# BoyBaykiller/OpenTK-PathTracer

Hardware: AMD Instinct MI355X
Metric: Msamples/sec + ms/frame @1080p 8-bounce default scene, 1/2/4/8 GPU (higher is better)
Workload: dtype f32

## Files before the change

### opentk-pathtracer_amd/csrc/mi355pt.cpp

```cpp
#include "pt_renderer.hpp"

#include <cmath>
#include <cstdio>
#include <cstdlib>
#include <chrono>
#include <thread>
#include <cstring>
#include <new>

namespace {
thread_local std::string g_create_error;
}

namespace ptimpl {

#define FEED_LOG(...)                                                                                                                \
    do {                                                                                                                             \
        if (pt::tuning().feedLog) {                                                                                                  \
            std::fprintf(stderr, "[feed %9.1f us] ", std::chrono::duration<double, std::micro>(std::chrono::steady_clock::now().time_since_epoch()).count() - 1e6 * (long long)(std::chrono::duration<double>(std::chrono::steady_clock::now().time_since_epoch()).count())); \
            std::fprintf(stderr, "%p ", (void *)h);                                                                                  \
            std::fprintf(stderr, __VA_ARGS__);                                                                                       \
            std::fprintf(stderr, "\n");                                                                                              \
        }                                                                                                                            \
    } while (0)
// ... 97 lines not shown
}

unsigned int feed_word(const pt_renderer::FeedState &f, bool closed)
{
    return (closed ? pt::kFeedClosed : 0u) | ((unsigned int)f.published << 16) | (f.slots16 & 0xffffu);
}

void feed_close(pt_handle h)
{
    pt_renderer::FeedState &f = h->feed;
    if (!f.open) return;
    f.open = false;
    __atomic_store_n(&h->hostFeed[f.hostWord], feed_word(f, true), __ATOMIC_RELEASE);
    FEED_LOG("close word %d = %08x (first %d published %d pendingSlot %d)", f.hostWord, feed_word(f, true), f.firstFrame, f.published, f.pendingSlot);
    for (pt_renderer::LaunchRecord &r : h->unverified)
        if (r.a.launchSeq == f.seq) r.a.batchFrames = f.published;
    const unsigned int tickets = (unsigned int)(((long long)f.published * f.tilesFrame + f.queueChunk - 1) / f.queueChunk);
    (f.streamIdx == 1 ? h->chainQueueBase : h->stripeQueueBase[0]) += tickets;
    for (int j = 0; j < f.published; j++) h->feedDoneBase[f.streamIdx][j & 7] += f.pixelsPerFrame;
    if (f.published >= 8) h->feedIdleStrikes = 0;
    if (f.pendingSlot >= 0) {
        h->fusedOrphanSlot = f.pendingSlot;
        f.pendingSlot = -1;
    }
}

static int resolve_fused_orphan(pt_handle h)
{
    if (h->fusedOrphanSlot < 0) return PT_OK;
    FEED_LOG("orphan present of slot %d: tone map from the image", h->fusedOrphanSlot);
    PresentSlot &s = h->slots[h->fusedOrphanSlot];
    h->fusedOrphanSlot = -1;
    if (!s.fusedWaiting) return PT_OK;
    void *const image = s.boundDev ? s.boundDev : s.dRgba8;
    const size_t pixels = (size_t)s.rows * s.width;
    PT_HIP(h, ptimpl::launch_tone_map(s.arithmetic, h->accum(), image, pixels, h->stream));
    PT_HIP(h, hipEventRecord(s.toneMapped, h->stream));
    PT_HIP(h, hipStreamWaitEvent(h->copyStream, s.toneMapped, 0));
    if (!s.boundDev) PT_HIP(h, hipMemcpyAsync(s.host, s.dRgba8, pixels * 4, hipMemcpyDeviceToHost, h->copyStream));
    PT_HIP(h, hipEventRecord(s.copied, h->copyStream));
    s.fusedWaiting = false;
    s.fedPresent = false;
    s.snapSource = nullptr;
    return PT_OK;
}

int join_stripes(pt_handle h, bool repairNow)
{
    FEED_LOG("join (repairNow %d, frame %d, pending %d, tagsLive %d, %zu remembered, flag %u)", (int)repairNow, h->frame, h->pendingFrames, (int)h->tagsLive, h->unverified.size(),
             h->hostErrWord ? *(volatile unsigned int *)h->hostErrWord : 0u);
    feed_close(h);
    if (h->pendingFrames > 0) {
        h->flushFinal = true;
        int rc = flush_frames(h);
        h->flushFinal = false;
        if (rc) return rc;
    }
    h->snapFrame = -1;
    h->mainDirty = true;
    h->chainBroken = true;
    if (h->chainPending) {
        PT_HIP(h, hipStreamWaitEvent(h->stream, h->chainDone, 0));
        h->chainPending = false;
    }
    for (int j = 0; j < kMaxStripes; j++) {
        if (h->stripePending[j]) {
            if (j > 0) PT_HIP(h, hipStreamWaitEvent(h->stream, h->stripeDone[j], 0));
            h->stripePending[j] = false;
        }
    }
    const bool raised = h->hostErrWord && *(volatile unsigned int *)h->hostErrWord;
    if (raised || (!h->unverified.empty() && (repairNow || h->tagsLive))) {
        if (raised) note_abandonment(h);
        if (int rc = enqueue_repairs(h, !raised && !h->repairPendingAll)) return rc;
        h->repairPendingAll = false;
    }
    return resolve_fused_orphan(h);
}

int settle_handover(pt_handle h)
{
    if (h->hostErrWord && *(volatile unsigned int *)h->hostErrWord) {
        note_abandonment(h);
        if (int rc = enqueue_repairs(h, false)) return rc;
        h->repairPendingAll = false;
        PT_HIP(h, hipStreamSynchronize(h->stream));
    }
    if (!h->unverified.empty()) FEED_LOG("settle: %zu launches forgotten (synchronised, flag down)", h->unverified.size());
    h->unverified.clear();
    if (h->repairCheckDue) {
        h->repairCheckDue = false;
        unsigned int ctl[4] = {0, 0, 0, 0};
        PT_HIP(h, hipMemcpy(ctl, h->dRepairCtl, sizeof ctl, hipMemcpyDeviceToHost));
        if (ctl[1] != h->inconsistentSeen) {
            h->inconsistentSeen = ctl[1];
            return fail(h, PT_E_HIP, "hand-over repair: a pixel's frame tag fits no launch of this handle (image inconsistent; pt_reset / pt_set_size start over)");
        }
    }
    return PT_OK;
}

int fix_alpha(pt_handle h, bool repairNow)
{
    if (int rc = join_stripes(h, repairNow)) return rc;
    if (h->tagsLive) {
        PT_HIP(h, pt::launch_set_alpha(h->accum(), h->tilePixels(), h->stream));
        h->tagsLive = false;
    }
    return PT_OK;
}

int ensure_stripe(pt_handle h, int j)
{
    if (j > 0 && !h->stripeStream[j]) PT_HIP(h, hipStreamCreateWithFlags(&h->stripeStream[j], hipStreamNonBlocking));
    if (!h->stripeDone[j]) PT_HIP(h, hipEventCreateWithFlags(&h->stripeDone[j], hipEventDisableTiming));
    return PT_OK;
}

hipStream_t stripe_stream(pt_handle h, int j) { return j == 0 ? h->stream : h->stripeStream[j]; }

int free_first_hit(pt_handle h)
{
    if (!h->dFirstHit) return PT_OK;
    PT_HIP(h, hipStreamSynchronize(h->stream));
    PT_HIP(h, hipFree(h->dFirstHit));
    h->dFirstHit = nullptr;
    return PT_OK;
}

int free_denoise(pt_handle h)
{
    h->denoiseResult = -1;
    h->denoiseVarianceValid = false;
    h->denoiseIntegratedValid = h->denoiseHistoryUsed = false;
    for (pt_renderer::DenoiseSet &set : h->denoiseSet) set.valid = false;
    if (!h->dGuides && !h->dDenoise[0] && !h->dDenoise[1] && !h->dVariance && !h->denoiseSet[0].image && !h->denoiseSet[0].guides &&
        !h->denoiseSet[1].image && !h->denoiseSet[1].guides)
        return PT_OK;
    PT_HIP(h, hipStreamSynchronize(h->stream));
    if (h->dGuides) PT_HIP(h, hipFree(h->dGuides));
    h->dGuides = nullptr;
    if (h->dVariance) PT_HIP(h, hipFree(h->dVariance));
    h->dVariance = nullptr;
    for (float4 *&img : h->dDenoise) {
        if (img) PT_HIP(h, hipFree(img));
        img = nullptr;
    }
    for (pt_renderer::DenoiseSet &set : h->denoiseSet) {
        if (set.image) PT_HIP(h, hipFree(set.image));
        set.image = nullptr;
        if (set.guides) PT_HIP(h, hipFree(set.guides));
        set.guides = nullptr;
    }
    return PT_OK;
}
}

namespace {

int ensure_accum(pt_handle h)
{
    size_t need = h->tilePixels();
    if (need > h->accumCapacity) {
        if (h->dAccum) PT_HIP(h, hipFree(h->dAccum));
        h->dAccum = nullptr;
        h->accumCapacity = 0;
        PT_HIP(h, hipMalloc((void **)&h->dAccum, need * sizeof(float4)));
        h->accumCapacity = need;
    }
    if ((size_t)((h->width + 7) / 8) * (size_t)((h->rows + 7) / 8) > h->tileMaskTiles) {
        const size_t tiles = (size_t)((h->width + 7) / 8) * (size_t)((h->rows + 7) / 8);
        PT_HIP(h, hipStreamSynchronize(h->stream));
        if (h->dTileMasks) PT_HIP(h, hipFree(h->dTileMasks));
        h->dTileMasks = nullptr;
        h->tileMaskTiles = 0;
        h->tileMasksValid = false;
        PT_HIP(h, hipMalloc((void **)&h->dTileMasks, tiles * pt::kTileMaskWords * sizeof(unsigned long long)));
        h->tileMaskTiles = tiles;
    }
    const size_t flagTiles = (size_t)((h->width + 7) / 8) * (size_t)((h->rows + 7) / 8);
    if (flagTiles > h->tileFlagTiles) {
        PT_HIP(h, hipStreamSynchronize(h->stream));
        if (h->dTileFlags) PT_HIP(h, hipFree(h->dTileFlags));
        h->dTileFlags = nullptr;
        h->tileFlagTiles = 0;
        PT_HIP(h, hipMalloc((void **)&h->dTileFlags, flagTiles * sizeof(unsigned int)));
        PT_HIP(h, hipMemsetAsync(h->dTileFlags, 0, flagTiles * sizeof(unsigned int), h->stream));
        h->tileFlagTiles = flagTiles;
    }
#ifdef PT_AUDIT
    if (need > h->auditCapacity) {
        PT_HIP(h, hipStreamSynchronize(h->stream));
        if (h->dAudit) PT_HIP(h, hipFree(h->dAudit));
        h->dAudit = nullptr;
        h->auditCapacity = 0;
        PT_HIP(h, hipMalloc((void **)&h->dAudit, need * sizeof(unsigned long long)));
        h->auditCapacity = need;
    }
#endif
    return PT_OK;
}

int audit_forget(pt_handle h)
{
    if (h->dAudit) PT_HIP(h, hipMemsetAsync(h->dAudit, 0xFF, h->tilePixels() * sizeof(unsigned long long), h->stream));
    return PT_OK;
}

int clear_accum(pt_handle h)
{
    if (h->boundAccum && h->boundBytes < h->tilePixels() * sizeof(float4))
        return fail(h, PT_E_BAD_ARGUMENT, "bound result buffer is smaller than the tile");
    if (int rc = join_stripes(h)) return rc;
    PT_HIP(h, pt::launch_clear(h->accum(), h->tilePixels(), h->stream));
    h->tagsLive = false;
    return audit_forget(h);
}

}

extern "C" {

PT_API const char *pt_version(void) { return "mi355pt 0.1 (gfx950, pt-f32)"; }

PT_API int pt_device_count(void)
{
    int n = 0;
    if (hipGetDeviceCount(&n) != hipSuccess) return 0;
    return n;
}

PT_API const char *pt_last_error(pt_handle h)
{
    if (h && h->magic == ptimpl::kAlive) return h->error.c_str();
    return g_create_error.c_str();
}

PT_API int pt_create(int device_id, int width, int height, pt_handle *out)
{
    if (!out) return fail(nullptr, PT_E_BAD_ARGUMENT, "out == NULL");
    *out = nullptr;
    if (width <= 0 || height <= 0) return fail(nullptr, PT_E_BAD_ARGUMENT, "width/height must be positive");
    if (width > PT_MAX_IMAGE_DIM || height > PT_MAX_IMAGE_DIM)
        return fail(nullptr, PT_E_OUT_OF_RANGE, "width/height exceed PT_MAX_IMAGE_DIM (32767)");
    int n = 0;
    hipError_t e = hipGetDeviceCount(&n);
    if (e != hipSuccess || n <= 0)
        return fail(nullptr, PT_E_NO_DEVICE, "no HIP device available (libmi355pt has no CPU fallback)");
    if (device_id < 0 || device_id >= n) return fail(nullptr, PT_E_BAD_ARGUMENT, "device_id out of range");
    pt_renderer *h = new (std::nothrow) pt_renderer();
    if (!h) return fail(nullptr, PT_E_OUT_OF_MEMORY, "host allocation failed");
    h->device = device_id;
    {
        const pt::Tuning &t = pt::tuning();
        if (t.drainCompaction >= -1) h->drainCompaction = t.drainCompaction;
        if (t.batchWorkgroupsPerCU >= 1 && t.batchWorkgroupsPerCU <= 8) h->batchWorkgroupsPerCU = t.batchWorkgroupsPerCU;
        if (t.frameBatch >= 1 && t.frameBatch <= 64) { h->maxBatch = t.frameBatch; h->maxBatchExplicit = true; }
        if (t.queueChunk >= 1 && t.queueChunk <= 1024) h->queueChunk = t.queueChunk;
    }
    h->width = width;
    h->height = height;
    h->y0 = 0;
    h->rows = height;
#define PT_CREATE_HIP(call)                                                                                            \
    do {                                                                                                               \
        hipError_t e2_ = (call);                                                                                       \
        if (e2_ != hipSuccess) {                                                                                       \
            int rc_ = hip_fail(nullptr, e2_, #call);                                                                   \
            pt_destroy(h);                                                                                             \
            return rc_;                                                                                                \
        }                                                                                                              \
    } while (0)
    PT_CREATE_HIP(hipSetDevice(device_id));
    PT_CREATE_HIP(hipStreamCreateWithFlags(&h->ownStream, hipStreamNonBlocking));
    h->stream = h->ownStream;
    PT_CREATE_HIP(hipEventCreateWithFlags(&h->inputsReady, hipEventDisableTiming));
    PT_CREATE_HIP(hipEventCreateWithFlags(&h->gatherReady, hipEventDisableTiming));
    PT_CREATE_HIP(hipStreamCreateWithFlags(&h->copyStream, hipStreamNonBlocking));
    PT_CREATE_HIP(hipEventCreate(&h->evBegin));
    PT_CREATE_HIP(hipEventCreate(&h->evEnd));
    PT_CREATE_HIP(hipMalloc((void **)&h->dObjects, PT_GAME_OBJECTS_UBO_SIZE));
    PT_CREATE_HIP(hipMemsetAsync(h->dObjects, 0, PT_GAME_OBJECTS_UBO_SIZE, h->stream));
    PT_CREATE_HIP(hipMalloc((void **)&h->dGrid, (ptgrid::kMaxCells + 1) * 2 + ptgrid::kMaxRefs + 16));
    PT_CREATE_HIP(hipMalloc((void **)&h->dLut, 256 * sizeof(float)));
    PT_CREATE_HIP(hipMalloc((void **)&h->dQueue, ptimpl::kQueueWords * sizeof(unsigned int)));
    PT_CREATE_HIP(hipMemsetAsync(h->dQueue, 0, ptimpl::kQueueWords * sizeof(unsigned int), h->stream));
    PT_CREATE_HIP(hipHostMalloc((void **)&h->hostErrWord, sizeof(unsigned int), hipHostMallocMapped));
    *h->hostErrWord = 0;
    PT_CREATE_HIP(hipHostGetDevicePointer((void **)&h->devErrWord, h->hostErrWord, 0));
    PT_CREATE_HIP(hipMalloc((void **)&h->dAbandon, sizeof(unsigned int)));
    PT_CREATE_HIP(hipMemsetAsync(h->dAbandon, 0xFF, sizeof(unsigned int), h->stream));
    PT_CREATE_HIP(hipMalloc((void **)&h->dRepairCtl, 4 * sizeof(unsigned int)));
    PT_CREATE_HIP(hipMemsetAsync(h->dRepairCtl, 0, 4 * sizeof(unsigned int), h->stream));
    {
        int khz = 0;
        if (hipDeviceGetAttribute(&khz, hipDeviceAttributeWallClockRate, device_id) != hipSuccess || khz <= 0) khz = 100000;
        (void)hipGetLastError();
        h->wallClockKhz = khz;
        const pt::Tuning &t = pt::tuning();
        const double unitsPerMs = (double)khz / 1024.0;
        double budget = (double)t.handoverBudgetMs * unitsPerMs, check = (double)t.handoverCheckUs * unitsPerMs / 1000.0;
        if (budget > 1.0e9) budget = 1.0e9;
        if (check > budget / 4.0) check = budget / 4.0;
        h->waitBudgetUnits = (unsigned int)budget;
        h->waitCheckUnits = (unsigned int)check;
    }
    PT_CREATE_HIP(hipHostMalloc((void **)&h->hostFeed, pt_renderer::kFeedHostWords * sizeof(unsigned int), hipHostMallocMapped | hipHostMallocCoherent));
    for (int i = 0; i < pt_renderer::kFeedHostWords; i++) h->hostFeed[i] = pt::kFeedClosed;
    PT_CREATE_HIP(hipHostMalloc((void **)&h->hostFeedDone, pt_renderer::kFeedHostWords * sizeof(unsigned int), hipHostMallocMapped | hipHostMallocCoherent));
    std::memset(h->hostFeedDone, 0, pt_renderer::kFeedHostWords * sizeof(unsigned int));
    PT_CREATE_HIP(hipHostGetDevicePointer((void **)&h->devFeedHostDone, h->hostFeedDone, 0));
    PT_CREATE_HIP(hipHostGetDevicePointer((void **)&h->devFeedHost, h->hostFeed, 0));
    PT_CREATE_HIP(hipMalloc((void **)&h->dFeedDev, (size_t)2 * pt::kFeedBcastSlots * pt::kFeedBcastStride * sizeof(unsigned int)));
    PT_CREATE_HIP(hipMemsetAsync(h->dFeedDev, 0, (size_t)2 * pt::kFeedBcastSlots * pt::kFeedBcastStride * sizeof(unsigned int), h->stream));
    PT_CREATE_HIP(hipMalloc((void **)&h->dFeedDone, (size_t)16 * pt::kFeedDoneStride * sizeof(unsigned long long)));
    PT_CREATE_HIP(hipMemsetAsync(h->dFeedDone, 0, (size_t)16 * pt::kFeedDoneStride * sizeof(unsigned long long), h->stream));
    PT_CREATE_HIP(hipHostMalloc((void **)&h->hostStarted, ptimpl::kStartedWords * sizeof(unsigned int), hipHostMallocMapped | hipHostMallocCoherent));
    std::memset(h->hostStarted, 0, ptimpl::kStartedWords * sizeof(unsigned int));
    PT_CREATE_HIP(hipHostGetDevicePointer((void **)&h->devStarted, h->hostStarted, 0));
#ifdef PT_AUDIT
    {
        const size_t words = 4 + (size_t)pt::kAuditLogRecords * pt::kAuditRecordWords;
        PT_CREATE_HIP(hipHostMalloc((void **)&h->hostAuditLog, words * sizeof(unsigned int), hipHostMallocMapped | hipHostMallocCoherent));
        std::memset(h->hostAuditLog, 0, words * sizeof(unsigned int));
        PT_CREATE_HIP(hipHostGetDevicePointer((void **)&h->devAuditLog, h->hostAuditLog, 0));
    }
#endif
    {
        hipDeviceProp_t prop;
        PT_CREATE_HIP(hipGetDeviceProperties(&prop, device_id));
        h->numCUs = prop.multiProcessorCount > 0 ? prop.multiProcessorCount : 256;
    }
    float lut[256];
    make_srgb_lut(lut);
    PT_CREATE_HIP(hipMemcpyAsync(h->dLut, lut, sizeof lut, hipMemcpyHostToDevice, h->stream));
    PT_CREATE_HIP(hipStreamSynchronize(h->stream));
#undef PT_CREATE_HIP
    int rc = ensure_accum(h);
    if (rc == PT_OK) rc = clear_accum(h);
    if (rc != PT_OK) {
        g_create_error = h->error;
        pt_destroy(h);
        return rc;
    }
    *out = h;
    return PT_OK;
}

PT_API int pt_destroy(pt_handle h)
{
    PT_CHECK_HANDLE(h);
    if (h->isGroup()) return ptimpl::group_destroy(h);
    h->pendingFrames = 0;
    (void)hipSetDevice(h->device);
    ptimpl::feed_close(h);
    for (int j = 0; j < ptimpl::kMaxStripes; j++)
        if (h->stripeStream[j]) (void)hipStreamSynchronize(h->stripeStream[j]);
    if (h->stream) (void)hipStreamSynchronize(h->stream);
    if (h->copyStream) (void)hipStreamSynchronize(h->copyStream);
    for (int k = 0; k < pt_renderer::kSnapshots; k++) {
        if (h->snapRead[k]) (void)hipEventDestroy(h->snapRead[k]);
        if (h->dSnap[k]) (void)hipFree(h->dSnap[k]);
    }
    ptimpl::free_slots(h);
    if (h->copyStream) (void)hipStreamDestroy(h->copyStream);
    if (h->gatherReady) (void)hipEventDestroy(h->gatherReady);
    for (int j = 0; j < ptimpl::kMaxStripes; j++)
        if (h->stripeStream[j]) (void)hipStreamSynchronize(h->stripeStream[j]);
    if (h->stream) (void)hipStreamSynchronize(h->stream);
    for (int j = 0; j < ptimpl::kMaxStripes; j++) {
        if (h->stripeDone[j]) (void)hipEventDestroy(h->stripeDone[j]);
        if (h->stripeStream[j]) (void)hipStreamDestroy(h->stripeStream[j]);
    }
    if (h->inputsReady) (void)hipEventDestroy(h->inputsReady);
    for (hipEvent_t e : h->launchEvents)
        if (e) (void)hipEventDestroy(e);
    if (h->dAbandon) (void)hipFree(h->dAbandon);
    if (h->dRepairCtl) (void)hipFree(h->dRepairCtl);
    if (h->dTileFlags) (void)hipFree(h->dTileFlags);
    if (h->dObjects) (void)hipFree(h->dObjects);
    if (h->dGrid) (void)hipFree(h->dGrid);
    if (h->dLut) (void)hipFree(h->dLut);
    if (h->dQueue) (void)hipFree(h->dQueue);
    if (h->dTileMasks) (void)hipFree(h->dTileMasks);
    if (h->hostErrWord) (void)hipHostFree(h->hostErrWord);
    if (h->hostStarted) (void)hipHostFree(h->hostStarted);
    if (h->hostFeed) (void)hipHostFree(h->hostFeed);
    if (h->hostFeedDone) (void)hipHostFree(h->hostFeedDone);
    if (h->dFeedDev) (void)hipFree(h->dFeedDev);
    if (h->dFeedDone) (void)hipFree(h->dFeedDone);
    for (hipEvent_t e : h->feedWordBusy)
        if (e) (void)hipEventDestroy(e);
    if (h->feedResetEvent) (void)hipEventDestroy(h->feedResetEvent);
    if (h->hostAuditLog) (void)hipHostFree(h->hostAuditLog);
    if (h->dAudit) (void)hipFree(h->dAudit);
    if (h->dEnv) (void)hipFree(h->dEnv);
    if (h->dAccum) (void)hipFree(h->dAccum);
    if (h->dRgba8) (void)hipFree(h->dRgba8);
    if (h->dFirstHit) (void)hipFree(h->dFirstHit);
    if (h->dPick) (void)hipFree(h->dPick);
    if (h->dGuides) (void)hipFree(h->dGuides);
    if (h->dVariance) (void)hipFree(h->dVariance);
    if (h->dDenoise[0]) (void)hipFree(h->dDenoise[0]);
    if (h->dDenoise[1]) (void)hipFree(h->dDenoise[1]);
    for (pt_renderer::DenoiseSet &set : h->denoiseSet) {
        if (set.image) (void)hipFree(set.image);
        if (set.guides) (void)hipFree(set.guides);
    }
    if (h->dTimeline) (void)hipFree(h->dTimeline);
    if (h->evBegin) (void)hipEventDestroy(h->evBegin);
    if (h->evEnd) (void)hipEventDestroy(h->evEnd);
    if (h->ownStream) (void)hipStreamDestroy(h->ownStream);
    h->magic = 0;
    delete h;
    return PT_OK;
}

PT_API int pt_set_size(pt_handle h, int width, int height)
{
    PT_CHECK_HANDLE(h);
    if (width <= 0 || height <= 0) return fail(h, PT_E_BAD_ARGUMENT, "width/height must be positive");
    if (width > PT_MAX_IMAGE_DIM || height > PT_MAX_IMAGE_DIM)
        return fail(h, PT_E_OUT_OF_RANGE, "width/height exceed PT_MAX_IMAGE_DIM (32767)");
    if (h->isGroup()) return ptimpl::group_set_size(h, width, height);
    if (int rc = flush_frames(h)) return rc;
    if (int rc = bind_device(h)) return rc;
    if (int rc = join_stripes(h)) return rc;
    if (int rc = ptimpl::free_first_hit(h)) return rc;
    if (int rc = ptimpl::free_denoise(h)) return rc;
    h->resetEpoch++;
    h->width = width;
    h->height = height;
    h->y0 = 0;
    h->rows = height;
    h->bandRows = 0;
    h->frame = 0;
    h->tileMasksValid = false;
    h->launchesSinceInputChange = 0;
    if (int rc = ensure_accum(h)) return rc;
    return clear_accum(h);
}

PT_API int pt_set_tile(pt_handle h, int y0, int rows)
{
    PT_CHECK_HANDLE(h);
    if (h->isGroup()) return fail(h, PT_E_BAD_ARGUMENT, "a group handle owns its tiling (pt_multi_set_partition)");
    if (int rc = flush_frames(h)) return rc;
    if (y0 < 0 || rows <= 0 || y0 + rows > h->height) return fail(h, PT_E_BAD_ARGUMENT, "tile outside the image");
    if (int rc = bind_device(h)) return rc;
    if (int rc = join_stripes(h)) return rc;
    if (int rc = ptimpl::free_first_hit(h)) return rc;
    if (int rc = ptimpl::free_denoise(h)) return rc;
    h->resetEpoch++;
    h->y0 = y0;
    h->rows = rows;
    h->bandRows = 0;
    h->frame = 0;
    h->tileMasksValid = false;
    h->launchesSinceInputChange = 0;
    if (int rc = ensure_accum(h)) return rc;
    return clear_accum(h);
}

PT_API int pt_set_interleaved_tile(pt_handle h, int rank, int world, int band_rows)
{
    PT_CHECK_HANDLE(h);
    if (h->isGroup()) return fail(h, PT_E_BAD_ARGUMENT, "a group handle owns its tiling (pt_multi_set_partition)");
    if (int rc = flush_frames(h)) return rc;
    if (world < 1 || rank < 0 || rank >= world || band_rows < 8 || (band_rows & 7))
        return fail(h, PT_E_BAD_ARGUMENT, "need 0 <= rank < world and band_rows a positive multiple of 8");
    if (int rc = bind_device(h)) return rc;
    long long rows = 0;
    for (long long b = rank; b * band_rows < h->height; b += world) {
        long long top = (b + 1) * band_rows;
        rows += (top < h->height ? top : h->height) - b * band_rows;
    }
    if (rows <= 0) return fail(h, PT_E_BAD_ARGUMENT, "this rank owns no rows (image too small for world * band_rows)");
    if (int rc = join_stripes(h)) return rc;
    if (int rc = ptimpl::free_first_hit(h)) return rc;
    if (int rc = ptimpl::free_denoise(h)) return rc;
    h->resetEpoch++;
    h->y0 = 0;
    h->rows = (int)rows;
    h->bandRows = band_rows;
    h->bandWorld = world;
    h->bandRank = rank;
    h->frame = 0;
    h->tileMasksValid = false;
    h->launchesSinceInputChange = 0;
    if (int rc = ensure_accum(h)) return rc;
    return clear_accum(h);
}

#define PT_FAN_OUT(h, call)                                                                                            \
    do {                                                                                                               \
        if ((h)->isGroup()) {                                                                                          \
            for (pt_handle part : (h)->parts) {                                                                        \
                int rc_ = (call);                                                                                      \
                if (rc_ != PT_OK) return fail((h), rc_, part->error);                                                  \
            }                                                                                                          \
            return PT_OK;                                                                                              \
        }                                                                                                              \
    } while (0)

PT_API int pt_reset(pt_handle h)
{
    PT_CHECK_HANDLE(h);
    PT_FAN_OUT(h, pt_reset(part));
    if (int rc = flush_frames(h)) return rc;
    if (int rc = bind_device(h)) return rc;
    if (int rc = ptimpl::fix_alpha(h)) return rc;
    h->frame = 0;
    h->resetEpoch++;
    return audit_forget(h);
}

PT_API int pt_set_params(pt_handle h, int num_spheres, int num_cuboids, int ray_depth, int spp, float focal_length,
                         float aperture_diameter)
{
    PT_CHECK_HANDLE(h);
    PT_FAN_OUT(h, pt_set_params(part, num_spheres, num_cuboids, ray_depth, spp, focal_length, aperture_diameter));
    if (num_spheres == h->numSpheres && num_cuboids == h->numCuboids && ray_depth == h->rayDepth && spp == h->spp &&
        std::memcmp(&focal_length, &h->focalLength, sizeof(float)) == 0 && std::memcmp(&aperture_diameter, &h->apertureDiameter, sizeof(float)) == 0)
        return PT_OK;
    if (num_spheres < 0 || num_spheres > PT_MAX_SPHERES || num_cuboids < 0 || num_cuboids > PT_MAX_CUBOIDS)
        return fail(h, PT_E_OUT_OF_RANGE, "object counts exceed the GameObjectsUBO arrays (256 spheres / 64 cuboids)");
    if (ray_depth < 0 || spp < 1) return fail(h, PT_E_BAD_ARGUMENT, "ray_depth must be >= 0 and spp >= 1");
    if (ray_depth > PT_MAX_RAY_DEPTH || spp > PT_MAX_SPP)
        return fail(h, PT_E_OUT_OF_RANGE, "ray_depth / spp exceed PT_MAX_RAY_DEPTH / PT_MAX_SPP (4095)");
    if (int rc = flush_frames(h)) return rc;
    if (num_spheres != h->numSpheres) h->gridDirty = true;
    if (num_spheres != h->numSpheres || num_cuboids != h->numCuboids || focal_length != h->focalLength || aperture_diameter != h->apertureDiameter) {
        h->tileMasksValid = false;
        h->launchesSinceInputChange = 0;
    }
    h->numSpheres = num_spheres;
    h->numCuboids = num_cuboids;
    h->rayDepth = ray_depth;
    h->spp = spp;
    h->focalLength = focal_length;
    h->apertureDiameter = aperture_diameter;
    return PT_OK;
}

PT_API int pt_upload_basic_data(pt_handle h, int byte_offset, int size, const void *src)
{
    PT_CHECK_HANDLE(h);
    PT_FAN_OUT(h, pt_upload_basic_data(part, byte_offset, size, src));
    if (!src) return fail(h, PT_E_BAD_ARGUMENT, "src == NULL");
    if (byte_offset < 0 || size < 0 || (long long)byte_offset + size > PT_BASIC_DATA_UBO_SIZE)
        return fail(h, PT_E_OUT_OF_RANGE, "BasicDataUBO range outside [0,144)");
    if (std::memcmp(h->basic + byte_offset, src, (size_t)size) == 0) return PT_OK;
    h->statFlushes++;
    if (int rc = flush_frames(h)) return rc;
    std::memcpy(h->basic + byte_offset, src, (size_t)size);
    h->tileMasksValid = false; h->launchesSinceInputChange = 0;
    return PT_OK;
}

PT_API int pt_upload_game_objects(pt_handle h, int byte_offset, int size, const void *src)
{
    PT_CHECK_HANDLE(h);
    PT_FAN_OUT(h, pt_upload_game_objects(part, byte_offset, size, src));
    if (!src) return fail(h, PT_E_BAD_ARGUMENT, "src == NULL");
    if (byte_offset < 0 || size < 0 || (long long)byte_offset + size > PT_GAME_OBJECTS_UBO_SIZE)
        return fail(h, PT_E_OUT_OF_RANGE, "GameObjectsUBO range outside [0,26624)");
    if (size == 0) return PT_OK;
    if (std::memcmp(h->objectsShadow + byte_offset, src, (size_t)size) == 0) return PT_OK;
    h->statFlushes++;
    if (int rc = bind_device(h)) return rc;
    if (int rc = join_stripes(h)) return rc;
    PT_HIP(h, hipMemcpyAsync((char *)h->dObjects + byte_offset, src, (size_t)size, hipMemcpyHostToDevice, h->stream));
    std::memcpy(h->objectsShadow + byte_offset, src, (size_t)size);
    if (byte_offset < PT_MAX_SPHERES * 80) h->gridDirty = true;
    h->tileMasksValid = false;
    h->launchesSinceInputChange = 0;
    return PT_OK;
}

PT_API int pt_set_environment(pt_handle h, int face_size, int format, const void *const faces[6])
{
    PT_CHECK_HANDLE(h);
    PT_FAN_OUT(h, pt_set_environment(part, face_size, format, faces));
    if (face_size <= 0 || face_size > 16384) return fail(h, PT_E_BAD_ARGUMENT, "face_size out of range");
    if (format != PT_ENV_RGBA32F && format != PT_ENV_SRGB8_A8) return fail(h, PT_E_BAD_ARGUMENT, "unknown format");
    if (!faces) return fail(h, PT_E_BAD_ARGUMENT, "faces == NULL");
    for (int f = 0; f < 6; f++)
        if (!faces[f]) return fail(h, PT_E_BAD_ARGUMENT, "faces[i] == NULL");
    if (int rc = bind_device(h)) return rc;
    if (int rc = join_stripes(h)) return rc;
    size_t faceBytes = (size_t)face_size * face_size * (format == PT_ENV_RGBA32F ? 16 : 4);
    size_t total = faceBytes * 6;
    if (total > h->envBytes) {
        PT_HIP(h, hipStreamSynchronize(h->stream));
        if (h->dEnv) PT_HIP(h, hipFree(h->dEnv));
        h->dEnv = nullptr;
        h->envBytes = 0;
        PT_HIP(h, hipMalloc(&h->dEnv, total));
        h->envBytes = total;
    }
    for (int f = 0; f < 6; f++)
        PT_HIP(h, hipMemcpyAsync((char *)h->dEnv + f * faceBytes, faces[f], faceBytes, hipMemcpyHostToDevice, h->stream));
    h->envSize = face_size;
    h->envFormat = format;
    return PT_OK;
}

}

namespace {

bool gpu_busy(pt_handle h);

struct LaunchMode {
    bool tagged = false, chainable = false;
    int stripes = 1, kernelVariant = 0;
};

constexpr long long kSmallChunkBelowTiles = 12000;

int fill_frame_args(pt_handle h, pt::FrameArgs &a, int firstFrame, int n)
{
    std::memcpy(a.invProj, h->basic, 64);
    std::memcpy(a.invView, h->basic + 64, 64);
    std::memcpy(a.viewPos, h->basic + 128, 12);
    a.focalLength = h->focalLength;
    a.apertureDiameter = h->apertureDiameter;
    a.width = h->width;
    a.height = h->height;
    a.invW = 1.0f / (float)h->width;
    a.invH = 1.0f / (float)h->height;
    a.numSpheres = h->numSpheres;
    a.numCuboids = h->numCuboids;
    a.rayDepth = h->rayDepth;
    a.spp = h->spp;
    a.frame = firstFrame;
    a.batchFrames = n;
    a.envSize = h->envSize;
    a.envFormat = h->envFormat;
    a.objects = h->dObjects;
    a.env = h->dEnv;
    a.srgbLut = h->dLut;
    a.tilesX = (h->width + 7) / 8;
    a.bandRows = h->bandRows;
    a.bandWorld = h->bandWorld;
    a.bandRank = h->bandRank;
    a.localRow0 = 0;
    a.numCUs = h->numCUs;
    a.queueChunk = h->queueChunk > 0 ? h->queueChunk : (n > 1 && (long long)((h->width + 7) / 8) * ((h->rows + 7) / 8) < kSmallChunkBelowTiles ? 4 : 8);
    a.errorWord = h->devErrWord;
    a.startedFlags = nullptr;
    a.launchSeq = 0;
    a.snapshot = nullptr;
    a.audit = nullptr;
    a.auditLog = h->devAuditLog;
    a.auditSabotage = 0;
#ifdef PT_AUDIT
    a.auditSabotage = pt::tuning().auditSabotage;
#endif
    a.timeline = h->dTimeline;
    if (h->gridDirty) {
        h->gridDirty = false;
        h->grid = ptgrid::build((const float *)h->objectsShadow, h->numSpheres);
        ptgrid::sphere_runs((const float *)h->objectsShadow, h->numSpheres, h->sphereRunStart);
        if (h->grid.valid) {
            if (int rc = join_stripes(h)) return rc;
            PT_HIP(h, hipMemcpyAsync(h->dGrid, h->grid.packed.data(), h->grid.packed.size(), hipMemcpyHostToDevice, h->stream));
        }
    }
    a.grid = h->grid.valid ? h->dGrid : nullptr;
    a.gridBytes = h->grid.valid ? (int)h->grid.packed.size() : 0;
    a.gridLdsBytes = 0;
    for (int k = 0; k < 3; k++) {
        a.gridDims[k] = h->grid.dims[k];
        a.gridLo[k] = h->grid.lo[k];
        a.gridHi[k] = h->grid.hi[k];
        a.gridCell[k] = h->grid.cell[k];
        a.gridInvCell[k] = h->grid.invCell[k];
        a.gridCenter[k] = h->grid.center[k];
    }
    a.gridReach2 = h->grid.reach2;
    std::memcpy(a.sphereRunStart, h->sphereRunStart, sizeof(a.sphereRunStart));
    a.tileMasks = nullptr;
    a.tagged = 0;
    a.keepTags = 0;
    a.chainTag = 0.0f;
    a.abandonWord = nullptr;
    a.tileFlags = nullptr;
    a.waitBudget = h->waitBudgetUnits;
    a.waitCheckInterval = h->waitCheckUnits;
    return PT_OK;
}

LaunchMode choose_launch_mode(pt_handle h, pt::FrameArgs &a, int n)
{
    LaunchMode m;
    m.kernelVariant = h->variant;
    if (h->arithmetic != PT_ARITH_CONTRACT) {
        m.chainable = false;
        m.tagged = false;
        m.stripes = 1;
        m.kernelVariant = 1;
        a.variant = m.kernelVariant;
        a.drainCompaction = 0;
        a.tagged = 0;
        return m;
    }
    const bool noSingleTagged = pt::tuning().noSingleTagged != 0;
    m.chainable = h->variant == 0 && !h->externalStream() && !ptimpl::timeline_blocks_pipelining(h);
    m.tagged = h->variant == 0 && (n > 1 || (m.chainable && !noSingleTagged && (gpu_busy(h) || (h->sawBatch && h->presentCadence != 1))));
    const int shortWg = pt::tuning().shortWorkgroupsPerCU;
    if (m.tagged) { m.stripes = 1; m.kernelVariant = 10 + (n < 8 ? shortWg : h->batchWorkgroupsPerCU) - 1; h->batchLaunched = true; if (n > 1) h->sawBatch = true; }
    else if (h->variant == 0 && h->externalStream()) { m.stripes = 1; m.kernelVariant = 14; }
    else if (h->variant == 0) { m.stripes = 2; m.kernelVariant = 14; }
    else if (h->variant >= 20 && h->variant < 50) { m.stripes = h->variant / 10; m.kernelVariant = 10 + h->variant % 10; }
    if (h->rows < 16 * m.stripes) m.stripes = 1;
    a.variant = m.kernelVariant;
    a.drainCompaction = h->drainCompaction >= 0 ? h->drainCompaction : (m.stripes > 1 || m.tagged ? 0 : 32);
    a.tagged = m.tagged ? 1 : 0;
    return m;
}

int use_tile_masks(pt_handle h, pt::FrameArgs &a)
{
    if (pt::tuning().tileMasks == 0) return PT_OK;
    const bool settled = h->launchesSinceInputChange > 2;
    h->launchesSinceInputChange += a.batchFrames;
    if (!h->tileMasksValid && settled) {
        if (int rc = join_stripes(h)) return rc;
        if ((size_t)a.tilesX * a.tilesY <= h->tileMaskTiles) {
            PT_HIP(h, pt::launch_tile_masks(a, h->dTileMasks, h->stream));
            h->tileMasksValid = true;
            h->statMaskBuilds++;
        }
    }
    if (h->tileMasksValid) a.tileMasks = h->dTileMasks;
    return PT_OK;
}

bool predecessor_resident(pt_handle h)
{
    for (int i = 0; i < h->lastWorkgroups; i++)
        if (((volatile unsigned int *)h->hostStarted)[i] != h->launchSeq) return false;
    return true;
}
bool wait_for_residency(pt_handle h, const pt::FrameArgs &a, long waitUs)
{
    if (pt::tuning().serialLaunches != 0) return false;
    if (h->overlapHoldoff > 0) h->overlapHoldoff--;
    const bool mayChain = !h->chainBroken && h->lastWorkgroups > 0 && h->lastWorkgroups <= ptimpl::kStartedWords && h->overlapHoldoff == 0;
    bool resident = mayChain && predecessor_resident(h);
    const bool bigShare = (long long)a.tilesX * a.tilesY >= 12000;
    if (mayChain && !resident && (bigShare || h->flushFinal)) {
        const auto t0 = std::chrono::steady_clock::now();
        while (!resident) {
            const auto waited = std::chrono::duration_cast<std::chrono::microseconds>(std::chrono::steady_clock::now() - t0).count();
            if (waited >= waitUs) break;
            if (waited > 200) std::this_thread::sleep_for(std::chrono::microseconds(20));
            resident = predecessor_resident(h);
        }
    }
    return resident;
}

void arm_handover(pt_handle h, pt::FrameArgs &a)
{
    a.launchSeq = ++h->launchSeq;
    if (a.launchSeq == 0 || a.launchSeq >= 0xfffffff0u) a.launchSeq = h->launchSeq = 1;
    a.abandonWord = h->dAbandon;
    a.tileFlags = a.chainTag == 0.0f ? h->dTileFlags : nullptr;
}
void remember_launch(pt_handle h, const pt::FrameArgs &a, hipEvent_t done)
{
    auto flag_down = [&]() -> bool { return !(h->hostErrWord && *(volatile unsigned int *)h->hostErrWord); };
    while (h->unverified.size() > 2 && hipEventQuery(h->unverified.front().done) == hipSuccess && flag_down()) {
        FEED_LOG("remember: launch %u frames [%d,+%d) seen complete with the flag down: forgotten", h->unverified.front().a.launchSeq, h->unverified.front().a.frame, h->unverified.front().a.batchFrames);
        h->unverified.pop_front();
    }
    (void)hipGetLastError();
    static_assert(pt_renderer::kLaunchEvents / 2 <= pt::kMaxUnverifiedLaunches, "frame-tag window (pt_kernels.hpp)");
    if (h->unverified.size() >= (size_t)pt_renderer::kLaunchEvents / 2) {
        (void)hipEventSynchronize(h->unverified.front().done);
        if (flag_down()) h->unverified.pop_front();
    }
    h->unverified.push_back({a, done});
    FEED_LOG("launch %u frames [%d,+%d) chainTag %g keepTags %d variant %d spp %d (%zu remembered)", a.launchSeq, a.frame, a.batchFrames, (double)a.chainTag, a.keepTags, a.variant, a.spp, h->unverified.size());
    if (pt::tuning().feedLog >= 2) {
        unsigned int w = 0, q[2] = {0, 0};
        (void)hipDeviceSynchronize();
        (void)hipMemcpy(&w, h->dAbandon, 4, hipMemcpyDeviceToHost);
        (void)hipMemcpy(&q[0], h->dQueue, 4, hipMemcpyDeviceToHost);
        (void)hipMemcpy(&q[1], h->dQueue + ptimpl::kChainQueueWord, 4, hipMemcpyDeviceToHost);
        FEED_LOG("  after launch %u: abandon word %08x, tickets main %u (host %u) chain %u (host %u), flag %u", a.launchSeq, w, q[0], h->stripeQueueBase[0], q[1], h->chainQueueBase,
                 h->hostErrWord ? *(volatile unsigned int *)h->hostErrWord : 0u);
// ... 707 lines not shown
        if (int rc = join_stripes(h)) return rc;
        if (s.inFlight) PT_HIP(h, hipStreamWaitEvent(h->stream, s.copied, 0));
        PT_HIP(h, ptimpl::launch_tone_map(h->presentArithmetic, h->accum(), image, pixels, h->stream));
        PT_HIP(h, hipEventRecord(s.toneMapped, h->stream));
        PT_HIP(h, hipStreamWaitEvent(h->copyStream, s.toneMapped, 0));
    }
    if (!s.boundDev) PT_HIP(h, hipMemcpyAsync(s.host, s.dRgba8, pixels * 4, hipMemcpyDeviceToHost, h->copyStream));
    PT_HIP(h, hipEventRecord(s.copied, h->copyStream));
    s.inFlight = true;
    s.valid = false;
    s.frame = h->frame;
    s.rows = h->rows;
    s.width = h->width;
    s.arithmetic = h->presentArithmetic;
    s.snapSource = nullptr;
    return PT_OK;
}

PT_API int pt_present_bind_device_image(pt_handle h, int slot, void *device_rgba8, size_t bytes)
{
    PT_CHECK_HANDLE(h);
    if (slot < 0 || slot >= PT_PRESENT_SLOTS) return fail(h, PT_E_BAD_ARGUMENT, "slot must be 0..PT_PRESENT_SLOTS-1");
    if (h->isGroup()) return fail(h, PT_E_BAD_ARGUMENT, "pt_present_bind_device_image is not available on a group handle");
    if (device_rgba8 && bytes < h->tilePixels() * 4) return fail(h, PT_E_BAD_ARGUMENT, "device image smaller than rows*width*4 bytes");
    if (int rc = bind_device(h)) return rc;
    ptimpl::PresentSlot &s = h->slots[slot];
    if (h->feed.open || h->fusedOrphanSlot >= 0) {
        ptimpl::feed_close(h);
        if (int rc = join_stripes(h)) return rc;
    }
    if (s.inFlight) {
        if (int rc = ptimpl::wait_slot(h, s, nullptr)) return rc;
        s.inFlight = false;
    }
    s.valid = false;
    s.fedPresent = false;
    s.boundDev = device_rgba8;
    s.boundBytes = device_rgba8 ? bytes : 0;
    return PT_OK;
}

PT_API int pt_present_wait(pt_handle h, int slot, const uint8_t **out_host_rgba8, size_t *out_row_pitch_bytes,
                           int *out_frame_index)
{
    PT_CHECK_HANDLE(h);
    if (slot < 0 || slot >= PT_PRESENT_SLOTS) return fail(h, PT_E_BAD_ARGUMENT, "slot must be 0..PT_PRESENT_SLOTS-1");
    ptimpl::PresentSlot &s = h->slots[slot];
    if (!s.inFlight && !s.valid) return fail(h, PT_E_BAD_ARGUMENT, "nothing was presented into this slot");
    if (int rc = bind_device(h)) return rc;
    if (s.inFlight) {
        bool fusedAbandoned = false;
        if (int rc = ptimpl::wait_slot(h, s, &fusedAbandoned)) return rc;
        if (fusedAbandoned) s.abandonEpoch = h->abandonEpoch - 1;
        s.inFlight = false;
        s.valid = true;
        if (!h->isGroup() && s.snapSource != nullptr) {
            if (h->hostErrWord && *(volatile unsigned int *)h->hostErrWord) {
                if (int rc = join_stripes(h)) return rc;
                if (*(volatile unsigned int *)h->hostErrWord) ptimpl::note_abandonment(h);
            }
            if (s.abandonEpoch != h->abandonEpoch && s.fedPresent) {
                if (int rc = ptimpl::fix_alpha(h)) return rc;
                void *const image = s.boundDev ? s.boundDev : s.dRgba8;
                const size_t pixels = (size_t)s.rows * s.width;
                PT_HIP(h, ptimpl::launch_tone_map(s.arithmetic, h->accum(), image, pixels, h->stream));
                if (!s.boundDev) PT_HIP(h, hipMemcpyAsync(s.host, s.dRgba8, pixels * 4, hipMemcpyDeviceToHost, h->stream));
                PT_HIP(h, hipStreamSynchronize(h->stream));
                if (int rc = ptimpl::settle_handover(h)) return rc;
                s.abandonEpoch = h->abandonEpoch;
                s.frame = h->frame;
            } else if (s.abandonEpoch != h->abandonEpoch) {
                int k = -1;
                for (int i = 0; i < pt_renderer::kSnapshots; i++)
                    if (h->dSnap[i] == s.snapSource && h->snapGeneration[i] == s.snapGeneration) k = i;
                if (k < 0)
                    return fail(h, PT_E_HIP, "present: a launch was abandoned and this slot's snapshot has been reused (call pt_present_wait on a slot before presenting into it again)");
                if (int rc = join_stripes(h)) return rc;
                void *const image = s.boundDev ? s.boundDev : s.dRgba8;
                const size_t pixels = (size_t)s.rows * s.width;
                PT_HIP(h, ptimpl::launch_tone_map(s.arithmetic, h->dSnap[k], image, pixels, h->stream));
                if (!s.boundDev) PT_HIP(h, hipMemcpyAsync(s.host, s.dRgba8, pixels * 4, hipMemcpyDeviceToHost, h->stream));
                PT_HIP(h, hipStreamSynchronize(h->stream));
                s.abandonEpoch = h->abandonEpoch;
            }
        }
    }
    if (out_host_rgba8) *out_host_rgba8 = s.boundDev ? nullptr : s.host;
    if (out_row_pitch_bytes) *out_row_pitch_bytes = (size_t)s.width * 4;
    if (out_frame_index) *out_frame_index = s.frame;
    return PT_OK;
}

PT_API int pt_get_frame_index(pt_handle h, int *out)
{
    PT_CHECK_HANDLE(h);
    if (!out) return fail(h, PT_E_BAD_ARGUMENT, "out == NULL");
    *out = h->isGroup() ? h->parts[0]->frame : h->frame;
    return PT_OK;
}

PT_API int pt_synchronize(pt_handle h)
{
    PT_CHECK_HANDLE(h);
    PT_FAN_OUT(h, pt_synchronize(part));
    if (int rc = bind_device(h)) return rc;
    if (int rc = ptimpl::fix_alpha(h, false)) return rc;
    PT_HIP(h, hipStreamSynchronize(h->stream));
    return ptimpl::settle_handover(h);
}

PT_API int pt_atmosphere_upload_data(pt_handle h, int byte_offset, int size, const void *src)
{
    PT_CHECK_HANDLE(h);
    PT_FAN_OUT(h, pt_atmosphere_upload_data(part, byte_offset, size, src));
    if (!src) return fail(h, PT_E_BAD_ARGUMENT, "src == NULL");
    if (byte_offset < 0 || size < 0 || (long long)byte_offset + size > PT_ATMOSPHERE_UBO_SIZE)
        return fail(h, PT_E_OUT_OF_RANGE, "AtmosphericDataUBO range outside [0,464)");
    std::memcpy(h->atmoUbo + byte_offset, src, (size_t)size);
    return PT_OK;
}

PT_API int pt_atmosphere_render(pt_handle h, int size, int i_steps, int j_steps, const float light_pos[3],
                                float light_intensity)
{
    PT_CHECK_HANDLE(h);
    PT_FAN_OUT(h, pt_atmosphere_render(part, size, i_steps, j_steps, light_pos, light_intensity));
    if (size <= 0 || size > 8192 || i_steps < 0 || j_steps < 0 || !light_pos)
        return fail(h, PT_E_BAD_ARGUMENT, "bad atmosphere parameters");
    if (int rc = bind_device(h)) return rc;
    if (int rc = join_stripes(h)) return rc;
    size_t total = (size_t)6 * size * size * 16;
    if (total > h->envBytes) {
        PT_HIP(h, hipStreamSynchronize(h->stream));
        if (h->dEnv) PT_HIP(h, hipFree(h->dEnv));
        h->dEnv = nullptr;
        h->envBytes = 0;
        PT_HIP(h, hipMalloc(&h->dEnv, total));
        h->envBytes = total;
    }
    pt::AtmoArgs a;
    std::memcpy(a.invProj, h->atmoUbo, 64);
    std::memcpy(a.invView, h->atmoUbo + 64, 6 * 64);
    a.lightPos[0] = light_pos[0];
    a.lightPos[1] = light_pos[1];
    a.lightPos[2] = light_pos[2];
    a.lightIntensity = light_intensity < 0.0f ? 0.0f : light_intensity;
    a.size = size;
    a.iSteps = i_steps;
    a.jSteps = j_steps;
    a.out = (float4 *)h->dEnv;
    PT_HIP(h, h->atmoArithmetic == PT_ARITH_REFERENCE ? pt::launch_atmosphere_reference(a, h->stream) : pt::launch_atmosphere(a, h->stream));
    h->envSize = size;
    h->envFormat = PT_ENV_RGBA32F;
    return PT_OK;
}

PT_API int pt_atmosphere_set_arithmetic(pt_handle h, int mode)
{
    PT_CHECK_HANDLE(h);
    if (mode != PT_ARITH_CONTRACT && mode != PT_ARITH_REFERENCE) return fail(h, PT_E_BAD_ARGUMENT, "mode must be PT_ARITH_CONTRACT or PT_ARITH_REFERENCE");
    PT_FAN_OUT(h, pt_atmosphere_set_arithmetic(part, mode));
    h->atmoArithmetic = mode;
    return PT_OK;
}

PT_API int pt_present_set_arithmetic(pt_handle h, int mode)
{
    PT_CHECK_HANDLE(h);
    if (mode != PT_ARITH_CONTRACT && mode != PT_ARITH_REFERENCE) return fail(h, PT_E_BAD_ARGUMENT, "mode must be PT_ARITH_CONTRACT or PT_ARITH_REFERENCE");
    PT_FAN_OUT(h, pt_present_set_arithmetic(part, mode));
    if (mode == h->presentArithmetic) return PT_OK;
    if (int rc = bind_device(h)) return rc;
    if (int rc = join_stripes(h)) return rc;
    h->presentArithmetic = mode;
    return PT_OK;
}

PT_API int pt_read_environment(pt_handle h, float *dst, int *out_face_size)
{
    PT_CHECK_HANDLE(h);
    if (h->isGroup()) {
        int rc = pt_read_environment(h->parts[0], dst, out_face_size);
        return rc == PT_OK ? rc : fail(h, rc, h->parts[0]->error);
    }
    if (!h->dEnv) return fail(h, PT_E_NO_ENVIRONMENT, "no environment set");
    if (out_face_size) *out_face_size = h->envSize;
    if (!dst) return PT_OK;
    if (int rc = bind_device(h)) return rc;
    if (int rc = join_stripes(h)) return rc;
    size_t n = (size_t)6 * h->envSize * h->envSize;
    if (h->envFormat == PT_ENV_RGBA32F) {
        PT_HIP(h, hipMemcpyAsync(dst, h->dEnv, n * 16, hipMemcpyDeviceToHost, h->stream));
        PT_HIP(h, hipStreamSynchronize(h->stream));
        return PT_OK;
    }
    float4 *tmp = nullptr;
    PT_HIP(h, hipMalloc((void **)&tmp, n * 16));
    hipError_t e = pt::launch_env_to_float(h->dEnv, h->envSize, h->envFormat, h->dLut, tmp, h->stream);
    if (e == hipSuccess) e = hipMemcpyAsync(dst, tmp, n * 16, hipMemcpyDeviceToHost, h->stream);
    if (e == hipSuccess) e = hipStreamSynchronize(h->stream);
    (void)hipFree(tmp);
    if (e != hipSuccess) return hip_fail(h, e, "pt_read_environment");
    return PT_OK;
}

PT_API int pt_result_device_ptr(pt_handle h, void **out_ptr, size_t *out_bytes)
{
    PT_CHECK_HANDLE(h);
    if (h->isGroup()) return ptimpl::group_result_device_ptr(h, out_ptr, out_bytes);
    if (int rc = bind_device(h)) return rc;
    if (int rc = ptimpl::fix_alpha(h)) return rc;
    if (out_ptr) *out_ptr = h->accum();
    if (out_bytes) *out_bytes = h->tilePixels() * sizeof(float4);
    return PT_OK;
}

PT_API int pt_bind_result_buffer(pt_handle h, void *device_ptr, size_t bytes)
{
    PT_CHECK_HANDLE(h);
    if (h->isGroup()) return fail(h, PT_E_BAD_ARGUMENT, "pt_bind_result_buffer is not available on a group handle");
    if (device_ptr && bytes < h->tilePixels() * sizeof(float4))
        return fail(h, PT_E_BAD_ARGUMENT, "buffer smaller than rows*width*16 bytes");
    if (int rc = bind_device(h)) return rc;
    if (int rc = ptimpl::fix_alpha(h)) return rc;
    h->boundAccum = (float4 *)device_ptr;
    h->boundBytes = device_ptr ? bytes : 0;
    if (device_ptr) PT_HIP(h, pt::launch_set_alpha(h->boundAccum, h->tilePixels(), h->stream));
    return audit_forget(h);
}

PT_API int pt_set_stream(pt_handle h, void *hip_stream)
{
    PT_CHECK_HANDLE(h);
    if (h->isGroup()) return fail(h, PT_E_BAD_ARGUMENT, "pt_set_stream is not available on a group handle");
    if (int rc = bind_device(h)) return rc;
    if (int rc = ptimpl::fix_alpha(h)) return rc;
    PT_HIP(h, hipStreamSynchronize(h->stream));
    h->stream = hip_stream ? (hipStream_t)hip_stream : h->ownStream;
    return PT_OK;
}

PT_API int pt_timer_begin(pt_handle h)
{
    PT_CHECK_HANDLE(h);
    PT_FAN_OUT(h, pt_timer_begin(part));
    if (int rc = bind_device(h)) return rc;
    if (int rc = join_stripes(h)) return rc;
    PT_HIP(h, hipEventRecord(h->evBegin, h->stream));
    return PT_OK;
}

PT_API int pt_timer_end(pt_handle h, float *out_ms)
{
    PT_CHECK_HANDLE(h);
    if (!out_ms) return fail(h, PT_E_BAD_ARGUMENT, "out == NULL");
    if (h->isGroup()) return ptimpl::group_timer_end(h, out_ms);
    if (int rc = bind_device(h)) return rc;
    if (int rc = join_stripes(h)) return rc;
    PT_HIP(h, hipEventRecord(h->evEnd, h->stream));
    PT_HIP(h, hipEventSynchronize(h->evEnd));
    PT_HIP(h, hipEventElapsedTime(out_ms, h->evBegin, h->evEnd));
    return PT_OK;
}

static_assert(pt::kFirstHitCuboidBase == PT_MAX_SPHERES, "first-hit ids: cuboid j is PT_MAX_SPHERES + j");

static void first_hit_args(pt_handle h, pt::FrameArgs &a, int frame_index)
{
    std::memset(&a, 0, sizeof a);
    std::memcpy(a.invProj, h->basic, 64);
    std::memcpy(a.invView, h->basic + 64, 64);
    std::memcpy(a.viewPos, h->basic + 128, 12);
    a.focalLength = h->focalLength;
    a.apertureDiameter = h->apertureDiameter;
    a.width = h->width;
    a.height = h->height;
    a.invW = 1.0f / (float)h->width;
    a.invH = 1.0f / (float)h->height;
    a.y0 = h->y0;
    a.rows = h->rows;
    a.bandRows = h->bandRows;
    a.bandWorld = h->bandWorld;
    a.bandRank = h->bandRank;
    a.numSpheres = h->numSpheres;
    a.numCuboids = h->numCuboids;
    a.rayDepth = 1;
    a.spp = 1;
    a.batchFrames = 1;
    a.frame = frame_index;
    a.objects = h->dObjects;
    a.tilesX = (h->width + 7) / 8;
    a.tilesY = (h->rows + 7) / 8;
}

PT_API int pt_first_hit_render(pt_handle h, int frame_index)
{
    PT_CHECK_HANDLE(h);
    if (frame_index < 0) return fail(h, PT_E_BAD_ARGUMENT, "frame_index must be >= 0");
    PT_FAN_OUT(h, pt_first_hit_render(part, frame_index));
    if (int rc = bind_device(h)) return rc;
    if (int rc = join_stripes(h)) return rc;
    if (!h->dFirstHit) PT_HIP(h, hipMalloc((void **)&h->dFirstHit, h->tilePixels() * 2 * sizeof(float4)));
    pt::FrameArgs a;
    first_hit_args(h, a, frame_index);
    PT_HIP(h, pt::launch_first_hit(a, h->dFirstHit, -1, h->stream));
    return PT_OK;
}
// ... 568 lines not shown
```

### opentk-pathtracer_amd/csrc/pt_denoise.hip

```cpp
#include "pt_kernel_common.hpp"

namespace pt {

__global__ __launch_bounds__(256) void pt_guides_kernel(const FrameArgs a, float4 *guides)
{
    SceneLds sc = stage_scene(a);
    const int tid = threadIdx.x;
    const int ns = a.numSpheres, nc = a.numCuboids;
    float4 *ids = g_lds + scene_lds_bytes(ns, nc, 0, false) / sizeof(float4);
    for (int i = tid; i < ns + nc; i += 256) ids[4 * i] = make_float4((float)(i < ns ? i : kFirstHitCuboidBase + (i - ns)), 0.0f, 0.0f, 0.0f);
    __syncthreads();
    sc.mat = ids;
    const int b = xcd_band_id(blockIdx.x, gridDim.x);
    const int wave = tid >> 6, lane = tid & 63;
    const int tile = b * 4 + wave;
    if (tile >= a.tilesX * a.tilesY) return;
    const int tx = tile % a.tilesX, ty = tile / a.tilesX;
    const int px = tx * 8 + (lane & 7);
    const int ly = ty * 8 + (lane >> 3);
    if (px >= a.width || ly >= a.rows) return;
#ifdef PT_PROFILE
    unsigned long long prof_dummy[10] = {0, 0, 0, 0, 0, 0, 0, 0, 0, 0};
#endif
    uint32_t seed = pixel_seed(px, global_row(a, ly), a.frame);
    v3 ro, rd;
    primary_ray(a, px, global_row(a, ly), seed, ro, rd);
    Hit h;
    const bool hit = ray_trace(sc, ns, nc, ro, rd, h PROF_DUMMY);
    float4 g0 = make_float4(0.0f, 0.0f, 0.0f, __int_as_float(-1));
    float4 g1 = make_float4(0.0f, 0.0f, 0.0f, __builtin_inff());
    if (hit) {
        g0 = make_float4(rd.x * h.T + ro.x, rd.y * h.T + ro.y, rd.z * h.T + ro.z, __int_as_float((int)h.m.albedo.x));
        g1 = make_float4(h.normal.x, h.normal.y, h.normal.z, h.T);
    }
    const size_t at = (size_t)ly * a.width + px;
    guides[2 * at] = g0;
    guides[2 * at + 1] = g1;
}

hipError_t launch_guides(const FrameArgs &args, float4 *guides, hipStream_t stream)
{
    FrameArgs a = args;
    a.materialsInLds = 0;
    a.gridLdsBytes = 0;
    a.envFormat = 0;
    if (a.tilesX < 1 || a.tilesY < 1) return hipErrorInvalidValue;
    const int tiles = a.tilesX * a.tilesY;
    const size_t lds = scene_lds_bytes(a.numSpheres, a.numCuboids, 0, false) + (size_t)(a.numSpheres + a.numCuboids) * 4 * sizeof(float4);
    hipLaunchKernelGGL(pt_guides_kernel, dim3((tiles + 3) / 4), dim3(256), lds, stream, a, guides);
    return hipGetLastError();
}

PT_DEV float dn_u(float r, float g, float b)
{
    const float l = (0.2126f * r + 0.7152f * g) + 0.0722f * b;
    return l / (1.0f + l);
}

template <int S>
__global__ __launch_bounds__(256) void pt_atrous_kernel(const AtrousArgs a)
{
    constexpr int TX = S ? 16 : 64, TY = S ? 16 : 4, HALO = 2 * S, LW = TX + 2 * HALO, LH = TY + 2 * HALO;
    __shared__ float4 sG0[S ? LW * LH : 1], sG1[S ? LW * LH : 1], sC[S ? LW * LH : 1];
    const int tid = threadIdx.x, lx = tid % TX, ly = tid / TX;
    const int x0 = blockIdx.x * TX, y0 = blockIdx.y * TY;
    const int px = x0 + lx, py = y0 + ly;
    const int step = S ? S : a.step;
    if constexpr (S != 0) {
        for (int i = tid; i < LW * LH; i += 256) {
            const int qx = x0 - HALO + i % LW, qy = y0 - HALO + i / LW;
            if (qx >= 0 && qx < a.width && qy >= 0 && qy < a.height) {
                const size_t at = (size_t)qy * a.width + qx;
                float4 c = a.colIn[at];
                c.w = dn_u(c.x, c.y, c.z);
                sG0[i] = a.guides[2 * at];
                sG1[i] = a.guides[2 * at + 1];
                sC[i] = c;
            }
        }
        __syncthreads();
    }
    if (px >= a.width || py >= a.height) return;
    const size_t center = (size_t)py * a.width + px;
    const int lc = (ly + HALO) * LW + lx + HALO;
    const float4 g0p = S ? sG0[lc] : a.guides[2 * center];
    const float4 g1p = S ? sG1[lc] : a.guides[2 * center + 1];
    float4 cp = S ? sC[lc] : a.colIn[center];
    const int idp = __float_as_int(g0p.w);
    float4 out = make_float4(cp.x, cp.y, cp.z, 1.0f);
    if (idp != -1) {
        const float up = S ? cp.w : dn_u(cp.x, cp.y, cp.z);
        const float planeDen = a.sigmaPlane * g1p.w;
        float W = 0.0f, Sr = 0.0f, Sg = 0.0f, Sb = 0.0f;
#pragma unroll
        for (int dy = -2; dy <= 2; dy++) {
#pragma unroll
            for (int dx = -2; dx <= 2; dx++) {
                const float kx = dx == 0 ? 0.375f : (dx == 1 || dx == -1 ? 0.25f : 0.0625f);
                const float ky = dy == 0 ? 0.375f : (dy == 1 || dy == -1 ? 0.25f : 0.0625f);
                const float hk = kx * ky;
                const int qx = px + step * dx, qy = py + step * dy;
                if (qx < 0 || qx >= a.width || qy < 0 || qy >= a.height) continue;
                const size_t at = (size_t)qy * a.width + qx;
                const int lq = lc + dy * S * LW + dx * S;
                const float4 g0q = S ? sG0[lq] : a.guides[2 * at];
                if (__float_as_int(g0q.w) != idp) continue;
                const float4 g1q = S ? sG1[lq] : a.guides[2 * at + 1];
                const float4 cq = S ? sC[lq] : a.colIn[at];
                const float d = (g1p.x * g1q.x + g1p.y * g1q.y) + g1p.z * g1q.z;
                float wn = d > 0.0f ? d : 0.0f;
                for (int k = 0; k < a.normalPower; k++) wn = wn * wn;
                const float ex = g0q.x - g0p.x, ey = g0q.y - g0p.y, ez = g0q.z - g0p.z;
                const float e = (g1p.x * ex + g1p.y * ey) + g1p.z * ez;
                const float r = e / planeDen;
                const float z = 1.0f - r * r;
                const float wz = z > 0.0f ? z : 0.0f;
                const float uq = S ? cq.w : dn_u(cq.x, cq.y, cq.z);
                const float da = (uq - up) * a.invSigma;
                const float c1 = 1.0f - da * da;
                const float c2 = c1 > 0.0f ? c1 : 0.0f;
                const float wc = c2 * c2;
                const float w = ((hk * wn) * wz) * wc;
                W = W + w;
                Sr = Sr + w * cq.x;
                Sg = Sg + w * cq.y;
                Sb = Sb + w * cq.z;
            }
        }
        if (W > 0.0f) out = make_float4(Sr / W, Sg / W, Sb / W, 1.0f);
    }
    a.colOut[center] = out;
}

hipError_t launch_atrous(const AtrousArgs &a, hipStream_t stream)
{
    if (a.width < 1 || a.height < 1 || a.step < 1) return hipErrorInvalidValue;
    if (a.step <= 2) {
        const dim3 grid((a.width + 15) / 16, (a.height + 15) / 16);
        if (a.step == 1) hipLaunchKernelGGL(pt_atrous_kernel<1>, grid, dim3(256), 0, stream, a);
        else hipLaunchKernelGGL(pt_atrous_kernel<2>, grid, dim3(256), 0, stream, a);
    } else {
        hipLaunchKernelGGL(pt_atrous_kernel<0>, dim3((a.width + 63) / 64, (a.height + 3) / 4), dim3(256), 0, stream, a);
    }
    return hipGetLastError();
}

__global__ void pt_denoise_copy_kernel(const float4 *in, float4 *out, size_t n)
{
    size_t i = (size_t)blockIdx.x * blockDim.x + threadIdx.x;
    const size_t stride = (size_t)gridDim.x * blockDim.x;
    for (; i < n; i += stride) {
        const float4 c = in[i];
        out[i] = make_float4(c.x, c.y, c.z, 1.0f);
    }
}

hipError_t launch_denoise_copy(const float4 *in, float4 *out, size_t n, hipStream_t stream)
{
    if (n == 0) return hipSuccess;
    size_t blocks = (n + 255) / 256;
    if (blocks > 2048) blocks = 2048;
    hipLaunchKernelGGL(pt_denoise_copy_kernel, dim3((unsigned)blocks), dim3(256), 0, stream, in, out, n);
    return hipGetLastError();
}

constexpr int kVarOutsideId = (int)0x80000000;

template <int R>
__global__ __launch_bounds__(256) void pt_variance_kernel(const VarianceArgs a)
{
    static_assert(R == 3, "the definition's 7x7 window");
    constexpr int LW = 23;
    __shared__ float2 sU[LW * LW];
    const int tid = threadIdx.x, lx = tid & 15, ly = tid >> 4;
    const int x0 = blockIdx.x * 16, y0 = blockIdx.y * 16;
// ... 227 lines not shown
```

### opentk-pathtracer_amd/csrc/pt_device.hpp

```cpp
#pragma once
#include "pt_debug_hooks.hpp"
#include "pt_kernels.hpp"
#include "pt_math.hpp"

namespace pt {

struct Material {
    v3 albedo;
    float specularChance;
    v3 emissiv;
    float specularRoughness;
    v3 absorbance;
    float refractionChance;
    float refractionRoughness, ior;
};

struct Hit {
    float T;
    bool fromInside;
    v3 nearHitPos, normal;
    Material m;
};

struct SceneLds {
    const float4 *sph;
    const float4 *cmin;
    const float4 *cmax;
    const float4 *mat;
    const float *invr;
    const float *lut;
    const float4 *objects;
    const unsigned short *gridStarts;
    const unsigned char *gridRefs;
};

__host__ __device__ inline size_t scene_lds_bytes(int ns, int nc, int envFormat, bool matInLds, int gridLdsBytes = 0)
{
    return (size_t)(ns + 2 * nc + (matInLds ? 4 * (ns + nc) : 0)) * 16 + (size_t)((ns + 3) & ~3) * 4 + (envFormat == 1 ? 1024 : 0) +
           (size_t)gridLdsBytes;
}

typedef const __attribute__((address_space(3))) float *LdsFloats;
struct EnvRef {
    const void *data;
    LdsFloats lut;
    int size, format;
};

typedef const __attribute__((address_space(4))) FrameArgs *ColdArgs;
typedef const __attribute__((address_space(4))) float *ColdFloats;
PT_DEV ColdArgs cold_args()
{
    ColdArgs p = (ColdArgs)__builtin_amdgcn_kernarg_segment_ptr();
    asm volatile("" : "+s"(p));
    return p;
}

PT_DEV v3 env_texel(const EnvRef &e, int face, int x, int y)
{
    size_t idx = ((size_t)face * e.size + (size_t)y) * e.size + (size_t)x;
    if (e.format == 0) {
        float4 t = ((const float4 *)e.data)[idx];
        return V(t.x, t.y, t.z);
    }
    uchar4 t = ((const uchar4 *)e.data)[idx];
    return V(e.lut[t.x], e.lut[t.y], e.lut[t.z]);
}

PT_DEV void face_to_dir(int face, float sc, float tc, float &x, float &y, float &z)
{
    switch (face) {
    case 0: x = 1.0f; y = -tc; z = -sc; break;
    case 1: x = -1.0f; y = -tc; z = sc; break;
    case 2: x = sc; y = 1.0f; z = tc; break;
    case 3: x = sc; y = -1.0f; z = -tc; break;
    case 4: x = sc; y = -tc; z = 1.0f; break;
    default: x = -sc; y = -tc; z = -1.0f; break;
    }
}

PT_DEV void dir_to_face(float x, float y, float z, int &face, float &sc, float &tc, float &ma)
{
    float ax = f_abs(x), ay = f_abs(y), az = f_abs(z);
    if (az >= f_max(ax, ay)) {
        face = z < 0.0f ? 5 : 4; ma = az; sc = z < 0.0f ? -x : x; tc = -y;
    } else if (ax >= ay) {
        face = x < 0.0f ? 1 : 0; ma = ax; sc = x < 0.0f ? z : -z; tc = -y;
    } else {
        face = y < 0.0f ? 3 : 2; ma = ay; sc = x; tc = y < 0.0f ? -z : z;
    }
}

PT_DEV v3 env_texel_wrapped(const EnvRef &e, int face, int ix, int iy)
{
    int S = e.size;
    if (ix >= 0 && ix < S && iy >= 0 && iy < S) return env_texel(e, face, ix, iy);
    float fs = (float)S;
    float rfs = f_div_ieee(1.0f, fs);
    float sc = ((float)ix + 0.5f) * rfs * 2.0f - 1.0f;
    float tc = ((float)iy + 0.5f) * rfs * 2.0f - 1.0f;
    float x, y, z, ma, nsc, ntc;
    int nface;
    face_to_dir(face, sc, tc, x, y, z);
    dir_to_face(x, y, z, nface, nsc, ntc, ma);
    float rma = f_rcp(ma);
    float u = (nsc * rma * 0.5f + 0.5f) * fs;
    float v = (ntc * rma * 0.5f + 0.5f) * fs;
    int nx = (int)__builtin_floorf(u), ny = (int)__builtin_floorf(v);
    nx = nx < 0 ? 0 : (nx > S - 1 ? S - 1 : nx);
    ny = ny < 0 ? 0 : (ny > S - 1 ? S - 1 : ny);
    return env_texel(e, nface, nx, ny);
}

PT_DEV v3 sample_env(const EnvRef &e, v3 d)
{
    int S = e.size, face;
    float sc, tc, ma;
    dir_to_face(d.x, d.y, d.z, face, sc, tc, ma);
    float ima = 0.5f * f_rcp(ma);
    float fs = (float)S;
    float u = f_fma(sc, ima, 0.5f) * fs - 0.5f;
    float v = f_fma(tc, ima, 0.5f) * fs - 0.5f;
    u = f_min(f_max(u, -1.0f), fs);
    v = f_min(f_max(v, -1.0f), fs);
    float fu = __builtin_floorf(u), fv = __builtin_floorf(v);
    float wu = u - fu, wv = v - fv;
    int x0 = (int)fu, y0 = (int)fv, x1 = x0 + 1, y1 = y0 + 1;
    bool offx0 = x0 < 0, offx1 = x1 >= S, offy0 = y0 < 0, offy1 = y1 >= S;
    float w00 = (1.0f - wu) * (1.0f - wv), w10 = wu * (1.0f - wv), w01 = (1.0f - wu) * wv, w11 = wu * wv;
    v3 t00, t10, t01, t11;
    if (!(offx0 || offx1 || offy0 || offy1)) {
        const unsigned base = ((unsigned)face * (unsigned)S + (unsigned)y0) * (unsigned)S + (unsigned)x0;
        if (e.format == 0) {
            const float4 *p = (const float4 *)e.data + base;
            float4 a = p[0], b = p[1], c = p[S], d = p[S + 1];
            t00 = V(a.x, a.y, a.z); t10 = V(b.x, b.y, b.z); t01 = V(c.x, c.y, c.z); t11 = V(d.x, d.y, d.z);
        } else {
            const uchar4 *p = (const uchar4 *)e.data + base;
            uchar4 a = p[0], b = p[1], c = p[S], d = p[S + 1];
            t00 = V(e.lut[a.x], e.lut[a.y], e.lut[a.z]); t10 = V(e.lut[b.x], e.lut[b.y], e.lut[b.z]);
            t01 = V(e.lut[c.x], e.lut[c.y], e.lut[c.z]); t11 = V(e.lut[d.x], e.lut[d.y], e.lut[d.z]);
        }
    } else {
        bool miss00 = offx0 && offy0, miss10 = offx1 && offy0, miss01 = offx0 && offy1, miss11 = offx1 && offy1;
        v3 zero = V(0.0f, 0.0f, 0.0f);
        t00 = miss00 ? zero : env_texel_wrapped(e, face, x0, y0);
        t10 = miss10 ? zero : env_texel_wrapped(e, face, x1, y0);
        t01 = miss01 ? zero : env_texel_wrapped(e, face, x0, y1);
        t11 = miss11 ? zero : env_texel_wrapped(e, face, x1, y1);
        if (miss00 || miss10 || miss01 || miss11) {
            float a = (miss00 ? w00 : miss10 ? w10 : miss01 ? w01 : w11) * 0.333333343f;
            w00 = miss00 ? 0.0f : w00 + a;
            w10 = miss10 ? 0.0f : w10 + a;
            w01 = miss01 ? 0.0f : w01 + a;
            w11 = miss11 ? 0.0f : w11 + a;
        }
    }
    v3 o;
    o.x = f_fma(t11.x, w11, f_fma(t01.x, w01, f_fma(t10.x, w10, t00.x * w00)));
    o.y = f_fma(t11.y, w11, f_fma(t01.y, w01, f_fma(t10.y, w10, t00.y * w00)));
    o.z = f_fma(t11.z, w11, f_fma(t01.z, w01, f_fma(t10.z, w10, t00.z * w00)));
    return o;
}

PT_DEV float f_sign(float x) { return x > 0.0f ? 1.0f : (x < 0.0f ? -1.0f : 0.0f); }
PT_DEV float f_step(float edge, float x) { return x < edge ? 0.0f : 1.0f; }

PT_DEV v3 cuboid_normal(v3 mn, v3 mx, v3 p)
{
    v3 half = v_scale(v_sub(mx, mn), 0.5f);
    v3 cs = v_sub(p, v_scale(v_add(mx, mn), 0.5f));
    v3 n;
    n.x = f_sign(cs.x) * f_step(f_abs(f_abs(cs.x) - half.x), EPSILON);
    n.y = f_sign(cs.y) * f_step(f_abs(f_abs(cs.y) - half.y), EPSILON);
    n.z = f_sign(cs.z) * f_step(f_abs(f_abs(cs.z) - half.z), EPSILON);
    return v_normalize(n);
}

PT_DEV Material load_material(const float4 *m)
{
    float4 a = m[0], b = m[1], c = m[2], d = m[3];
    Material r;
    r.albedo = V(a.x, a.y, a.z);     r.specularChance = a.w;
    r.emissiv = V(b.x, b.y, b.z);    r.specularRoughness = b.w;
    r.absorbance = V(c.x, c.y, c.z); r.refractionChance = c.w;
    r.refractionRoughness = d.x;     r.ior = d.y;
    return r;
}

#ifndef PT_WALK_ROUNDS
#define PT_WALK_ROUNDS 6
#endif

template <bool MASKED, bool MATLDS, bool GRID = false, bool SHARE = false>
PT_DEV bool ray_trace_t(const SceneLds &sc, int ns, int nc, v3 o, v3 d, Hit &h, const unsigned long long *masks, float &walkFrom PROF_PARAM)
{
    PROF_BEGIN
    float T = FLOAT_MAX, wt2 = 0.0f;
    int winner = -1;
    bool needBrute = true;
    float wf = -1.0f;
    if (GRID && !MASKED && sc.gridStarts != nullptr) {
        ColdArgs ca = cold_args();
        const v3 rel = V(o.x - ca->gridCenter[0], o.y - ca->gridCenter[1], o.z - ca->gridCenter[2]);
        const float dd = v_dot(d, d);
        needBrute = !(v_dot(rel, rel) <= ca->gridReach2 && __builtin_fabsf(dd - 1.0f) < 1e-5f);
        if (!needBrute) {
            const float ix_ = __builtin_fabsf(d.x) > 1e-18f ? __builtin_amdgcn_rcpf(d.x) : (d.x < 0.0f ? -1e18f : 1e18f);
            const float iy_ = __builtin_fabsf(d.y) > 1e-18f ? __builtin_amdgcn_rcpf(d.y) : (d.y < 0.0f ? -1e18f : 1e18f);
            const float iz_ = __builtin_fabsf(d.z) > 1e-18f ? __builtin_amdgcn_rcpf(d.z) : (d.z < 0.0f ? -1e18f : 1e18f);
            const float ax0 = (ca->gridLo[0] - o.x) * ix_, ax1 = (ca->gridHi[0] - o.x) * ix_;
            const float ay0 = (ca->gridLo[1] - o.y) * iy_, ay1 = (ca->gridHi[1] - o.y) * iy_;
            const float az0 = (ca->gridLo[2] - o.z) * iz_, az1 = (ca->gridHi[2] - o.z) * iz_;
            float tn = f_max(0.0f, f_max(f_min(ax0, ax1), f_max(f_min(ay0, ay1), f_min(az0, az1))));
            const bool resumed = walkFrom >= 0.0f;
            tn = resumed ? f_max(tn, walkFrom) : tn;
            const float tf = f_min(f_max(ax0, ax1), f_min(f_max(ay0, ay1), f_max(az0, az1)));
            if (tn <= tf) {
                const int nx = ca->gridDims[0], ny = ca->gridDims[1], nz = ca->gridDims[2];
                const v3 p = v_fma(d, tn, o);
                int cx = (int)((p.x - ca->gridLo[0]) * ca->gridInvCell[0]), cy = (int)((p.y - ca->gridLo[1]) * ca->gridInvCell[1]),
                    cz = (int)((p.z - ca->gridLo[2]) * ca->gridInvCell[2]);
                cx = cx < 0 ? 0 : (cx >= nx ? nx - 1 : cx);
                cy = cy < 0 ? 0 : (cy >= ny ? ny - 1 : cy);
                cz = cz < 0 ? 0 : (cz >= nz ? nz - 1 : cz);
                const bool px = !(d.x < 0.0f), py = !(d.y < 0.0f), pz = !(d.z < 0.0f);
                float mx = (ca->gridLo[0] + (float)(cx + (px ? 1 : 0)) * ca->gridCell[0] - o.x) * ix_;
                float my = (ca->gridLo[1] + (float)(cy + (py ? 1 : 0)) * ca->gridCell[1] - o.y) * iy_;
                float mz = (ca->gridLo[2] + (float)(cz + (pz ? 1 : 0)) * ca->gridCell[2] - o.z) * iz_;
                const float dx = __builtin_fabsf(ca->gridCell[0] * ix_), dy = __builtin_fabsf(ca->gridCell[1] * iy_),
                            dz = __builtin_fabsf(ca->gridCell[2] * iz_);
                int rx = px ? nx - 1 - cx : cx, ry = py ? ny - 1 - cy : cy, rz = pz ? nz - 1 - cz : cz;
                int cell = (cz * ny + cy) * nx + cx;
                const int sx = px ? 1 : -1, sy = py ? nx : -nx, sz = pz ? nx * ny : -(nx * ny);
                int L = -1, viol = 0;
                bool first = !resumed;
                int k = sc.gridStarts[cell], kEnd = sc.gridStarts[cell + 1];
                for (int round = 0;; round++) {
                    const bool xm = mx <= my && mx <= mz, ym = !xm && my <= mz;
                    const float texit = xm ? mx : (ym ? my : mz);
                    const bool more = (xm ? rx : (ym ? ry : rz)) > 0;
                    const int ncell = more ? cell + (xm ? sx : (ym ? sy : sz)) : cell;
                    const int nk = sc.gridStarts[ncell], nkEnd = sc.gridStarts[ncell + 1];
                    int j = sc.gridRefs[k], jn = sc.gridRefs[k + 1];
                    float4 s = sc.sph[j];
                    while (k < kEnd) {
                        const float4 sn = sc.sph[jn];
                        const int jnn = sc.gridRefs[k + 2];
                        k++;
                        const v3 oc = V(o.x - s.x, o.y - s.y, o.z - s.z);
                        const float b = v_dot(d, oc);
                        const float c = f_fma(-s.w, s.w, v_dot(oc, oc));
                        const float disc = f_fma(b, b, -c);
                        if (!(disc < 0.0f) && !(c > 0.0f && b > 1e-10f)) {
                            const float sq = pt_sqrt(disc);
                            const float t1 = -b - sq, t2 = -b + sq;
                            const bool valid = (t1 <= t2) & (t2 > 0.0f);
                            const bool inside = valid & (t1 < 0.0f);
                            const bool nearer = (t1 < T) | ((t1 == T) & (winner != L) & (j < winner));
                            const bool accOut = valid & !inside & (j > L) & nearer;
                            const bool accIn = inside & first;
                            viol |= (inside & !first) ? 1 : 0;
                            const bool acc = accIn | accOut;
                            T = acc ? (inside ? t2 : t1) : T;
                            wt2 = acc ? t2 : wt2;
                            winner = acc ? j : winner;
                            L = accIn ? j : L;
                        }
                        j = jn;
                        jn = jnn;
                        s = sn;
                    }
                    first = false;
                    if (T <= texit || !more) break;
                    if (round == PT_WALK_ROUNDS - 1) { wf = texit; break; }
                    mx = xm ? mx + dx : mx;
                    my = ym ? my + dy : my;
                    mz = (xm || ym) ? mz : mz + dz;
                    rx = xm ? rx - 1 : rx;
                    ry = ym ? ry - 1 : ry;
                    rz = (xm || ym) ? rz : rz - 1;
                    cell = ncell;
                    k = nk;
                    kEnd = nkEnd;
                }
                needBrute = viol != 0;
            }
        }
        if (needBrute) { T = FLOAT_MAX; wt2 = 0.0f; winner = -1; wf = -1.0f; }
    }
    auto candidate = [&](int i, float b, float c, float disc) {
        if (!(disc < 0.0f) && !(c > 0.0f && b > 1e-10f)) {
            float sq = pt_sqrt(disc);
            float t1 = -b - sq, t2 = -b + sq;
            if (t1 <= t2 && t2 > 0.0f && t1 < T) {
                T = t1 < 0.0f ? t2 : t1;
                wt2 = t2;
                winner = i;
            }
        }
    };
    int i = 0;
    if (MASKED) {
#pragma unroll
        for (int w = 0; w < 4; w++) {
            if (w * 64 >= ns) break;
            unsigned long long mk = masks[w];
            while (mk != 0ull) {
                int k = w * 64 + (int)__builtin_ctzll(mk);
// ... 241 lines not shown

PT_DEV unsigned long long cone_cuboid_mask(const SceneLds &sc, int nc, v3 O, float rho, float ct, const v3 dirs[4], float lensSin)
{
    const int lane = threadIdx.x & 63;
    const bool usable = ct > 0.05f;
    const bool in = lane < nc;
    const float4 mn = sc.cmin[in ? lane : 0], mx = sc.cmax[in ? lane : 0];
    const float scale = 1.0f + f_max(f_max(f_abs(O.x), f_max(f_abs(O.y), f_abs(O.z))),
                                     f_max(f_max(f_abs(mn.x), f_max(f_abs(mn.y), f_abs(mn.z))), f_max(f_abs(mx.x), f_max(f_abs(mx.y), f_abs(mx.z)))));
    const float pad = f_fma(scale, 2e-3f, rho * 1.01f);
    const float q = f_fma(lensSin, 1.01f, 1e-3f);
    bool outside = false;
    const int order[5] = {0, 1, 3, 2, 0};
#pragma unroll
    for (int e = 0; e < 4; e++) {
        const v3 a = dirs[order[e]], b = dirs[order[e + 1]];
        v3 n = V(a.y * b.z - a.z * b.y, a.z * b.x - a.x * b.z, a.x * b.y - a.y * b.x);
        const v3 mid = V(dirs[0].x + dirs[1].x + dirs[2].x + dirs[3].x, dirs[0].y + dirs[1].y + dirs[2].y + dirs[3].y, dirs[0].z + dirs[1].z + dirs[2].z + dirs[3].z);
        const float il = __builtin_amdgcn_rsqf(f_fma(n.z, n.z, f_fma(n.y, n.y, n.x * n.x)));
        const float sgn = (n.x * mid.x + n.y * mid.y + n.z * mid.z) < 0.0f ? -il : il;
        n = V(n.x * sgn, n.y * sgn, n.z * sgn);
        bool allOut = true;
#pragma unroll
        for (int v = 0; v < 8; v++) {
            const v3 p = V(((v & 1) ? mx.x : mn.x) - O.x, ((v & 2) ? mx.y : mn.y) - O.y, ((v & 4) ? mx.z : mn.z) - O.z);
            const float len = __builtin_amdgcn_sqrtf(f_fma(p.z, p.z, f_fma(p.y, p.y, p.x * p.x)));
            const float g = f_fma(n.x, p.x, f_fma(n.y, p.y, n.z * p.z)) + f_fma(len + rho, q, pad);
            allOut = allOut && (g < 0.0f);
        }
        outside = outside || allOut;
    }
    const unsigned long long keep = __ballot(in && !(usable && outside));
    return keep;
}

PT_DEV void hemisphere_draws(uint32_t &seed, float &z, float &a)
{
    z = f_fma(rand01(seed), 2.0f, -1.0f);
    a = rand01(seed) * 2.0f * PI;
}
PT_DEV v3 hemisphere_direction(v3 n, float z, float a)
{
    float r = pt_sqrt(f_fma(-z, z, 1.0f));
    float sn, cs;
    pt_sincos(a, sn, cs);
    return v_normalize(v_add(n, V(r * cs, r * sn, z)));
}
PT_DEV v3 cosine_sample_hemisphere(v3 n, uint32_t &seed)
{
    float z, a;
    hemisphere_draws(seed, z, a);
    return hemisphere_direction(n, z, a);
}

PT_DEV float fresnel_schlick(float cosTheta, float n1, float n2)
{
    float r0 = (n1 - n2) * f_rcp(n1 + n2);
    r0 *= r0;
    return f_fma(1.0f - r0, pt_pow5(1.0f - cosTheta), r0);
}

PT_DEV v3 f_reflect(v3 i, v3 n) { return v_fma(n, -(2.0f * v_dot(n, i)), i); }

PT_DEV v3 f_refract(v3 i, v3 n, float eta)
{
    float ni = v_dot(n, i);
    float k = f_fma(-(eta * eta), f_fma(-ni, ni, 1.0f), 1.0f);
    if (k < 0.0f) return V(0.0f, 0.0f, 0.0f);
    float f = f_fma(eta, ni, pt_sqrt(k));
    return V(f_fma(eta, i.x, -(f * n.x)), f_fma(eta, i.y, -(f * n.y)), f_fma(eta, i.z, -(f * n.z)));
}

PT_DEV float bsdf(v3 &ro, v3 &rd, const Hit &h, bool &isRefractive, uint32_t &seed)
{
    isRefractive = false;
    float spec = h.m.specularChance, refr = h.m.refractionChance;
    if (spec > 0.0f) {
        float n1 = h.fromInside ? h.m.ior : 1.0f, n2 = !h.fromInside ? h.m.ior : 1.0f;
        spec = f_mix(spec, 1.0f, fresnel_schlick(v_dot(v_neg(rd), h.normal), n1, n2));
        float diffuse = 1.0f - spec - refr;
        refr = 1.0f - spec - diffuse;
    }
    float hz, ha;
    hemisphere_draws(seed, hz, ha);
    float prob;
    float roll = rand01(seed);
    const bool specular = spec > roll;
    const bool refractive = !specular && spec + refr > roll;
    v3 hn = h.normal;
    if (refractive) {
        hemisphere_draws(seed, hz, ha);
        hn = v_neg(h.normal);
    }
    const v3 hemi = hemisphere_direction(hn, hz, ha);
    v3 raw = hemi;
    bool lobe = false;
    if (specular) {
        v3 refl = f_reflect(rd, h.normal);
        raw = v_mix(refl, hemi, h.m.specularRoughness * h.m.specularRoughness);
        prob = spec;
        lobe = true;
    } else if (refractive) {
        v3 rf = f_refract(rd, h.normal, h.fromInside ? h.m.ior : f_rcp(h.m.ior));
        raw = v_mix(rf, hemi, h.m.refractionRoughness * h.m.refractionRoughness);
        prob = refr;
        isRefractive = true;
        lobe = true;
    } else {
        prob = 1.0f - spec - refr;
    }
    rd = lobe ? v_normalize(raw) : raw;
    ro = v_fma(rd, EPSILON, h.nearHitPos);
    return f_max(prob, EPSILON);
}

template <bool MASKED, bool MATLDS, bool GRID = false, bool SHARE = false>
PT_DEV bool bounce_step_t(const SceneLds &sc, int ns, int nc, const EnvRef &env, v3 &ro, v3 &rd, v3 &throughput, v3 &rad,
                          uint32_t &seed, const unsigned long long *masks, float &walkFrom PROF_PARAM)
{
    Hit h;
    const bool hit = ray_trace_t<MASKED, MATLDS, GRID, SHARE>(sc, ns, nc, ro, rd, h, masks, walkFrom PROF_PASS);
    if constexpr (GRID) {
        if (walkFrom >= 0.0f) return true;
    }
    if (hit) {
        PROF_BEGIN
        if (h.fromInside) {
            h.normal = v_neg(h.normal);
            throughput.x *= pt_exp<SHARE>(-h.m.absorbance.x * h.T);
            throughput.y *= pt_exp<SHARE>(-h.m.absorbance.y * h.T);
            throughput.z *= pt_exp<SHARE>(-h.m.absorbance.z * h.T);
        }
        PROF_MARK(4)
        bool isRefractive;
        float prob = bsdf(ro, rd, h, isRefractive, seed);
        PROF_MARK(5)
#ifdef PT_PROFILE
        prof[8] += 1ull;
        prof[9] += __ballot(isRefractive) != 0ull ? 1ull : 0ull;
#endif
        rad = V(f_fma(h.m.emissiv.x, throughput.x, rad.x), f_fma(h.m.emissiv.y, throughput.y, rad.y),
                f_fma(h.m.emissiv.z, throughput.z, rad.z));
        if (!isRefractive) throughput = v_mul(throughput, h.m.albedo);
        throughput = v_scale(throughput, f_rcp(prob));
        float p = f_max(throughput.x, f_max(throughput.y, throughput.z));
        if (rand01(seed) > p) return false;
        throughput = v_scale(throughput, f_rcp(p));
        return true;
    }
    PROF_BEGIN
    v3 e;
    if (env.data == nullptr) {
        ColdArgs ca = cold_args();
        EnvRef cold{ca->env, env.lut, ca->envSize, ca->envFormat};
        e = sample_env(cold, rd);
    } else {
        e = sample_env(env, rd);
    }
    rad = V(f_fma(e.x, throughput.x, rad.x), f_fma(e.y, throughput.y, rad.y), f_fma(e.z, throughput.z, rad.z));
    PROF_MARK(6)
    return false;
}
PT_DEV bool bounce_step(const SceneLds &sc, int ns, int nc, const EnvRef &env, v3 &ro, v3 &rd, v3 &throughput, v3 &rad,
                        uint32_t &seed PROF_PARAM)
{
    float fresh = -1.0f;
    return bounce_step_t<false, true>(sc, ns, nc, env, ro, rd, throughput, rad, seed, nullptr, fresh PROF_PASS);
}

PT_DEV v3 radiance(const FrameArgs &a, const SceneLds &sc, const EnvRef &env, v3 ro, v3 rd, uint32_t &seed)
{
#ifdef PT_PROFILE
    unsigned long long prof_dummy[10] = {0, 0, 0, 0, 0, 0, 0, 0, 0, 0};
#endif
    v3 throughput = V(1.0f, 1.0f, 1.0f), rad = V(0.0f, 0.0f, 0.0f);
    for (int i = 0; i < a.rayDepth; i++)
        if (!bounce_step(sc, a.numSpheres, a.numCuboids, env, ro, rd, throughput, rad, seed PROF_DUMMY)) break;
    return rad;
}

template <typename FP>
PT_DEV void mat_vec(FP m, float x, float y, float z, float w, float *out)
{
#pragma unroll
    for (int r = 0; r < 4; r++) out[r] = f_fma(m[12 + r], w, f_fma(m[8 + r], z, f_fma(m[4 + r], y, m[r] * x)));
}

template <typename FP>
PT_DEV void primary_ray_cam(FP cam, float invW, float invH, int px, int py, uint32_t &seed, v3 &ro, v3 &rd)
{
    FP invProj = cam, invView = cam + 16;
    v3 viewPos = V(cam[32], cam[33], cam[34]);
    float u0 = rand01(seed), u1 = rand01(seed);
    float ndcx = f_fma(((float)px + u0) * invW, 2.0f, -1.0f);
    float ndcy = f_fma(((float)py + u1) * invH, 2.0f, -1.0f);
    float eye[4], wd[4];
    mat_vec(invProj, ndcx, ndcy, -1.0f, 0.0f, eye);
    mat_vec(invView, eye[0], eye[1], -1.0f, 0.0f, wd);
    v3 dir = v_normalize(V(wd[0], wd[1], wd[2]));
    v3 focal = v_fma(dir, cam[35], viewPos);
    float angle = rand01(seed) * 2.0f * PI;
    float rr = pt_sqrt(rand01(seed));
    float sn, cs;
    pt_sincos(angle, sn, cs);
    float half_ap = cam[36] * 0.5f;
    float ox = half_ap * (cs * rr), oy = half_ap * (sn * rr);
    float org[4];
    mat_vec(invView, ox, oy, 0.0f, 1.0f, org);
    ro = V(org[0], org[1], org[2]);
    rd = v_normalize(v_sub(focal, ro));
}

PT_DEV void primary_ray(const FrameArgs &a, int px, int py, uint32_t &seed, v3 &ro, v3 &rd)
{
    primary_ray_cam<const float *>(a.invProj, a.invW, a.invH, px, py, seed, ro, rd);
}

PT_DEV int global_row_v(int bandRows, int bandWorld, int bandRank, int localRow0, int y0, int ly)
{
    if (bandRows == 0) return y0 + ly;
    int l = localRow0 + ly;
    int band = l / bandRows;
    return (band * bandWorld + bandRank) * bandRows + (l - band * bandRows);
}
PT_DEV int global_row(const FrameArgs &a, int ly) { return global_row_v(a.bandRows, a.bandWorld, a.bandRank, a.localRow0, a.y0, ly); }

PT_DEV uint32_t pixel_seed(int px, int py, int frame)
{
    return ((uint32_t)px * 1973u + (uint32_t)py * 9277u + (uint32_t)frame * 2699u) | 1u;
}

PT_DEV float4 resolve_pixel(const FrameArgs &a, v3 irr, float4 last)
{
    irr = v_scale(irr, f_div_ieee(1.0f, (float)a.spp));
    float w = f_div_ieee(1.0f, (float)(a.frame + 1));
    return make_float4(f_mix(last.x, irr.x, w), f_mix(last.y, irr.y, w), f_mix(last.z, irr.z, w), 1.0f);
}

PT_DEV float4 shade_pixel(const FrameArgs &a, const SceneLds &sc, const EnvRef &env, int px, int py, float4 last)
{
    uint32_t seed = pixel_seed(px, py, a.frame);
    v3 irr = V(0.0f, 0.0f, 0.0f);
    for (int s = 0; s < a.spp; s++) {
        v3 ro, rd;
        primary_ray(a, px, py, seed, ro, rd);
        irr = v_add(irr, radiance(a, sc, env, ro, rd, seed));
    }
    return resolve_pixel(a, irr, last);
}

}
```

### opentk-pathtracer_amd/csrc/pt_first_hit.hip

```cpp
#include "pt_kernel_common.hpp"

namespace pt {

__global__ __launch_bounds__(256) void pt_first_hit_kernel(const FrameArgs a, float4 *records, const int pickTile)
{
    SceneLds sc = stage_scene(a);
    const int tid = threadIdx.x;
    const int ns = a.numSpheres, nc = a.numCuboids;
    float4 *ids = g_lds + scene_lds_bytes(ns, nc, 0, false) / sizeof(float4);
    for (int i = tid; i < ns + nc; i += 256) ids[4 * i] = make_float4((float)(i < ns ? i : kFirstHitCuboidBase + (i - ns)), 0.0f, 0.0f, 0.0f);
    __syncthreads();
    sc.mat = ids;
    const int b = xcd_band_id(blockIdx.x, gridDim.x);
    const int wave = tid >> 6, lane = tid & 63;
    const int tile = pickTile >= 0 ? pickTile : b * 4 + wave;
    if (tile >= a.tilesX * a.tilesY || (pickTile >= 0 && wave != 0)) return;
    const int tx = tile % a.tilesX, ty = tile / a.tilesX;
    const int px = tx * 8 + (lane & 7);
    const int ly = ty * 8 + (lane >> 3);
    if (px >= a.width || ly >= a.rows) return;
#ifdef PT_PROFILE
    unsigned long long prof_dummy[10] = {0, 0, 0, 0, 0, 0, 0, 0, 0, 0};
#endif
    uint32_t seed = pixel_seed(px, global_row(a, ly), a.frame);
    v3 ro, rd;
    primary_ray(a, px, global_row(a, ly), seed, ro, rd);
    Hit h;
    const bool hit = ray_trace(sc, ns, nc, ro, rd, h PROF_DUMMY);
    const float t = hit ? h.T : __builtin_inff();
    const int id = hit ? (int)h.m.albedo.x : -1;
    const size_t at = pickTile >= 0 ? (size_t)lane : (size_t)ly * a.width + px;
    records[2 * at] = make_float4(ro.x, ro.y, ro.z, t);
    records[2 * at + 1] = make_float4(rd.x, rd.y, rd.z, __int_as_float(id));
}

hipError_t launch_first_hit(const FrameArgs &args, float4 *records, int pickTile, hipStream_t stream)
{
    FrameArgs a = args;
    a.materialsInLds = 0;
    a.gridLdsBytes = 0;
    a.envFormat = 0;
    if (a.tilesX < 1 || a.tilesY < 1 || pickTile >= a.tilesX * a.tilesY) return hipErrorInvalidValue;
    const int tiles = a.tilesX * a.tilesY;
    const size_t lds = scene_lds_bytes(a.numSpheres, a.numCuboids, 0, false) + (size_t)(a.numSpheres + a.numCuboids) * 4 * sizeof(float4);
    hipLaunchKernelGGL(pt_first_hit_kernel, dim3(pickTile >= 0 ? 1 : (tiles + 3) / 4), dim3(256), lds, stream, a, records, pickTile);
    return hipGetLastError();
}

}
```

### opentk-pathtracer_amd/csrc/pt_helper_kernels.hip

```cpp
#include "pt_atmosphere.hpp"
#include "pt_device.hpp"
#include "pt_kernels.hpp"
#include "pt_math.hpp"

namespace pt {

__global__ void pt_clear_kernel(float4 *p, size_t n)
{
    size_t i = (size_t)blockIdx.x * blockDim.x + threadIdx.x;
    size_t stride = (size_t)gridDim.x * blockDim.x;
    for (; i < n; i += stride) p[i] = make_float4(0.0f, 0.0f, 0.0f, 0.0f);
}

hipError_t launch_clear(float4 *p, size_t n, hipStream_t stream)
{
    if (n == 0) return hipSuccess;
    size_t blocks = (n + 255) / 256;
    if (blocks > 2048) blocks = 2048;
    hipLaunchKernelGGL(pt_clear_kernel, dim3((unsigned)blocks), dim3(256), 0, stream, p, n);
    return hipGetLastError();
}

__global__ void pt_set_alpha_kernel(float4 *p, size_t n)
{
    size_t i = (size_t)blockIdx.x * blockDim.x + threadIdx.x;
    size_t stride = (size_t)gridDim.x * blockDim.x;
    for (; i < n; i += stride) p[i].w = 1.0f;
}

hipError_t launch_set_alpha(float4 *p, size_t n, hipStream_t stream)
{
    if (n == 0) return hipSuccess;
    size_t blocks = (n + 255) / 256;
    if (blocks > 2048) blocks = 2048;
    hipLaunchKernelGGL(pt_set_alpha_kernel, dim3((unsigned)blocks), dim3(256), 0, stream, p, n);
    return hipGetLastError();
}

template <typename T>
__global__ __launch_bounds__(256) void pt_assemble_bands_kernel(const AssembleArgs a)
{
    const size_t n = (size_t)a.width * a.height;
    size_t i = (size_t)blockIdx.x * 256 + threadIdx.x;
    const size_t stride = (size_t)gridDim.x * 256;
    for (; i < n; i += stride) {
        const int y = (int)(i / a.width), x = (int)(i - (size_t)y * a.width);
        const int band = y / a.bandRows, g = band % a.world, lb = band / a.world;
        const size_t ly = (size_t)lb * a.bandRows + (size_t)(y - band * a.bandRows);
        ((T *)a.out)[i] = ((const T *)a.stage)[a.partOffset[g] + ly * a.width + x];
    }
}

hipError_t launch_assemble_bands(const AssembleArgs &a, hipStream_t stream)
{
    const size_t n = (size_t)a.width * a.height;
    if (n == 0) return hipSuccess;
    size_t blocks = (n + 255) / 256;
    if (blocks > 8192) blocks = 8192;
    if (a.bytesPerPixel == 16) hipLaunchKernelGGL(pt_assemble_bands_kernel<float4>, dim3((unsigned)blocks), dim3(256), 0, stream, a);
    else hipLaunchKernelGGL(pt_assemble_bands_kernel<uchar4>, dim3((unsigned)blocks), dim3(256), 0, stream, a);
    return hipGetLastError();
}

__global__ void pt_env_to_float_kernel(const void *env, int size, int format, const float *lut, float4 *out)
{
    size_t n = (size_t)6 * size * size;
    size_t i = (size_t)blockIdx.x * blockDim.x + threadIdx.x;
    if (i >= n) return;
    if (format == 0) {
        out[i] = ((const float4 *)env)[i];
    } else {
        uchar4 t = ((const uchar4 *)env)[i];
        out[i] = make_float4(lut[t.x], lut[t.y], lut[t.z], (float)t.w / 255.0f);
    }
}

hipError_t launch_env_to_float(const void *env, int envSize, int envFormat, const float *srgbLut, float4 *out,
                               hipStream_t stream)
{
    size_t n = (size_t)6 * envSize * envSize;
    hipLaunchKernelGGL(pt_env_to_float_kernel, dim3((unsigned)((n + 255) / 256)), dim3(256), 0, stream, env, envSize,
                       envFormat, srgbLut, out);
    return hipGetLastError();
}

__global__ __launch_bounds__(256) void pt_postprocess_kernel(const float4 *accum, uchar4 *out, size_t n)
{
    __builtin_amdgcn_s_setprio(3);
    size_t i = (size_t)blockIdx.x * 256 + threadIdx.x;
    size_t stride = (size_t)gridDim.x * 256;
    for (; i < n; i += stride) {
        float4 c = accum[i];
        uchar4 o;
        o.x = to_unorm8(linear_to_inverse_gamma(aces_film(c.x), 2.4f));
        o.y = to_unorm8(linear_to_inverse_gamma(aces_film(c.y), 2.4f));
        o.z = to_unorm8(linear_to_inverse_gamma(aces_film(c.z), 2.4f));
        o.w = 255;
        out[i] = o;
    }
}

hipError_t launch_postprocess(const float4 *accum, void *outRgba8, size_t n, hipStream_t stream)
{
    if (n == 0) return hipSuccess;
    size_t blocks = (n + 255) / 256;
    if (blocks > 4096) blocks = 4096;
    hipLaunchKernelGGL(pt_postprocess_kernel, dim3((unsigned)blocks), dim3(256), 0, stream, accum, (uchar4 *)outRgba8, n);
    return hipGetLastError();
}

PT_DEV v3 atmo_texel_direction(const AtmoArgs &a, int face, int x, int y)
{
    const int S = a.size;
    float ndcx = f_fma((float)x / (float)S, 2.0f, -1.0f), ndcy = f_fma((float)y / (float)S, 2.0f, -1.0f);
    float eye[4], wd[4];
    mat_vec(a.invProj, ndcx, ndcy, -1.0f, 0.0f, eye);
    mat_vec(a.invView[face], eye[0], eye[1], -1.0f, 0.0f, wd);
    return v_normalize(V(wd[0], wd[1], wd[2]));
}

__host__ __device__ inline int atmo_half_columns(int S) { return S / 2 + 1; }
__host__ __device__ inline int atmo_row_lanes(int S) { return S + 1 + 4 * atmo_half_columns(S); }

__global__ __launch_bounds__(256) void atmo_precompute_kernel(const AtmoArgs a)
{
    const int S = a.size, C = atmo_half_columns(S), T = atmo_row_lanes(S);
    const size_t i = (size_t)blockIdx.x * 256 + threadIdx.x;
    if (i >= (size_t)S * T) return;
    const int y = (int)(i / T);
    int r = (int)(i % T), face, x;
    if (r < S) { face = 0; x = r; }
    else if (r == S) { face = 1; x = 0; }
    else { r -= S + 1; face = 2 + r / C; x = r % C; }
    const v3 dir = atmo_texel_direction(a, face, x, y);
    const v3 r0 = V(0.0f, 6376e3f, 0.0f), sun = V(a.lightPos[0], a.lightPos[1], a.lightPos[2]), kRlh = V(5.5e-6f, 13.0e-6f, 22.4e-6f);
    const v3 col = atmosphere(dir, r0, sun, a.lightIntensity, 6371e3f, 6471e3f, kRlh, 21e-6f, 8e3f, 1.2e3f, 0.758f, a.iSteps, a.jSteps);
    a.out[((size_t)face * S + y) * S + x] = make_float4(col.x, col.y, col.z, 1.0f);
    const int mface = face < 2 ? 1 - face : face, mx = S - x;
    if (x < 1 || (mface == face && mx == x)) return;
    const v3 pdir = atmo_texel_direction(a, mface, mx, y);
    v3 pcol = col;
    if (!(a.lightPos[0] == 0.0f && pdir.x == -dir.x && pdir.y == dir.y && pdir.z == dir.z))
        pcol = atmosphere(pdir, r0, sun, a.lightIntensity, 6371e3f, 6471e3f, kRlh, 21e-6f, 8e3f, 1.2e3f, 0.758f, a.iSteps, a.jSteps);
    a.out[((size_t)mface * S + y) * S + mx] = make_float4(pcol.x, pcol.y, pcol.z, 1.0f);
}

hipError_t launch_atmosphere(const AtmoArgs &a, hipStream_t stream)
{
    const size_t n = (size_t)a.size * atmo_row_lanes(a.size);
    hipLaunchKernelGGL(atmo_precompute_kernel, dim3((unsigned)((n + 255) / 256)), dim3(256), 0, stream, a);
    return hipGetLastError();
}

}
```

### opentk-pathtracer_amd/csrc/pt_integrate_multisample.hip

```cpp
#include "pt_kernel_common.hpp"

namespace pt {

template <bool MATLDS, bool GRID = false>
__global__ __launch_bounds__(256, 5) void pt_integrate_multisample_kernel(const FrameArgs a)
{
    __shared__ __attribute__((aligned(16))) BlockQueue queue;
    constexpr int NWAVES = 4;
    const int numTilesFrame = a.tilesX * a.tilesY;
    const int numTiles = numTilesFrame * a.batchFrames;
    if (threadIdx.x == 0) {
        long long first = (long long)blockIdx.x * a.queueChunk;
        long long last = first + a.queueChunk < numTiles ? first + a.queueChunk : numTiles;
        if (first >= numTiles || a.tagged) { first = 0; last = 0; }
        queue.pair = ((unsigned long long)last << 32) | (unsigned long long)first;
        queue.lock = 0u;
        queue.done = 0u;
        if (a.startedFlags)
            __hip_atomic_store(a.startedFlags + blockIdx.x, a.launchSeq, __ATOMIC_RELAXED, __HIP_MEMORY_SCOPE_SYSTEM);
    }
    CHAOS(1);
    SceneLds sc = stage_scene(a);
    EnvRef env{nullptr, (LdsFloats)sc.lut, 0, 0};
    const int tid = threadIdx.x, wave = tid >> 6, lane = tid & 63;
    char *ringBase = (char *)g_lds + scene_lds_bytes(a.numSpheres, a.numCuboids, a.envFormat, a.materialsInLds != 0, a.gridLdsBytes);
    PathEntryM *ring = (PathEntryM *)ringBase + wave * 64;
    const int CONT_BATCH_MIN = a.contBatchMin;
    const int parkCapacity = a.contCapacity;
    ContEntry *cq = (ContEntry *)(ringBase + NWAVES * 64 * (int)sizeof(PathEntryM)) + wave * parkCapacity;
#ifndef PT_MS_IRR_LDS
#define PT_MS_IRR_LDS 0
#endif
#ifndef PT_MS_EARLY
#define PT_MS_EARLY 40
#endif
    constexpr bool IRR_LDS = !MATLDS && PT_MS_IRR_LDS != 0;
    [[maybe_unused]] float *const laneIrr = (float *)(ringBase + NWAVES * 64 * (int)sizeof(PathEntryM) + NWAVES * parkCapacity * (int)sizeof(ContEntry)) + wave * 4 * 64 + lane;
    v3 irrReg = V(0, 0, 0);
    auto get_irr = [&]() -> v3 {
        if constexpr (IRR_LDS) return V(laneIrr[0], laneIrr[64], laneIrr[128]);
        else return irrReg;
    };
    auto set_irr = [&](v3 v) -> void {
        if constexpr (IRR_LDS) { laneIrr[0] = v.x; laneIrr[64] = v.y; laneIrr[128] = v.z; }
        else irrReg = v;
    };
    auto pixel_xy = [&](int p) -> int {
        ColdArgs ca = cold_args();
        const int ly = p >> 16, x = p & 0xffff;
        return x | (global_row_v(ca->bandRows, ca->bandWorld, ca->bandRank, ca->localRow0, ca->y0, ly) << 16);
    };

    int avail = 0, parked = 0, qhead = 0;
    HandoverBound bound;
    bound.init();
    unsigned int stallSince = 0u;
    auto qslot = [&](int i) -> int {
        int sl = qhead + i;
        return sl >= parkCapacity ? sl - parkCapacity : sl;
    };
    bool exhausted = false;
    int pixReg = -1, counters = IRR_LDS ? -1 : 0;
    auto lane_idle = [&]() -> bool {
        if constexpr (IRR_LDS) return counters < 0;
        else return pixReg < 0;
    };
    auto set_idle = [&]() -> void {
        if constexpr (IRR_LDS) counters = -1;
        else pixReg = -1;
    };
    auto get_pix = [&]() -> int {
        if constexpr (IRR_LDS) return __builtin_bit_cast(int, laneIrr[192]);
        else return pixReg;
    };
    auto set_pix = [&](int p) -> void {
        if constexpr (IRR_LDS) laneIrr[192] = __builtin_bit_cast(float, p);
        else pixReg = p;
    };
    auto c_bounce = [&]() -> int { return counters & 0xfff; };
    auto c_sample = [&]() -> int { return (counters >> 12) & 0xfff; };
    auto c_fj = [&]() -> int { return (counters >> 24) & 0x7f; };
    bool needRay = false, pending = false;
    float walkFrom = -1.0f;
#ifdef PT_PROFILE
    unsigned long long prof_dummy[10] = {0, 0, 0, 0, 0, 0, 0, 0, 0, 0};
#endif
    uint32_t seed = 0;
    v3 ro = V(0, 0, 0), rd = V(0, 0, 1), throughput = V(1, 1, 1), rad = V(0, 0, 0);

    auto fold = [&](float4 last, v3 rirr, int rfj) -> float4 {
        ColdArgs ca = cold_args();
        rirr = v_scale(rirr, f_div_ieee(1.0f, (float)ca->spp));
        const float w = f_div_ieee(1.0f, (float)(ca->frame + rfj + 1));
        const float alpha = (rfj == ca->batchFrames - 1 && !ca->keepTags) ? 1.0f : frame_tag(ca->frame + rfj);
        return make_float4(f_mix(last.x, rirr.x, w), f_mix(last.y, rirr.y, w), f_mix(last.z, rirr.z, w), alpha);
    };
    auto try_resolve = [&](int rpix, int rfj, v3 rirr) -> bool {
        const size_t pidx = (size_t)((rpix >> 16) * cold_args()->width + (rpix & 0xffff));
        float4 *ptr = a.accum + pidx;
        if (!a.tagged) {
            const float4 last = *ptr, next = fold(last, rirr, 0);
            AUDIT_RESOLVE(a, pidx, a.frame, last, next, 5);
            *ptr = next;
            if (float4 *snap = cold_args()->snapshot) snap[pidx] = next;
            return true;
        }
        CHAOS(20);
        float4 last = load_pixel_sc1(ptr);
        const float expected = rfj > 0 ? frame_tag(a.frame + rfj - 1) : a.chainTag;
        if (expected != 0.0f && last.w != expected) return false;
        if (AUDIT_SABOTAGED(a, rpix, rfj)) last.x += 1.0f;
        CHAOS(21);
        const float4 next = fold(last, rirr, rfj);
        AUDIT_RESOLVE(a, pidx, a.frame + rfj, last, next, 6);
        store_pixel_sc1(ptr, next);
        if (rfj == cold_args()->batchFrames - 1)
            if (float4 *snap = cold_args()->snapshot) snap[pidx] = make_float4(next.x, next.y, next.z, 1.0f);
        CHAOS(22);
        return true;
    };

    auto rescue = [&]() -> void {
        const int room = parkCapacity - parked;
        if (room > 0) {
            if (lane < room) {
                ContEntry e;
                e.pix = get_pix(); e.seed = seed; e.sfj = c_sample() | (c_fj() << 16);
                const v3 irr = get_irr();
                e.irr[0] = irr.x; e.irr[1] = irr.y; e.irr[2] = irr.z;
                cq[qslot(parked + lane)] = e;
                set_idle();
                pending = false;
            }
            parked += room < 64 ? room : 64;
        }
        __builtin_amdgcn_wave_barrier();
    };

    for (;;) {
        bool idle = lane_idle();
        unsigned long long m = __ballot(idle);
        bool forcePass = parked > 0 && avail < 64 && __ballot(!(!lane_idle() && pending && !needRay)) == 0ull;
        if constexpr (GRID && PT_MS_EARLY > 0) forcePass = forcePass || (parked + PT_MS_EARLY >= parkCapacity && avail <= 64 - PT_MS_EARLY && parked > 0);
        for (int pass = 0; pass < 16 && (m != 0ull || forcePass); pass++) {
            if (avail == 0 || forcePass) {
                const bool fromQueue = forcePass || parked >= CONT_BATCH_MIN || (exhausted && parked > 0);
                forcePass = false;
                const int base = avail;
                int tile = -1;
                if (!fromQueue) {
                    if (exhausted) break;
                    tile = queue_pop_tile(&queue);
                    if (tile < 0) {
                        exhausted = true;
                        continue;
                    }
                    if (unsigned int *flags = cold_args()->tileFlags)
                        if (tile < numTilesFrame && lane == 0) flags[tile] = cold_args()->launchSeq;
                }
                ColdArgs ca = cold_args();
                ColdFloats cam = (ColdFloats)ca;
                const int width = ca->width;
                const float invW = ca->invW, invH = ca->invH;
                bool valid = false;
                int tpix = 0, tpxy = 0, tsample = 0, tfj = 0;
                uint32_t tseed = 0;
                v3 tirr = V(0.0f, 0.0f, 0.0f);
                if (fromQueue) {
                    const int n = parked < 64 - base ? parked : 64 - base;
                    valid = lane < n;
                    if (valid) {
                        const ContEntry e = cq[qslot(lane)];
                        tpix = e.pix; tpxy = pixel_xy(e.pix); tseed = e.seed;
                        tsample = e.sfj & 0xffff; tfj = e.sfj >> 16;
                        tirr = V(e.irr[0], e.irr[1], e.irr[2]);
                    }
                    qhead = qslot(n);
                    parked -= n;
                    __builtin_amdgcn_wave_barrier();
                } else {
                    const int tilesX = ca->tilesX;
                    int tx, ty;
                    fast_divmod(tile, numTilesFrame, ca->tilesFrameMagic, tfj, tile);
                    fast_divmod(tile, tilesX, ca->tilesXMagic, ty, tx);
                    const int x = tx * 8 + (lane & 7), ly = ty * 8 + (lane >> 3);
                    valid = x < width && ly < ca->rows;
                    if (valid) {
                        const int gy = global_row_v(ca->bandRows, ca->bandWorld, ca->bandRank, ca->localRow0, ca->y0, ly);
                        tpix = x | (ly << 16);
                        tpxy = x | (gy << 16);
                        tseed = pixel_seed(x, gy, ca->frame + tfj);
                    }
                }
                const bool twaiting = valid && tsample >= a.spp;
                valid = valid && !twaiting;
                v3 to = V(0.0f, 0.0f, 0.0f), td = V(0.0f, 0.0f, 1.0f), tthr = V(1.0f, 1.0f, 1.0f), trad = V(0.0f, 0.0f, 0.0f);
                if (valid) primary_ray_cam(cam, invW, invH, tpxy & 0xffff, tpxy >> 16, tseed, to, td);
                unsigned long long masks[5];
                if (!fromQueue && ca->tileMasks != nullptr) {
                    const __attribute__((address_space(4))) unsigned long long *tm =
                        (const __attribute__((address_space(4))) unsigned long long *)ca->tileMasks + (size_t)tile * kTileMaskWords;
                    masks[0] = tm[0]; masks[1] = tm[1]; masks[2] = tm[2]; masks[3] = tm[3]; masks[4] = tm[4];
                } else if (fromQueue && ca->tileMasks != nullptr) {
                    masks[0] = masks[1] = masks[2] = masks[3] = masks[4] = 0ull;
                    const int myTile = ((tpix >> 16) >> 3) * ca->tilesX + ((tpix & 0xffff) >> 3);
                    unsigned long long rem = __ballot(valid);
                    int distinct = 0;
                    while (rem != 0ull && distinct < 8) {
                        const int t = __builtin_amdgcn_readlane(myTile, (int)__builtin_ctzll(rem));
                        const __attribute__((address_space(4))) unsigned long long *tm =
                            (const __attribute__((address_space(4))) unsigned long long *)ca->tileMasks + (size_t)t * kTileMaskWords;
                        masks[0] |= tm[0]; masks[1] |= tm[1]; masks[2] |= tm[2]; masks[3] |= tm[3]; masks[4] |= tm[4];
                        rem &= ~__ballot(valid && myTile == t);
                        distinct++;
                    }
                    if (rem != 0ull) cull_spheres(sc, a.numSpheres, valid, to, td, masks);
                } else {
                    cull_spheres(sc, a.numSpheres, valid, to, td, masks);
                }
                bool tcont = false;
                float walkFresh = -1.0f;
                if (valid) {
                    if (0 < a.rayDepth) tcont = bounce_step_t<true, MATLDS>(sc, a.numSpheres, a.numCuboids, env, to, td, tthr, trad, tseed, masks, walkFresh PROF_DUMMY);
                    if (1 >= a.rayDepth) tcont = false;
                }
                const unsigned long long cm = __ballot(tcont);
                if (tcont) {
                    const int slot = base + __builtin_amdgcn_mbcnt_hi((unsigned)(cm >> 32), __builtin_amdgcn_mbcnt_lo((unsigned)cm, 0u));
                    PathEntryM e;
                    e.pix = tpix; e.counters = 1 | (tsample << 12) | (tfj << 24); e.seed = tseed;
                    e.ro[0] = to.x; e.ro[1] = to.y; e.ro[2] = to.z;
                    e.rd[0] = td.x; e.rd[1] = td.y; e.rd[2] = td.z;
                    e.thr[0] = tthr.x; e.thr[1] = tthr.y; e.thr[2] = tthr.z;
                    e.rad[0] = trad.x; e.rad[1] = trad.y; e.rad[2] = trad.z;
                    e.irr[0] = tirr.x; e.irr[1] = tirr.y; e.irr[2] = tirr.z;
                    ring[slot] = e;
                }
                avail = base + __builtin_popcountll(cm);
// ... 152 lines not shown
```

### opentk-pathtracer_amd/csrc/pt_integrate_persistent.hip

```cpp
#include <cstdio>

#include "pt_kernel_common.hpp"
#include "pt_tuning.hpp"

namespace pt {

__global__ __launch_bounds__(256) void pt_integrate_kernel(const FrameArgs a)
{
    SceneLds sc = stage_scene(a);
    EnvRef env{a.env, (LdsFloats)sc.lut, a.envSize, a.envFormat};
    const int tid = threadIdx.x;
    const int b = xcd_band_id(blockIdx.x, gridDim.x);
    const int wave = tid >> 6, lane = tid & 63;
    const int tile = b * 4 + wave;
    if (tile >= a.tilesX * a.tilesY) return;
    const int tx = tile % a.tilesX, ty = tile / a.tilesX;
    const int px = tx * 8 + (lane & 7);
    const int ly = ty * 8 + (lane >> 3);
    if (px >= a.width || ly >= a.rows) return;
    const size_t idx = (size_t)ly * a.width + px;
    float4 last = a.accum[idx];
    const float4 next = shade_pixel(a, sc, env, px, global_row(a, ly), last);
    AUDIT_RESOLVE(a, idx, a.frame, last, next, 1);
    a.accum[idx] = next;
}

__global__ __launch_bounds__(256) void pt_repair_kernel(const FrameArgs a, unsigned int *ctl)
{
    if (*(const volatile unsigned int *)a.abandonWord > a.launchSeq) return;
    SceneLds sc = stage_scene(a);
    EnvRef env{a.env, (LdsFloats)sc.lut, a.envSize, a.envFormat};
    const int tid = threadIdx.x, wave = tid >> 6, lane = tid & 63;
    const int tiles = a.tilesX * a.tilesY, n = a.batchFrames;
#ifdef PT_PROFILE
    unsigned long long prof_dummy[10] = {0, 0, 0, 0, 0, 0, 0, 0, 0, 0};
#endif
    for (int tile = (int)blockIdx.x * 4 + wave; tile < tiles; tile += (int)gridDim.x * 4) {
        const int tx = tile % a.tilesX, ty = tile / a.tilesX;
        const int px = tx * 8 + (lane & 7), ly = ty * 8 + (lane >> 3);
        if (px >= a.width || ly >= a.rows) continue;
        const int gy = global_row(a, ly);
        const size_t idx = (size_t)ly * a.width + px;
        float4 last = a.accum[idx];
        int done = 0, odd = 0;
        if (last.w >= FRAME_TAG) {
            const int rel = ((int)last.w - (int)FRAME_TAG - a.frame) & kFrameTagMask;
            if (rel < n) done = rel + 1;
            else if (rel <= kFrameTagMask / 2) done = n;
            else if (last.w != a.chainTag) odd = 1;
        } else if (last.w == 1.0f) {
            done = (a.chainTag != 0.0f || (a.tileFlags && a.tileFlags[tile] == a.launchSeq)) ? n : 0;
        } else if (a.chainTag != 0.0f) {
            odd = 1;
        }
        for (int j = done; j < n; j++) {
            uint32_t seed = pixel_seed(px, gy, a.frame + j);
            v3 irr = V(0.0f, 0.0f, 0.0f);
            for (int sidx = 0; sidx < a.spp; sidx++) {
                v3 ro, rd;
                primary_ray(a, px, gy, seed, ro, rd);
                irr = v_add(irr, radiance(a, sc, env, ro, rd, seed));
            }
            irr = v_scale(irr, f_div_ieee(1.0f, (float)a.spp));
            const float w = f_div_ieee(1.0f, (float)(a.frame + j + 1));
            const float alpha = (j == n - 1 && !a.keepTags) ? 1.0f : frame_tag(a.frame + j);
            const float4 next = make_float4(f_mix(last.x, irr.x, w), f_mix(last.y, irr.y, w), f_mix(last.z, irr.z, w), alpha);
            AUDIT_RESOLVE(a, idx, a.frame + j, last, next, 8);
            last = next;
        }
        if (done < n) {
            a.accum[idx] = last;
            if (a.snapshot) a.snapshot[idx] = make_float4(last.x, last.y, last.z, 1.0f);
            atomicAdd(ctl, (unsigned int)(n - done));
        }
        if (odd) atomicAdd(ctl + 1, 1u);
    }
}

__global__ void pt_repair_done_kernel(unsigned int *abandonWord, unsigned int *queueMain, unsigned int expectMain, unsigned int *queueChain,
                                      unsigned int expectChain, unsigned int *ctl)
{
    if (*abandonWord == ABANDON_NONE) return;
    *abandonWord = ABANDON_NONE;
    *queueMain = expectMain;
    *queueChain = expectChain;
    ctl[2] += 1u;
}

hipError_t launch_repair(const FrameArgs &args, unsigned int *ctl, hipStream_t stream)
{
    FrameArgs a = args;
    a.materialsInLds = 1;
    a.gridLdsBytes = 0;
    a.tileMasks = nullptr;
    a.timeline = nullptr;
    const int tiles = a.tilesX * a.tilesY;
    if (tiles <= 0 || a.abandonWord == nullptr) return hipSuccess;
    int nwg = 2 * a.numCUs;
    if (nwg > (tiles + 3) / 4) nwg = (tiles + 3) / 4;
    const size_t lds = scene_lds_bytes(a.numSpheres, a.numCuboids, a.envFormat, true);
    hipLaunchKernelGGL(pt_repair_kernel, dim3(nwg), dim3(256), lds, stream, a, ctl);
    return hipGetLastError();
}

hipError_t launch_repair_done(unsigned int *abandonWord, unsigned int *queueMain, unsigned int expectMain, unsigned int *queueChain,
                              unsigned int expectChain, unsigned int *ctl, hipStream_t stream)
{
    hipLaunchKernelGGL(pt_repair_done_kernel, dim3(1), dim3(1), 0, stream, abandonWord, queueMain, expectMain, queueChain, expectChain, ctl);
    return hipGetLastError();
}

__global__ __launch_bounds__(256) void pt_integrate_pool_kernel(const FrameArgs a, const int poolTiles)
{
    SceneLds sc = stage_scene(a);
    EnvRef env{a.env, (LdsFloats)sc.lut, a.envSize, a.envFormat};
    const int tid = threadIdx.x;
    const int b = xcd_band_id(blockIdx.x, gridDim.x);
    const int wave = tid >> 6;
    const int numTiles = a.tilesX * a.tilesY;
    const int pool = b * 4 + wave;
    int next = pool * poolTiles * 64;
    int tileEnd = (pool + 1) * poolTiles;
    const int poolEnd = (tileEnd < numTiles ? tileEnd : numTiles) * 64;
    if (next >= poolEnd) return;

#ifdef PT_PROFILE
    unsigned long long prof_dummy[10] = {0, 0, 0, 0, 0, 0, 0, 0, 0, 0};
#endif
    int pix = -1;
    int px = 0, py = 0, sample = 0, bounce = 0;
    bool needRay = false;
    uint32_t seed = 0;
    v3 ro = V(0, 0, 0), rd = V(0, 0, 1), throughput = V(1, 1, 1), rad = V(0, 0, 0), irr = V(0, 0, 0);

    for (;;) {
        bool idle = pix < 0;
        unsigned long long m = __ballot(idle);
        if (m != 0ull && next < poolEnd) {
            int rank = __builtin_amdgcn_mbcnt_hi((unsigned)(m >> 32), __builtin_amdgcn_mbcnt_lo((unsigned)m, 0u));
            int cand = next + rank;
            if (idle && cand < poolEnd) {
                int tile = cand >> 6, q = cand & 63;
                int tx = tile % a.tilesX, ty = tile / a.tilesX;
                int x = tx * 8 + (q & 7), ly = ty * 8 + (q >> 3);
                if (x < a.width && ly < a.rows) {
                    px = x;
                    py = global_row(a, ly);
                    pix = ly * a.width + x;
                    seed = pixel_seed(px, py, a.frame);
                    sample = 0;
                    irr = V(0.0f, 0.0f, 0.0f);
                    needRay = true;
                }
            }
            next += __builtin_popcountll(m);
        }
        bool active = pix >= 0;
        if (!__any(active)) {
            if (next >= poolEnd) break;
            continue;
        }
        if (active && needRay) {
            primary_ray(a, px, py, seed, ro, rd);
            throughput = V(1.0f, 1.0f, 1.0f);
            rad = V(0.0f, 0.0f, 0.0f);
            bounce = 0;
            needRay = false;
        }
        if (active) {
            bool cont = false;
            if (bounce < a.rayDepth) cont = bounce_step(sc, a.numSpheres, a.numCuboids, env, ro, rd, throughput, rad, seed PROF_DUMMY);
            bounce++;
            if (!cont || bounce >= a.rayDepth) {
                irr = v_add(irr, rad);
                sample++;
                if (sample < a.spp) {
                    needRay = true;
                } else {
                    float4 last = a.accum[pix];
                    const float4 next = resolve_pixel(a, irr, last);
                    AUDIT_RESOLVE(a, (size_t)pix, a.frame, last, next, 2);
                    a.accum[pix] = next;
                    pix = -1;
                }
            }
        }
    }
}

struct PathState {
    int pix, pxy, counters;
    uint32_t seed;
    float ro[3], rd[3], thr[3], rad[3], irr[3];
    int pad;
};
constexpr int DONATE_MAX = 32;

__host__ __device__ constexpr int pool_slots(int waves) { return (waves - 1) * DONATE_MAX; }

struct DrainControl {
    unsigned int pushed;
    unsigned int taken;
    unsigned int alive;
    unsigned int pushing;
    unsigned int lock;
    unsigned int pad[3];
};

template <int NWAVES, int MIN_WAVES_PER_SIMD, bool TIMELINE, bool SPP1, bool MATLDS, bool GRID = false, bool CARRY = false, bool COMPACT = true, bool FEED = false>
__global__ __launch_bounds__(NWAVES * 64, MIN_WAVES_PER_SIMD) void pt_integrate_persistent_kernel(const FrameArgs a)
{
    static_assert(!(CARRY && COMPACT), "the carrying kernels are only launched without drain compaction");
    static_assert(!FEED || (SPP1 && !COMPACT && !TIMELINE), "frame-fed launches: spp = 1, no drain compaction");
    __shared__ __attribute__((aligned(16))) BlockQueue queue;
    __shared__ __attribute__((aligned(16))) DrainControl drain;
    __shared__ __attribute__((aligned(16))) FeedQueue feedq;
    __shared__ unsigned int wgDone[8];
    __shared__ unsigned int waveDone[FEED ? NWAVES * 8 : 1];
    const int numTilesFrame = a.tilesX * a.tilesY;
    const int numTiles = numTilesFrame * a.batchFrames;
    auto frame_weights = [&]() -> float2 * { return (float2 *)((char *)g_lds + cold_args()->sceneLdsBytes); };
    if (SPP1) {
        float2 *fw = frame_weights();
        for (int j = (int)threadIdx.x; j < a.batchFrames; j += (int)blockDim.x)
            fw[j] = make_float2(f_div_ieee(1.0f, (float)(a.frame + j + 1)), (j == a.batchFrames - 1 && !a.keepTags) ? 1.0f : frame_tag(a.frame + j));
    }
    if (threadIdx.x == 0) {
        long long first = (long long)blockIdx.x * a.queueChunk;
        long long last = first + a.queueChunk < numTiles ? first + a.queueChunk : numTiles;
        if (first >= numTiles || a.tagged) { first = 0; last = 0; }
        queue.pair = ((unsigned long long)last << 32) | (unsigned long long)first;
        queue.lock = 0u;
        queue.done = 0u;
        drain.pushed = 0u;
        drain.taken = 0u;
        drain.alive = (unsigned int)NWAVES;
        drain.pushing = 0u;
        drain.lock = 0u;
        if constexpr (FEED) {
            feedq.stash = 0ull;
            feedq.limit = 0u;
            feedq.word = 0u;
            feedq.pollAt = 0u;
        }
        if (a.startedFlags)
            __hip_atomic_store(a.startedFlags + blockIdx.x, a.launchSeq, __ATOMIC_RELAXED, __HIP_MEMORY_SCOPE_SYSTEM);
#ifdef PT_AUDIT
        if (a.tagged && a.audit && a.auditLog && blockIdx.x == 0) {
            const unsigned int c = __hip_atomic_load((const unsigned int *)a.queue, __ATOMIC_RELAXED, __HIP_MEMORY_SCOPE_AGENT);
            if ((unsigned int)(c - a.queueBase) > (unsigned int)numTiles + 65536u) {
                const unsigned int slot = atomicAdd(a.auditLog, 1u);
                if (slot < (unsigned int)kAuditLogRecords) {
                    unsigned int *r = a.auditLog + 4 + slot * kAuditRecordWords;
                    r[0] = 91u; r[1] = c; r[2] = a.queueBase; r[3] = 0u; r[4] = 0u; r[5] = 0u; r[6] = 0u; r[7] = a.launchSeq;
                    r[8] = (unsigned int)a.frame | ((unsigned int)a.batchFrames << 24); r[9] = __float_as_uint(a.chainTag); r[10] = 0u;
                    r[11] = (unsigned int)a.tagged | ((unsigned int)a.keepTags << 1) | ((unsigned int)a.variant << 8);
                }
            }
        }
#endif
    }
    if constexpr (FEED) {
        if (threadIdx.x < 8) wgDone[threadIdx.x] = 0u;
        if (threadIdx.x < NWAVES * 8) waveDone[threadIdx.x] = 0u;
    }
    CHAOS(1);
    SceneLds sc = stage_scene(a);
    EnvRef env{nullptr, (LdsFloats)sc.lut, 0, 0};
    const int tid = threadIdx.x, wave = tid >> 6, lane = tid & 63;
    [[maybe_unused]] unsigned int *const myDone = waveDone + (FEED ? wave * 8 : 0);
    [[maybe_unused]] auto count_resolved = [&](int rfj) -> void {
        if constexpr (FEED) atomicAdd(myDone + (rfj & 7), 1u);
    };
    [[maybe_unused]] auto release_resolved = [&]() -> void {
        if constexpr (FEED) {
            asm volatile("s_waitcnt vmcnt(0)" ::: "memory");
            if (lane < 8) {
                const unsigned int v = lds_load(myDone + lane);
                if (v != 0u) {
                    lds_store(myDone + lane, 0u);
                    atomicAdd(wgDone + lane, v);
                }
            }
        }
    };
    [[maybe_unused]] auto flush_resolved = [&]() -> void {
        if constexpr (FEED) {
            if (lane < 8) {
                const unsigned int v = atomicExch(wgDone + lane, 0u);
                if (v != 0u) __hip_atomic_fetch_add(cold_args()->feedDone + lane * kFeedDoneStride, (unsigned long long)v, __ATOMIC_RELAXED, __HIP_MEMORY_SCOPE_AGENT);
            }
        }
    };
    [[maybe_unused]] auto display_slot_before = [&](int rfj) -> unsigned int {
        if constexpr (FEED) {
            if (rfj == 0) return (unsigned int)cold_args()->displayPrev;
            return (lds_load(&feedq.word) >> (2 * ((rfj - 1) & 7))) & 3u;
        } else {
            return 0u;
        }
    };
    [[maybe_unused]] auto display_pixel = [&](unsigned int slot, int rpix, float r, float g, float b) -> void {
        if constexpr (FEED) {
            ColdArgs ca = cold_args();
            uchar4 *img = slot == 1u ? ca->displayImages[0] : (slot == 2u ? ca->displayImages[1] : ca->displayImages[2]);
            uchar4 o;
            o.x = to_unorm8(linear_to_inverse_gamma(aces_film(r), 2.4f));
            o.y = to_unorm8(linear_to_inverse_gamma(aces_film(g), 2.4f));
            o.z = to_unorm8(linear_to_inverse_gamma(aces_film(b), 2.4f));
            o.w = 255;
            unsigned int packed;
            __builtin_memcpy(&packed, &o, 4);
            asm volatile("global_store_dword %0, %1, off sc1\n\ts_nop 0" : : "v"(img + rpix), "v"(packed) : "memory");
        }
    };
    [[maybe_unused]] auto store_snapshot = [&](int rpix, int rfj, float4 next) -> void {
        if constexpr (!FEED) {
            if (float4 *snap = cold_args()->snapshot)
                if (rfj == cold_args()->batchFrames - 1) snap[rpix] = make_float4(next.x, next.y, next.z, 1.0f);
        }
    };

    static_assert(!CARRY || SPP1, "the pixel travels with the path in the tile-pass kernels only");
    using PathRec = typename std::conditional<CARRY, PathEntryCarry, PathEntry>::type;
    constexpr int ENTRY_BYTES = SPP1 ? (int)sizeof(PathRec) : (int)sizeof(RingEntry);
    char *ringBase = (char *)g_lds + scene_lds_bytes(a.numSpheres, a.numCuboids, a.envFormat, a.materialsInLds != 0, a.gridLdsBytes) +
                     (SPP1 ? frame_weight_bytes(a.batchFrames) : 0);
    RingEntry *ring = (RingEntry *)(ringBase + wave * 64 * ENTRY_BYTES);
    PathRec *pring = (PathRec *)(ringBase + wave * 64 * ENTRY_BYTES);
    constexpr int LANE_LAST_BYTES = CARRY ? NWAVES * 3 * 64 * 4 : 0;
    float *laneLast = (float *)(ringBase + NWAVES * 64 * ENTRY_BYTES) + wave * 3 * 64 + lane;
    PathState *pool = (PathState *)(ringBase + NWAVES * 64 * ENTRY_BYTES + LANE_LAST_BYTES);
    const bool compaction = COMPACT && a.drainCompaction != 0;
    ParkedResolve *parkedList = (ParkedResolve *)(ringBase + NWAVES * 64 * ENTRY_BYTES + LANE_LAST_BYTES) + wave * a.parkedMax;
    const bool parking = SPP1 && a.tagged && !compaction && a.parkedMax > 0;
    int nparked = 0;
    bool parkProgress = false;
    unsigned int parkSince = 0u;
    HandoverBound bound;
    bound.init();
    const int donateMax = a.drainCompaction < DONATE_MAX ? a.drainCompaction : DONATE_MAX;
    const bool leader = lane == 0;

    if constexpr (FEED) {
        if (blockIdx.x == 0 && wave == NWAVES - 1) {
            ColdArgs ca = cold_args();
            unsigned int j = 0;
            unsigned int seen = 0u;
            for (;;) {
                unsigned int w = __hip_atomic_load(ca->feedHost, __ATOMIC_RELAXED, __HIP_MEMORY_SCOPE_SYSTEM);
                w = (unsigned int)__builtin_amdgcn_readfirstlane((int)w);
                if (w != seen) {
#ifdef PT_FEED_TIMES
                    if (lane == 0 && a.startedFlags) __hip_atomic_store(a.startedFlags + 3100 + (feed_count(w) & 63), (unsigned int)wall_clock64(), __ATOMIC_RELAXED, __HIP_MEMORY_SCOPE_SYSTEM);
#endif
                    for (int s4 = lane; s4 < kFeedBcastSlots; s4 += 64)
                        __hip_atomic_store(ca->feedBcast + s4 * kFeedBcastStride, w, __ATOMIC_RELAXED, __HIP_MEMORY_SCOPE_AGENT);
                    seen = w;
                }
                while (j < (unsigned int)ca->batchFrames) {
                    const unsigned long long need = ca->feedBase[j & 7] + ca->feedPixels * (unsigned long long)(j / 8 + 1);
                    const unsigned long long have = __hip_atomic_load(ca->feedDone + (j & 7) * kFeedDoneStride, __ATOMIC_RELAXED, __HIP_MEMORY_SCOPE_AGENT);
                    if (!__builtin_amdgcn_readfirstlane((int)(have >= need))) break;
                    j++;
                    if (lane == 0) __hip_atomic_store(ca->feedHostDone, j, __ATOMIC_RELAXED, __HIP_MEMORY_SCOPE_SYSTEM);
#ifdef PT_FEED_TIMES
                    if (lane == 0 && a.startedFlags) __hip_atomic_store(a.startedFlags + 3000 + (j & 63), (unsigned int)wall_clock64(), __ATOMIC_RELAXED, __HIP_MEMORY_SCOPE_SYSTEM);
#endif
                }
                if (((w & kFeedClosed) && j >= feed_count(w)) || j >= (unsigned int)ca->batchFrames) break;
                if (launch_abandoned()) break;
                __builtin_amdgcn_s_sleep(8);
            }
            return;
        }
    }
    int avail = 0;
    bool exhausted = false;
    bool lastAlive = false;
#ifdef PT_PROFILE
    unsigned long long prof[10] = {0, 0, 0, 0, 0, 0, 0, 0, 0, 0}, prof_dummy[10] = {0, 0, 0, 0, 0, 0, 0, 0, 0, 0}, prof_util[3] = {0, 0, 0};
    unsigned long long prof_t = __builtin_readcyclecounter();
#endif
    unsigned long long tStart = 0, tExhausted = 0, nIter = 0;
    if (TIMELINE) tStart = wall_clock64();

    int pix = -1, px = 0, py = 0, sample = 0, bounce = 0;
    bool needRay = false;
    uint32_t seed = 0;
    v3 ro = V(0, 0, 0), rd = V(0, 0, 1), throughput = V(1, 1, 1), rad = V(0, 0, 0), irr = V(0, 0, 0);
    int fj = 0;
    bool pending = false;
    float walkFrom = -1.0f, walkFresh = -1.0f;
    auto begin_path = [&]() -> void { pending = false; walkFrom = -1.0f; };

    auto fold = [&](float4 last, v3 rirr, int rfj) -> float4 {
        float w, alpha;
        if constexpr (SPP1) {
            const float2 wa = frame_weights()[rfj];
            w = wa.x;
            alpha = wa.y;
        } else {
            ColdArgs ca = cold_args();
            rirr = v_scale(rirr, f_div_ieee(1.0f, (float)ca->spp));
            w = f_div_ieee(1.0f, (float)(ca->frame + rfj + 1));
            alpha = (rfj == ca->batchFrames - 1 && !ca->keepTags) ? 1.0f : frame_tag(ca->frame + rfj);
        }
        return make_float4(f_mix(last.x, rirr.x, w), f_mix(last.y, rirr.y, w), f_mix(last.z, rirr.z, w), alpha);
    };
    [[maybe_unused]] auto commit_resolve = [&](int rpix, int rfj, v3 rirr, v3 rlast) -> void {
        const float4 last = make_float4(rlast.x, rlast.y, rlast.z, 0.0f);
        const float4 next = fold(last, rirr, rfj);
        AUDIT_RESOLVE(a, (size_t)rpix, a.frame + rfj, last, next, 7);
        if (!a.tagged) a.accum[rpix] = next;
        else store_pixel_sc1(a.accum + rpix, next);
        store_snapshot(rpix, rfj, next);
        count_resolved(rfj);
    };
    auto try_resolve = [&](int rpix, int rfj, v3 rirr) -> bool {
        float4 *ptr = a.accum + rpix;
        if (!a.tagged) {
            float4 last = *ptr;
            const float4 next = fold(last, rirr, 0);
            AUDIT_RESOLVE(a, (size_t)rpix, a.frame, last, next, 3);
            *ptr = next;
            if (float4 *snap = cold_args()->snapshot) snap[rpix] = next;
            return true;
        }
        CHAOS(10);
        float4 last = load_pixel_sc1(ptr);
        const float expected = rfj > 0 ? frame_tag(a.frame + rfj - 1) : a.chainTag;
        if (expected != 0.0f && last.w != expected) return false;
        if constexpr (FEED) {
            if (cold_args()->displayOn != 0) {
                const unsigned int dslot = (rfj == 0) ? (unsigned int)cold_args()->displayPrev : ((lds_load(&feedq.word) >> (2 * ((rfj - 1) & 7))) & 3u);
                if (dslot != 0u) display_pixel(dslot, rpix, last.x, last.y, last.z);
            }
        }
        if (AUDIT_SABOTAGED(a, rpix, rfj)) last.x += 1.0f;
        CHAOS(11);
        const float4 next = fold(last, rirr, rfj);
        AUDIT_RESOLVE(a, (size_t)rpix, a.frame + rfj, last, next, 4);
        store_pixel_sc1(ptr, next);
        store_snapshot(rpix, rfj, next);
        count_resolved(rfj);
        CHAOS(12);
        return true;
    };

    auto park_resolves = [&](bool want, int rpix, int rfj, v3 rirr) -> bool {
        const unsigned long long wm = __ballot(want);
        if (wm == 0ull) return false;
        const int rank = __builtin_amdgcn_mbcnt_hi((unsigned)(wm >> 32), __builtin_amdgcn_mbcnt_lo((unsigned)wm, 0u));
        const int room = a.parkedMax - nparked;
        const bool fits = want && rank < room;
        if (fits) {
            ParkedResolve e;
            e.pix = rpix; e.fj = rfj; e.irr[0] = rirr.x; e.irr[1] = rirr.y; e.irr[2] = rirr.z;
            parkedList[nparked + rank] = e;
        }
        const int n = __builtin_popcountll(wm);
        nparked += n < room ? n : room;
        __builtin_amdgcn_wave_barrier();
        return fits;
    };
    auto service_parked = [&]() -> void {
        parkProgress = false;
        if (nparked == 0) return;
        CHAOS(4);
        const bool mine = lane < nparked;
        ParkedResolve e = {0, 0, {0.0f, 0.0f, 0.0f}};
        bool keep = false;
        if (mine) {
            e = parkedList[lane];
            keep = !try_resolve(e.pix, e.fj, V(e.irr[0], e.irr[1], e.irr[2]));
        }
        const unsigned long long km = __ballot(keep);
        __builtin_amdgcn_wave_barrier();
        if (keep) parkedList[__builtin_amdgcn_mbcnt_hi((unsigned)(km >> 32), __builtin_amdgcn_mbcnt_lo((unsigned)km, 0u))] = e;
        const int left = __builtin_popcountll(km);
        parkProgress = left < nparked;
        nparked = left;
        __builtin_amdgcn_wave_barrier();
    };

    [[maybe_unused]] bool starved = false;
    [[maybe_unused]] unsigned int idlePolls = 0u;
    [[maybe_unused]] unsigned int lastLimit = 0u;
    [[maybe_unused]] unsigned int idleSince = 0u;
    for (;;) {
        bool idle = pix < 0;
        unsigned long long m = __ballot(idle);
        if constexpr (FEED) starved = false;
        for (int pass = 0; (SPP1 ? pass < 16 : pass < 2) && m != 0ull; pass++) {
            if (avail == 0) {
                if (exhausted) break;
                    int tile;
                    if constexpr (FEED) {
                        tile = queue_pop_tile_feed(&queue, &feedq);
                        if (tile < 0) release_resolved();
                        if ((tile & 7) == 0 || tile < 0) flush_resolved();
                        if (tile == QUEUE_NOT_YET) {
                            starved = true;
                            break;
                        }
                        idleSince = 0u;
                    } else {
                        tile = queue_pop_tile(&queue);
                    }
                    if (tile < 0) {
                        exhausted = true;
                        if (TIMELINE) tExhausted = wall_clock64();
                    } else if constexpr (SPP1) {
#ifdef PT_PROFILE
                        const unsigned long long prof_tile0 = __builtin_readcyclecounter();
#endif
                        ColdArgs ca = cold_args();
                        ColdFloats cam = (ColdFloats)ca;
                        const int width = ca->width, tilesX = ca->tilesX;
                        const float invW = ca->invW, invH = ca->invH;
                        int tfj, tx, ty;
                        fast_divmod(tile, numTilesFrame, ca->tilesFrameMagic, tfj, tile);
                        fast_divmod(tile, tilesX, ca->tilesXMagic, ty, tx);
                        int x = tx * 8 + (lane & 7), ly = ty * 8 + (lane >> 3);
                        const bool valid = x < width && ly < ca->rows;
                        v3 to = V(0.0f, 0.0f, 0.0f), td = V(0.0f, 0.0f, 1.0f), tthr = V(1.0f, 1.0f, 1.0f), trad = V(0.0f, 0.0f, 0.0f);
                        uint32_t tseed = 0;
                        int tpix = 0;
                        if (valid) {
                            int gy = global_row_v(ca->bandRows, ca->bandWorld, ca->bandRank, ca->localRow0, ca->y0, ly);
                            tseed = pixel_seed(x, gy, ca->frame + tfj);
                            primary_ray_cam(cam, invW, invH, x, gy, tseed, to, td);
                            tpix = ly * width + x;
                        }
                        unsigned long long masks[5];
                        if (const unsigned long long *cached = ca->tileMasks) {
                            const __attribute__((address_space(4))) unsigned long long *tm =
                                (const __attribute__((address_space(4))) unsigned long long *)cached + (size_t)tile * kTileMaskWords;
                            masks[0] = tm[0]; masks[1] = tm[1]; masks[2] = tm[2]; masks[3] = tm[3]; masks[4] = tm[4];
                        } else {
                            cull_spheres(sc, a.numSpheres, valid, to, td, masks);
                        }
                        if (unsigned int *flags = ca->tileFlags)
                            if (tfj == 0 && lane == 0) flags[tile] = ca->launchSeq;
                        bool tcont = false, tkeep = false;
                        [[maybe_unused]] bool plastOk = false;
                        [[maybe_unused]] float4 plast = make_float4(0.0f, 0.0f, 0.0f, 0.0f);
                        if (valid) {
                            if (0 < a.rayDepth)
                                tcont = bounce_step_t<true, MATLDS>(sc, a.numSpheres, a.numCuboids, env, to, td, tthr, trad, tseed, masks, walkFresh PROF_DUMMY);
                            if (1 >= a.rayDepth) tcont = false;
                            tkeep = tcont;
                            if constexpr (CARRY) {
                                plast = a.accum[tpix];
                                const float expected = tfj > 0 ? frame_tag(a.frame + tfj - 1) : a.chainTag;
                                plastOk = !a.tagged || expected == 0.0f || plast.w == expected;
                                if constexpr (FEED) {
                                    release_resolved();
                                    if (cold_args()->displayOn != 0) {
                                        const unsigned int dslot = display_slot_before(tfj);
                                        if (dslot != 0u && plastOk) display_pixel(dslot, tpix, plast.x, plast.y, plast.z);
                                    }
                                }
                            }
                            if (CARRY && !tcont && plastOk) {
                                commit_resolve(tpix, tfj, v_add(V(0.0f, 0.0f, 0.0f), trad), V(plast.x, plast.y, plast.z));
                            } else if (!tcont) {
                                v3 tirr = v_add(V(0.0f, 0.0f, 0.0f), trad);
                                tkeep = !try_resolve(tpix, tfj, tirr);
                            }
                        }
                        if (parking) {
                            const bool twait = valid && !tcont && tkeep;
                            if (park_resolves(twait, tpix, tfj, v_add(V(0.0f, 0.0f, 0.0f), trad))) tkeep = false;
                        }
                        const unsigned long long cm = __ballot(tkeep);
                        if (tkeep) {
                            int slot = __builtin_amdgcn_mbcnt_hi((unsigned)(cm >> 32), __builtin_amdgcn_mbcnt_lo((unsigned)cm, 0u));
                            PathRec e;
                            e.pix = tpix; e.bounce = (tcont ? 1 : a.rayDepth) | (tfj << 16); e.seed = tseed;
                            e.ro[0] = to.x; e.ro[1] = to.y; e.ro[2] = to.z;
                            e.rd[0] = td.x; e.rd[1] = td.y; e.rd[2] = td.z;
                            e.thr[0] = tthr.x; e.thr[1] = tthr.y; e.thr[2] = tthr.z;
                            if constexpr (CARRY) {
                                const bool radZero = (__float_as_uint(trad.x) | __float_as_uint(trad.y) | __float_as_uint(trad.z)) == 0u;
                                const bool carryLast = plastOk && radZero;
                                if (carryLast) e.bounce |= PATH_HAS_LAST;
                                e.x[0] = carryLast ? plast.x : trad.x; e.x[1] = carryLast ? plast.y : trad.y; e.x[2] = carryLast ? plast.z : trad.z;
                            } else {
                                e.rad[0] = trad.x; e.rad[1] = trad.y; e.rad[2] = trad.z;
                            }
                            pring[slot] = e;
                        }
                        __builtin_amdgcn_wave_barrier();
                        avail = __builtin_popcountll(cm);
                        if constexpr (!CARRY) release_resolved();
#ifdef PT_PROFILE
                        {
                            const unsigned long long d_ = __builtin_readcyclecounter() - prof_tile0;
                            prof[6] += d_;
                            prof_t += d_;
                        }
#endif
                    } else {
                        ColdArgs ca = cold_args();
                        ColdFloats cam = (ColdFloats)ca;
                        const int width = ca->width, tilesX = ca->tilesX;
                        const float invW = ca->invW, invH = ca->invH;
                        int tfj, tx, ty;
                        fast_divmod(tile, numTilesFrame, ca->tilesFrameMagic, tfj, tile);
                        if (unsigned int *flags = ca->tileFlags)
                            if (tfj == 0 && lane == 0) flags[tile] = ca->launchSeq;
                        fast_divmod(tile, tilesX, ca->tilesXMagic, ty, tx);
                        int x = tx * 8 + (lane & 7), ly = ty * 8 + (lane >> 3);
                        RingEntry e;
                        e.pix = -1;
                        e.pxy = 0; e.seed = 0; e.ox = e.oy = e.oz = e.dx = e.dy = e.dz = 0.0f; e.pad = tfj;
                        if (x < width && ly < ca->rows) {
                            int gy = global_row_v(ca->bandRows, ca->bandWorld, ca->bandRank, ca->localRow0, ca->y0, ly);
                            uint32_t sd = pixel_seed(x, gy, ca->frame + tfj);
                            v3 o, d;
                            primary_ray_cam(cam, invW, invH, x, gy, sd, o, d);
                            e.pix = ly * width + x;
                            e.pxy = x | (gy << 16);
                            e.seed = sd;
                            e.ox = o.x; e.oy = o.y; e.oz = o.z; e.dx = d.x; e.dy = d.y; e.dz = d.z;
                        }
                        ring[lane] = e;
                        __builtin_amdgcn_wave_barrier();
                        avail = 64;
                    }

                if (exhausted) break;
                if (SPP1 && avail == 0) continue;
            }
            CHAOS(3);
            if constexpr (SPP1) {
                int rank = __builtin_amdgcn_mbcnt_hi((unsigned)(m >> 32), __builtin_amdgcn_mbcnt_lo((unsigned)m, 0u));
                if (idle && rank < avail) {
                    PathRec e = pring[avail - 1 - rank];
                    pix = e.pix;
                    bounce = e.bounce & 0xffff;
                    fj = (e.bounce >> 16) & 0x3fff;
                    if constexpr (CARRY) {
                        if (e.bounce & PATH_HAS_LAST) fj |= 0x4000;
                        laneLast[0] = e.x[0]; laneLast[64] = e.x[1]; laneLast[128] = e.x[2];
                    }
                    pending = false;
                    walkFrom = -1.0f;
                    seed = e.seed;
                    ro = V(e.ro[0], e.ro[1], e.ro[2]);
                    rd = V(e.rd[0], e.rd[1], e.rd[2]);
                    throughput = V(e.thr[0], e.thr[1], e.thr[2]);
                    if constexpr (CARRY) {
                        const bool hasLast = (e.bounce & PATH_HAS_LAST) != 0;
                        rad = V(hasLast ? 0.0f : e.x[0], hasLast ? 0.0f : e.x[1], hasLast ? 0.0f : e.x[2]);
                    } else {
                        rad = V(e.rad[0], e.rad[1], e.rad[2]);
                    }
                }
                int n = __builtin_popcountll(m);
                avail = n < avail ? avail - n : 0;
            } else {
                int rank = __builtin_amdgcn_mbcnt_hi((unsigned)(m >> 32), __builtin_amdgcn_mbcnt_lo((unsigned)m, 0u));
                if (idle && rank < avail) {
                    RingEntry e = ring[avail - 1 - rank];
                    if (e.pix >= 0) {
                        pix = e.pix;
                        px = e.pxy & 0xffff;
                        py = e.pxy >> 16;
                        seed = e.seed;
                        ro = V(e.ox, e.oy, e.oz);
                        rd = V(e.dx, e.dy, e.dz);
                        throughput = V(1.0f, 1.0f, 1.0f);
                        rad = V(0.0f, 0.0f, 0.0f);
                        irr = V(0.0f, 0.0f, 0.0f);
                        sample = 0;
                        fj = e.pad;
                        begin_path();
                        bounce = 0;
                        needRay = false;
                    }
                }
                int n = __builtin_popcountll(m);
                avail = n < avail ? avail - n : 0;
            }
            idle = pix < 0;
            m = __ballot(idle);
        }
        if (m != 0ull) {
            if (avail > 0) {
            } else if (exhausted && compaction) {
                unsigned int pushed = lds_load(&drain.pushed), taken = lds_load(&drain.taken);
                pushed = (unsigned int)__builtin_amdgcn_readfirstlane((int)pushed);
                taken = (unsigned int)__builtin_amdgcn_readfirstlane((int)taken);
                if (pushed > taken) {
                    unsigned int want = (unsigned int)__builtin_popcountll(m), have = pushed - taken;
                    unsigned int k = want < have ? want : have;
                    unsigned int got = ~0u;
                    if (leader) got = atomicCAS(&drain.taken, taken, taken + k);
                    got = (unsigned int)__builtin_amdgcn_readfirstlane((int)got);
                    if (got == taken) {
                        int rank = __builtin_amdgcn_mbcnt_hi((unsigned)(m >> 32), __builtin_amdgcn_mbcnt_lo((unsigned)m, 0u));
                        if (idle && (unsigned int)rank < k) {
                            PathState st = pool[taken + rank];
                            pix = st.pix;
                            bounce = (st.counters >> 12) & 0xfff;
                            begin_path();
                            pending = (st.counters >> 25) & 1;
                            fj = (st.counters >> 26) & 0x3f;
                            if constexpr (CARRY) {
                                if (st.counters & 1) fj |= 0x4000;
                                laneLast[0] = st.irr[0]; laneLast[64] = st.irr[1]; laneLast[128] = st.irr[2];
                            }
                            seed = st.seed;
                            ro = V(st.ro[0], st.ro[1], st.ro[2]);
                            rd = V(st.rd[0], st.rd[1], st.rd[2]);
                            throughput = V(st.thr[0], st.thr[1], st.thr[2]);
                            rad = V(st.rad[0], st.rad[1], st.rad[2]);
                            if constexpr (!SPP1) {
                                px = st.pxy & 0xffff;
                                py = st.pxy >> 16;
                                sample = st.counters & 0xfff;
                                needRay = (st.counters >> 24) & 1;
                                irr = V(st.irr[0], st.irr[1], st.irr[2]);
                            }
                        }
                    }
                }
            }
        }
        bool active = pix >= 0;
        const unsigned long long am = __ballot(active);
        if constexpr (FEED) {
            if (am != 0ull) idleSince = 0u;
        }
        if (am == 0ull) {
            if (parking && nparked > 0) {
                service_parked();
                if (nparked > 0) {
                    if (bound.tick(0ull, parkSince, !parkProgress)) {
                        nparked = 0;
                        stop_queue(&queue);
                    }
                }
                if (nparked > 0 && exhausted && avail == 0) __builtin_amdgcn_s_sleep(8);
            }
            if constexpr (FEED) {
                if (starved && !exhausted && nparked == 0) {
                    release_resolved();
                    flush_resolved();
                    for (unsigned int round = 0;; round++) {
                        const unsigned int lim = (unsigned int)__builtin_amdgcn_readfirstlane((int)lds_load(&feedq.limit));
                        const unsigned int wd = (unsigned int)__builtin_amdgcn_readfirstlane((int)lds_load(&feedq.word));
                        if (lim != lastLimit || (wd >> 31) != 0u) {
                            lastLimit = lim;
                            idleSince = 0u;
                            break;
                        }
                        if ((round & 7u) == 0u) {
                            const unsigned int now = (unsigned int)wall_clock64();
                            if (idleSince == 0u) idleSince = now | 1u;
                            if ((int)(now - idleSince) > (int)cold_args()->feedIdleTicks) {
                                abandon_launch(kAbandonIdle);
                                stop_queue(&queue);
                                break;
                            }
                            if (launch_abandoned()) {
                                stop_queue(&queue);
                                break;
                            }
                        }
                        __builtin_amdgcn_s_sleep(127);
                        if ((round & (NWAVES - 1)) == (unsigned int)wave) {
                            ColdArgs ca = cold_args();
                            unsigned int w = __hip_atomic_load(ca->feedBcast + (blockIdx.x % kFeedBcastSlots) * kFeedBcastStride, __ATOMIC_RELAXED, __HIP_MEMORY_SCOPE_AGENT);
                            w = (unsigned int)__builtin_amdgcn_readfirstlane((int)w);
                            if (lane == 0) {
                                lds_store(&feedq.limit, feed_count(w) * (unsigned int)(ca->tilesX * ca->tilesY));
                                lds_store(&feedq.word, w);
                            }
                        }
                    }
                    continue;
                }
            }
            if (!(exhausted && avail == 0 && nparked == 0)) continue;
            if (!compaction) break;
            unsigned int old = 0;
            if (leader) old = atomicSub(&drain.alive, 1u);
            old = (unsigned int)__builtin_amdgcn_readfirstlane((int)old);
            if (old > 1u) break;
            lastAlive = true;
            unsigned int pushing = lds_load(&drain.pushing), pushed = lds_load(&drain.pushed), taken = lds_load(&drain.taken);
            bool pending = __builtin_amdgcn_readfirstlane((int)(pushing != 0u || pushed != taken)) != 0;
            if (!pending) break;
            if (leader) atomicAdd(&drain.alive, 1u);
            __builtin_amdgcn_s_sleep(1);
            continue;
        }
        if (compaction && exhausted && avail == 0 && !lastAlive && __builtin_popcountll(am) <= donateMax) {
            unsigned int old = 0, base = 0;
            if (leader) {
                atomicAdd(&drain.pushing, 1u);
                old = atomicSub(&drain.alive, 1u);
            }
            old = (unsigned int)__builtin_amdgcn_readfirstlane((int)old);
            bool committed = old > 1u;
            if (committed) {
                if (leader) {
                    while (atomicCAS(&drain.lock, 0u, 1u) != 0u) __builtin_amdgcn_s_sleep(1);
                    base = lds_load(&drain.pushed);
                }
                base = (unsigned int)__builtin_amdgcn_readfirstlane((int)base);
                unsigned int n = (unsigned int)__builtin_popcountll(am);
                if (base + n <= (unsigned int)pool_slots(NWAVES)) {
                    int rank = __builtin_amdgcn_mbcnt_hi((unsigned)(am >> 32), __builtin_amdgcn_mbcnt_lo((unsigned)am, 0u));
                    if (active) {
                        PathState st;
                        st.pix = pix;
                        st.pxy = SPP1 ? 0 : (px | (py << 16));
                        st.counters = (SPP1 ? 0 : (sample | ((needRay ? 1 : 0) << 24))) | (bounce << 12) | ((pending ? 1 : 0) << 25) | ((fj & 0x3f) << 26);
                        if (CARRY && (fj & 0x4000)) st.counters |= 1;
                        st.seed = seed;
                        st.ro[0] = ro.x; st.ro[1] = ro.y; st.ro[2] = ro.z;
                        st.rd[0] = rd.x; st.rd[1] = rd.y; st.rd[2] = rd.z;
                        st.thr[0] = throughput.x; st.thr[1] = throughput.y; st.thr[2] = throughput.z;
                        st.rad[0] = rad.x; st.rad[1] = rad.y; st.rad[2] = rad.z;
                        st.irr[0] = SPP1 ? 0.0f : irr.x; st.irr[1] = SPP1 ? 0.0f : irr.y; st.irr[2] = SPP1 ? 0.0f : irr.z;
                        if constexpr (CARRY) { st.irr[0] = laneLast[0]; st.irr[1] = laneLast[64]; st.irr[2] = laneLast[128]; }
                        st.pad = 0;
                        pool[base + rank] = st;
                    }
                    __builtin_amdgcn_fence(__ATOMIC_RELEASE, "workgroup");
                    if (leader) {
                        lds_store(&drain.pushed, base + n);
                        __builtin_amdgcn_fence(__ATOMIC_RELEASE, "workgroup");
                        atomicExch(&drain.lock, 0u);
                        atomicSub(&drain.pushing, 1u);
                    }
                    break;
                }
                if (leader) atomicExch(&drain.lock, 0u);
            } else {
                lastAlive = true;
            }
            if (leader) {
                atomicAdd(&drain.alive, 1u);
                atomicSub(&drain.pushing, 1u);
            }
        }
        if (TIMELINE) nIter++;
        PROF_MARK(0)
#ifdef PT_PROFILE
        prof_util[0] += 1ull;
        prof_util[1] += (unsigned long long)__builtin_popcountll(am);
        prof_util[2] += (unsigned long long)__builtin_popcountll(__ballot(active && pending));
#endif
        if constexpr (SPP1) {
            const bool trace = active && !pending;
            bool cont = false;
            if (trace && bounce < a.rayDepth) cont = bounce_step_t<false, MATLDS, GRID, (MATLDS && !GRID)>(sc, a.numSpheres, a.numCuboids, env, ro, rd, throughput, rad, seed, nullptr, walkFrom PROF_PASS);
            if (trace && !(GRID && walkFrom >= 0.0f)) {
                bounce++;
                pending = !cont || bounce >= a.rayDepth;
            }
#ifdef PT_PROFILE
            prof_t = __builtin_readcyclecounter();
#endif
            if (CARRY && active && pending && (fj & 0x4000)) {
                commit_resolve(pix, fj & 0x3fff, v_add(V(0.0f, 0.0f, 0.0f), rad), V(laneLast[0], laneLast[64], laneLast[128]));
                pix = -1;
                pending = false;
            }
            if (active && pending) {
                v3 firr = v_add(V(0.0f, 0.0f, 0.0f), rad);
                if (try_resolve(pix, fj, firr)) {
                    pix = -1;
                    pending = false;
                }
            }
            if (parking) {
                const bool wait = pix >= 0 && pending;
                if (park_resolves(wait, pix, fj, v_add(V(0.0f, 0.0f, 0.0f), rad))) {
                    pix = -1;
                    pending = false;
                }
                service_parked();
            }
            const bool waits = pix >= 0 && pending;
            const unsigned long long waitMask = __ballot(waits);
            if (waitMask != 0ull || nparked > 0) {
                if (bound.tick(waitMask, parkSince, nparked > 0 && !parkProgress)) {
                    if (waits) {
                        pix = -1;
                        pending = false;
                    }
                    nparked = 0;
                    stop_queue(&queue);
                } else if (__ballot(pix >= 0 && !pending) == 0ull && avail == 0) {
                    __builtin_amdgcn_s_sleep(8);
                }
            }
        } else {
        if (active && needRay) {
            primary_ray(a, px, py, seed, ro, rd);
            throughput = V(1.0f, 1.0f, 1.0f);
            rad = V(0.0f, 0.0f, 0.0f);
            bounce = 0;
            needRay = false;
        }
        {
            const bool trace = active && !pending;
            bool cont = false;
            if (trace && bounce < a.rayDepth) cont = bounce_step_t<false, MATLDS, GRID>(sc, a.numSpheres, a.numCuboids, env, ro, rd, throughput, rad, seed, nullptr, walkFrom PROF_PASS);
            if (trace) {
                const bool sliced = GRID && walkFrom >= 0.0f;
                if (!sliced) bounce++;
                if (!sliced && (!cont || bounce >= a.rayDepth)) {
                    irr = v_add(irr, rad);
                    sample++;
                    if (sample < a.spp) needRay = true;
                    else pending = true;
                }
            }
#ifdef PT_PROFILE
            prof_t = __builtin_readcyclecounter();
#endif
            if (active && pending) {
                if (try_resolve(pix, fj, irr)) {
                    pix = -1;
                    pending = false;
                }
            }
        }
        {
            const bool waits = pix >= 0 && pending;
            const unsigned long long waitMask = __ballot(waits);
            if (waitMask != 0ull) {
                unsigned int noList = 0u;
                if (bound.tick(waitMask, noList, false)) {
                    if (waits) {
                        pix = -1;
                        pending = false;
                    }
                    stop_queue(&queue);
                } else if (__ballot(pix >= 0 && !pending) == 0ull) {
                    __builtin_amdgcn_s_sleep(8);
                }
            }
        }
        }
        PROF_MARK(7)
    }
    release_resolved();
    flush_resolved();
#ifdef PT_PROFILE
    if (a.timeline && lane == 0)
        for (int k = 0; k < 8; k++) {
            atomicAdd(a.timeline + 200000 + k, prof[k]);
            if (k < 3) atomicAdd(a.timeline + 200008 + k, prof_util[k]);
            if (k < 2) atomicAdd(a.timeline + 200011 + k, prof[8 + k]);
        }
#endif
    if (TIMELINE && lane == 0) {
        unsigned long long *t = a.timeline + ((size_t)blockIdx.x * NWAVES + wave) * 4;
        t[0] = tStart; t[1] = tExhausted; t[2] = wall_clock64(); t[3] = nIter;
    }
}

__global__ __launch_bounds__(256) void pt_tile_masks_kernel(const FrameArgs a, unsigned long long *out)
{
    SceneLds sc = stage_scene(a);
    const int wave = threadIdx.x >> 6, lane = threadIdx.x & 63;
    const int tile = blockIdx.x * 4 + wave;
    if (tile >= a.tilesX * a.tilesY) return;
    const int tx = tile % a.tilesX, ty = tile / a.tilesX;
    const int gy0 = global_row(a, ty * 8);
    v3 O, A, dirs[4];
    float rho, ct, lensSin;
    tile_cone<const float *>(a.invProj, a.invW, a.invH, tx * 8, gy0, O, A, rho, ct, dirs, lensSin);
    unsigned long long masks[5];
    cone_sphere_masks(sc, a.numSpheres, O, A, rho, ct, masks);
    masks[4] = cone_cuboid_mask(sc, a.numCuboids, O, rho, ct, dirs, lensSin);
    if (lane == 0) {
        unsigned long long *o = out + (size_t)tile * kTileMaskWords;
        o[0] = masks[0]; o[1] = masks[1]; o[2] = masks[2]; o[3] = masks[3]; o[4] = masks[4]; o[5] = o[6] = o[7] = 0ull;
    }
}

hipError_t launch_tile_masks(const FrameArgs &args, unsigned long long *masks, hipStream_t stream)
{
    FrameArgs a = args;
    a.materialsInLds = 0;
    a.envFormat = 0;
    a.gridLdsBytes = 0;
    const int tiles = a.tilesX * a.tilesY;
    if (tiles <= 0) return hipSuccess;
    const size_t lds = scene_lds_bytes(a.numSpheres, a.numCuboids, 0, false);
    hipLaunchKernelGGL(pt_tile_masks_kernel, dim3((tiles + 3) / 4), dim3(256), lds, stream, a, masks);
    return hipGetLastError();
}

static int pool_tiles_for_variant(int variant)
{
    switch (variant) {
    case 2: return 8;
    case 3: return 4;
    case 4: return 16;
    case 5: return 32;
    case 6: return 2;
    default: return 8;
    }
}

constexpr size_t kLdsPerCU = 160 * 1024, kLdsGranule = 1280;
constexpr size_t kStaticLds = 64, kStaticLdsFed = 256;
constexpr long long kBatchPassWorkgroupLds = 31ll * 1024;
constexpr int kParkedFloor = 16, kParkedStep = 8;
constexpr int kCarryMinTiles = 12000;

#ifndef PT_GRID_MIN_WAVES
#define PT_GRID_MIN_WAVES 6
#endif
#ifndef PT_SPP1_WAVES
#define PT_SPP1_WAVES 6
#endif
#define PT_PERSISTENT_ROW(MW, TL, S1, ML, G, C, CP, F) {{MW, TL, S1, ML, G, C, CP, F}, pt_integrate_persistent_kernel<4, MW, TL, S1, ML, G, C, CP, F>}
static const KernelRow kPersistentKernels[] = {
    PT_PERSISTENT_ROW(6, false, true, true, false, true, false, true),
    PT_PERSISTENT_ROW(6, false, true, true, false, false, false, true),
    PT_PERSISTENT_ROW(PT_SPP1_WAVES, true, true, true, false, false, true, false),
    PT_PERSISTENT_ROW(PT_SPP1_WAVES, false, true, true, false, true, false, false),
    PT_PERSISTENT_ROW(PT_SPP1_WAVES, false, true, true, false, false, false, false),
    PT_PERSISTENT_ROW(PT_SPP1_WAVES, false, true, true, false, false, true, false),
    PT_PERSISTENT_ROW(PT_GRID_MIN_WAVES, false, true, false, true, true, false, false),
    PT_PERSISTENT_ROW(5, false, true, false, true, true, false, false),
    PT_PERSISTENT_ROW(PT_GRID_MIN_WAVES, false, true, false, true, false, false, false),
    PT_PERSISTENT_ROW(PT_SPP1_WAVES, false, true, false, false, false, true, false),
    PT_PERSISTENT_ROW(5, false, false, true, false, false, true, false),
    PT_PERSISTENT_ROW(5, false, false, false, true, false, true, false),
    PT_PERSISTENT_ROW(5, false, false, false, false, false, true, false),
};
#undef PT_PERSISTENT_ROW

LaunchPlan plan_launch(const FrameArgs &in, const Tuning &tune, bool wantFeed)
{
    LaunchPlan p = {};
    p.error = hipSuccess;
    FrameArgs &a = p.args;
    a = in;
    if (!wantFeed) { a.feedHost = nullptr; a.feedBcast = nullptr; a.feedDone = nullptr; a.displayImages[0] = a.displayImages[1] = a.displayImages[2] = nullptr; a.displayPrev = 0; a.displayOn = 0; }
    a.materialsInLds = 1;
    a.gridLdsBytes = 0;
    const int tiles = a.tilesX * a.tilesY;
    a.tilesFrameMagic = div_magic((unsigned int)tiles);
    a.tilesXMagic = div_magic((unsigned int)a.tilesX);
    size_t lds = scene_lds_bytes(a.numSpheres, a.numCuboids, a.envFormat, true);
    if (a.variant == 1) {
        p.family = kFamilySimple;
        p.workgroups = (tiles + 3) / 4;
        p.ldsBytes = lds;
    } else if (a.variant == 0 || a.variant >= 10) {
        p.family = kFamilyPersistent;
        const int waves = 4;
        int k = a.variant == 0 ? 4 : a.variant - 10;
        if (k < 0 || k > 7) k = 4;
        int blocksPerCU = k + 1;
        if (a.spp != 1 && blocksPerCU > 5) blocksPerCU = 5;
        if (a.batchFrames < 1 || a.batchFrames > MAX_BATCH_FRAMES) {
            p.error = hipErrorInvalidValue;
            return p;
        }
        if (a.batchFrames > 64) a.drainCompaction = 0;
        const int numChunks = (int)(((long long)tiles * a.batchFrames + a.queueChunk - 1) / a.queueChunk);
        auto grid_size = [&](int perCU) {
            int n = a.numCUs * perCU;
            if (n > numChunks) n = numChunks;
            return n < 1 ? 1 : n;
        };
        int nwg = grid_size(blocksPerCU);
        if (nwg > kStartedWords) a.startedFlags = nullptr;
        a.parkedMax = PARKED_MAX;
        if (tune.parkedMax >= 0) a.parkedMax = tune.parkedMax > PARKED_MAX ? PARKED_MAX : tune.parkedMax;
        const int parkedMaxPlain = a.parkedMax;
        const bool spp1 = a.spp == 1;
        const bool noBatchPass = tune.noBatchPass != 0;
        const long long batchPassMinTiles = tune.batchPassMinTiles;
        const bool smallPipelined = a.tagged && (long long)a.tilesX * a.tilesY < batchPassMinTiles;
        const bool useBatchPass = !spp1 && a.drainCompaction == 0 && !noBatchPass && !smallPipelined;
        int park = 0;
        if (useBatchPass) {
            const long long left = kBatchPassWorkgroupLds - (long long)lds - (long long)waves * 64 * (long long)sizeof(PathEntryM);
            park = (int)(left / (long long)(waves * sizeof(ContEntry))) & ~7;
            if (tune.parkCapacity >= 0) park = tune.parkCapacity & ~7;
            if (park > 128) park = 128;
            if (park < 64) park = 64;
        }
        a.contCapacity = park;
        a.contBatchMin = tune.parkMin;
        const bool noGrid = tune.noSphereGrid != 0;
#ifdef PT_PROFILE
        const bool perWaveTimeline = false;
#else
        const bool perWaveTimeline = a.timeline != nullptr;
#endif
        const bool useGrid = a.grid != nullptr && a.gridBytes > 0 && !noGrid && !perWaveTimeline;
        a.gridLdsBytes = useGrid ? (a.gridBytes + 15) & ~15 : 0;
        if (useGrid && spp1) a.drainCompaction = 0;
        lds += (size_t)a.gridLdsBytes;
        const bool gridCarry = useGrid && spp1 && tune.gridCarry != 0 && tiles >= kCarryMinTiles && tune.carryLast != 0 && a.drainCompaction == 0 && !perWaveTimeline;
        if (gridCarry && blocksPerCU > 5 && tune.gridCarry == 1) {
            blocksPerCU = 5;
            nwg = grid_size(blocksPerCU);
        }
// ... 146 lines not shown
```

### opentk-pathtracer_amd/csrc/pt_kernels.hpp

```cpp
#pragma once
#include <hip/hip_runtime.h>
#include <stddef.h>
#include <stdint.h>

namespace pt {

struct FrameArgs {
    float invProj[16];
    float invView[16];
    float viewPos[3];
    float focalLength, apertureDiameter;
    int width, height;
    int y0, rows;
    int bandRows, bandWorld, bandRank, localRow0;
    int numSpheres, numCuboids;
    int rayDepth, spp;
    int frame;
    int envSize, envFormat;
    const float *objects;
    const void *env;
    const float *srgbLut;
    float4 *accum;
    int tilesX, tilesY;
    int variant;
    unsigned int *queue;
    unsigned int *errorWord;
    unsigned int queueBase;
    int numCUs;
    int queueChunk;
    int drainCompaction;
    int batchFrames;
    int tagged;
    int keepTags;
    float chainTag;
    int contCapacity;
    int contBatchMin;
    int parkedMax;
    int materialsInLds;
    unsigned long long *timeline;
    unsigned int *startedFlags;
    unsigned int launchSeq;
    unsigned int *abandonWord;
    unsigned int *tileFlags;
    unsigned int waitBudget, waitCheckInterval;
    const unsigned char *grid;
    int gridBytes;
    int gridLdsBytes;
    unsigned int tilesFrameMagic, tilesXMagic;
    float invW, invH;
    int sceneLdsBytes;
    int gridDims[3];
    float gridLo[3], gridHi[3], gridCell[3], gridInvCell[3];
    float gridCenter[3];
    float gridReach2;
    unsigned long long sphereRunStart[4];
    const unsigned long long *tileMasks;
    float4 *snapshot;
    const unsigned int *feedHost;
    unsigned int *feedBcast;
    unsigned long long *feedDone;
    unsigned int feedIdleTicks;
    unsigned int *feedHostDone;
    unsigned long long feedBase[8];
    unsigned long long feedPixels;
    uchar4 *displayImages[3];
    int displayPrev;
    int displayOn;
    unsigned long long *audit;
    unsigned int *auditLog;
    int auditSabotage;
};
constexpr int kFrameTagMask = 0xFFFFF;
constexpr int kMaxBatchFrames = 256, kMaxUnverifiedLaunches = 128;
static_assert((long long)kMaxBatchFrames * (kMaxUnverifiedLaunches + 2) * 8 <= (kFrameTagMask + 1) / 2, "frame tags would alias within the repair window");
static_assert(kFrameTagMask + 2 < (1 << 24), "frame tags must be exact in binary32");
constexpr unsigned int kFeedClosed = 0x80000000u;
constexpr int kFeedBcastSlots = 256, kFeedBcastStride = 16;
constexpr int kFeedDoneStride = 64;
constexpr int kFeedCapacity = 32;
constexpr unsigned int kAbandonContended = 1u, kAbandonIdle = 2u;
constexpr int kAuditLogRecords = 1024, kAuditRecordWords = 12;
constexpr int kTileMaskWords = 8;
constexpr int kStartedWords = 4096;

static_assert(offsetof(FrameArgs, invProj) == 0 && offsetof(FrameArgs, invView) == 64 && offsetof(FrameArgs, viewPos) == 128 &&
                  offsetof(FrameArgs, focalLength) == 140 && offsetof(FrameArgs, apertureDiameter) == 144,
              "camera block layout");

struct AtmoArgs {
    float invProj[16];
    float invView[6][16];
    float lightPos[3];
    float lightIntensity;
    int size, iSteps, jSteps;
    float4 *out;
};

enum KernelFamily {
    kFamilySimple = 0,
    kFamilyPool = 1,
    kFamilyPersistent = 2,
    kFamilyMultisample = 3,
};
struct KernelKey {
    int minWavesPerSimd;
    bool timeline, spp1, matLds, grid, carry, compact, feed;
};
inline bool operator==(const KernelKey &a, const KernelKey &b)
{
    return a.minWavesPerSimd == b.minWavesPerSimd && a.timeline == b.timeline && a.spp1 == b.spp1 && a.matLds == b.matLds && a.grid == b.grid &&
           a.carry == b.carry && a.compact == b.compact && a.feed == b.feed;
}
struct LaunchPlan {
    hipError_t error;
    int family;
    KernelKey kernel;
    int workgroups;
    size_t ldsBytes;
    int poolTiles;
    unsigned int ticketsConsumed;
    bool fed;
    FrameArgs args;
    int workgroupsPerCU;
    bool batchPass;
    size_t queueLdsBytes, staticLdsBytes;
    int fitPerCU;
};
struct Tuning;
LaunchPlan plan_launch(const FrameArgs &in, const Tuning &tune, bool wantFeed);
int launch_kernel_row(const LaunchPlan &p);

hipError_t launch_integrate(const FrameArgs &a, hipStream_t stream, unsigned int *ticketsConsumed, int *workgroups = nullptr, bool *fed = nullptr);
hipError_t launch_repair(const FrameArgs &a, unsigned int *ctl, hipStream_t stream);
hipError_t launch_integrate_reference(const FrameArgs &a, hipStream_t stream);
hipError_t launch_repair_done(unsigned int *abandonWord, unsigned int *queueMain, unsigned int expectMain, unsigned int *queueChain,
                              unsigned int expectChain, unsigned int *ctl, hipStream_t stream);
constexpr int kFirstHitCuboidBase = 256;
hipError_t launch_first_hit(const FrameArgs &a, float4 *records, int pickTile, hipStream_t stream);
hipError_t launch_guides(const FrameArgs &a, float4 *guides, hipStream_t stream);
struct AtrousArgs {
    const float4 *colIn;
    const float4 *guides;
    float4 *colOut;
    int width, height;
    int step;
    float invSigma;
    float sigmaPlane;
    int normalPower;
};
hipError_t launch_atrous(const AtrousArgs &a, hipStream_t stream);
hipError_t launch_denoise_copy(const float4 *in, float4 *out, size_t pixels, hipStream_t stream);
struct VarianceArgs {
    const float4 *colIn;
    const float4 *guides;
    float *var;
    int width, height;
};
hipError_t launch_variance(const VarianceArgs &a, hipStream_t stream);
struct AtrousVarArgs {
    const float4 *colIn;
    const float *varIn;
    const float4 *guides;
    float4 *colOut;
    int width, height;
    int step;
    float k2;
    float sigmaPlane;
    int normalPower;
    int last;
};
hipError_t launch_atrous_var(const AtrousVarArgs &a, hipStream_t stream);
struct TemporalArgs {
    const float4 *colIn;
    const float4 *guides;
    const float4 *histImage;
    const float4 *histGuides;
    float4 *out;
    int width, height;
    float n;
    float maxHistory;
    float B[9];
    float O[3];
    float sigmaPlane;
    int normalPower;
};
hipError_t launch_temporal(const TemporalArgs &a, hipStream_t stream);
hipError_t launch_atmosphere(const AtmoArgs &a, hipStream_t stream);
hipError_t launch_atmosphere_reference(const AtmoArgs &a, hipStream_t stream);
hipError_t launch_tile_masks(const FrameArgs &a, unsigned long long *masks, hipStream_t stream);
hipError_t launch_clear(float4 *p, size_t n, hipStream_t stream);
hipError_t launch_set_alpha(float4 *p, size_t n, hipStream_t stream);
struct AssembleArgs {
    const void *stage;
    void *out;
    int width, height, bandRows, world, bytesPerPixel;
    unsigned long long partOffset[16];
};
hipError_t launch_assemble_bands(const AssembleArgs &a, hipStream_t stream);
hipError_t launch_postprocess(const float4 *accum, void *outRgba8, size_t n, hipStream_t stream);
hipError_t launch_postprocess_reference(const float4 *accum, void *outRgba8, size_t n, hipStream_t stream);
hipError_t launch_env_to_float(const void *env, int envSize, int envFormat, const float *srgbLut, float4 *out,
                               hipStream_t stream);

}
```

### opentk-pathtracer_amd/csrc/pt_renderer.hpp

```cpp
#pragma once
#include "../../include/mi355pt.h"

#include <hip/hip_runtime.h>

#include <deque>
#include <string>
#include <vector>

#include "pt_kernels.hpp"
#include "pt_sphere_grid.hpp"

namespace ptimpl {
constexpr uint32_t kAlive = 0x4d335054u;
constexpr int kMaxStripes = 4;
constexpr int kQueueWords = 128, kChainQueueWord = 64;
#ifdef PT_PROFILE
#define PT_TIMELINE_BLOCKS(h) false
#else
#define PT_TIMELINE_BLOCKS(h) ((h)->dTimeline != nullptr)
#endif
constexpr int kStartedWords = pt::kStartedWords;

struct PresentSlot {
    void *dRgba8 = nullptr;
    void *boundDev = nullptr;
    size_t boundBytes = 0;
    size_t devPixels = 0;
    uint8_t *host = nullptr;
    size_t hostPixels = 0;
    hipEvent_t toneMapped = nullptr;
    hipEvent_t copied = nullptr;
    bool inFlight = false;
    bool valid = false;
    int frame = 0, rows = 0, width = 0;
    const void *snapSource = nullptr;
    unsigned int snapGeneration = 0, abandonEpoch = 0;
    bool fedPresent = false;
    int fusedWord = 0;
    unsigned int fusedNeed = 0;
    bool fusedWaiting = false;
    int arithmetic = PT_ARITH_CONTRACT;
};
}

struct pt_renderer {
    uint32_t magic = ptimpl::kAlive;
    int device = 0;
    int width = 0, height = 0;
    int y0 = 0, rows = 0;
    int bandRows = 0, bandWorld = 1, bandRank = 0;
    int numSpheres = 0, numCuboids = 0, rayDepth = 1, spp = 1;
    float focalLength = 0.0f, apertureDiameter = 0.0f;
    int frame = 0;
    int variant = 0;
    int arithmetic = PT_ARITH_CONTRACT;
    int atmoArithmetic = PT_ARITH_CONTRACT;
    int presentArithmetic = PT_ARITH_CONTRACT;

    unsigned char basic[PT_BASIC_DATA_UBO_SIZE] = {0};
    unsigned char atmoUbo[PT_ATMOSPHERE_UBO_SIZE] = {0};

    float *dObjects = nullptr;
    unsigned char objectsShadow[PT_GAME_OBJECTS_UBO_SIZE] = {0};
    bool gridDirty = true;
    ptgrid::SphereGrid grid;
    unsigned long long sphereRunStart[4] = {~0ull, ~0ull, ~0ull, ~0ull};
    unsigned long long *dTileMasks = nullptr;
    size_t tileMaskTiles = 0;
    bool tileMasksValid = false;
    int launchesSinceInputChange = 0;
    unsigned long long statLaunches = 0, statMaskBuilds = 0, statFlushes = 0;
    unsigned char *dGrid = nullptr;
    float *dLut = nullptr;
    unsigned int *dQueue = nullptr;
    unsigned int *hostErrWord = nullptr, *devErrWord = nullptr;
    unsigned int *dAbandon = nullptr;
    unsigned int *dRepairCtl = nullptr;
    unsigned int *dTileFlags = nullptr;
    size_t tileFlagTiles = 0;
    struct LaunchRecord { pt::FrameArgs a; hipEvent_t done; };
    std::deque<LaunchRecord> unverified;
    static constexpr int kLaunchEvents = 256;
    hipEvent_t launchEvents[kLaunchEvents] = {};
    unsigned int launchEventNext = 0;
    bool repairPendingAll = false;
    bool repairCheckDue = false;
    unsigned int inconsistentSeen = 0;
    unsigned int abandonEpoch = 0;
    int overlapHoldoff = 0;
    int wallClockKhz = 100000;
    unsigned int waitBudgetUnits = 0, waitCheckUnits = 0;
    int queueChunk = 0;
    unsigned long long *dTimeline = nullptr;
    int pendingFrames = 0;
    int maxBatch = 64;
    bool maxBatchExplicit = false;
    int batchWorkgroupsPerCU = 6;
    bool batchLaunched = false;
    bool lastPresentBound = false;
    int rendersSincePresent = 0;
    int presentCadence = 0;
    hipEvent_t mainDone = nullptr;
    bool mainInFlight = false;
    hipEvent_t chainDone = nullptr;
    unsigned int *hostStarted = nullptr, *devStarted = nullptr;
    unsigned int launchSeq = 0;
    int lastWorkgroups = 0;
    int lastStreamIdx = 0;
    bool chainInFlight = false, chainPending = false;
    bool chainNeedsInputs = false;
    bool chainBroken = true;
    bool tagsLive = false;
    float lastTag = 0.0f;
    bool flushFinal = false;
    bool sawBatch = false;
    bool stripeInFlight[ptimpl::kMaxStripes] = {false, false, false, false};
    int drainCompaction = -1;
    int numCUs = 256;
    void *dEnv = nullptr;
    size_t envBytes = 0;
    int envSize = 0, envFormat = PT_ENV_RGBA32F;

    float4 *dAccum = nullptr;
    size_t accumCapacity = 0;
    float4 *boundAccum = nullptr;
    void *dRgba8 = nullptr;
    size_t rgba8Capacity = 0;
    size_t boundBytes = 0;
    float4 *dFirstHit = nullptr;
    float4 *dPick = nullptr;
    float4 *dGuides = nullptr;
    float4 *dDenoise[2] = {nullptr, nullptr};
    int denoiseResult = -1;
    int denoiseIterations = 5, denoiseNormalPower = 5;
    float denoiseSigmaColor = 0.5f, denoiseSigmaPlane = 0.02f;
    int denoiseMode = 0;
    float denoiseSigmaVariance = 6.0f;
    float *dVariance = nullptr;
    bool denoiseVarianceValid = false;
    struct DenoiseSet {
        float4 *image = nullptr, *guides = nullptr;
        float B[9] = {0}, O[3] = {0};
        unsigned long long epoch = 0;
        bool valid = false;
    };
    DenoiseSet denoiseSet[2];
    int denoiseCurrent = 0;
    unsigned long long resetEpoch = 0;
    int denoiseTemporal = 0, denoiseMaxHistory = 32;
    bool denoiseIntegratedValid = false;
    bool denoiseHistoryUsed = false;

    unsigned long long *dAudit = nullptr;
    size_t auditCapacity = 0;
    unsigned int *hostAuditLog = nullptr, *devAuditLog = nullptr;

    hipStream_t ownStream = nullptr, stream = nullptr;
    hipStream_t stripeStream[ptimpl::kMaxStripes] = {nullptr, nullptr, nullptr, nullptr};
    hipEvent_t stripeDone[ptimpl::kMaxStripes] = {nullptr, nullptr, nullptr, nullptr};
    hipEvent_t inputsReady = nullptr;
    bool mainDirty = true;
    bool stripePending[ptimpl::kMaxStripes] = {false, false, false, false};
    int stripeRow0[ptimpl::kMaxStripes] = {0, 0, 0, 0}, stripeRows[ptimpl::kMaxStripes] = {0, 0, 0, 0};
    unsigned int stripeQueueBase[ptimpl::kMaxStripes] = {0, 0, 0, 0};
    unsigned int chainQueueBase = 0;
    hipEvent_t evBegin = nullptr, evEnd = nullptr;

    hipStream_t copyStream = nullptr;
    ptimpl::PresentSlot slots[PT_PRESENT_SLOTS];
    static constexpr int kSnapshots = 3;
    float4 *dSnap[kSnapshots] = {nullptr, nullptr, nullptr};
    size_t snapCapacity[kSnapshots] = {0, 0, 0};
    hipEvent_t snapRead[kSnapshots] = {nullptr, nullptr, nullptr};
    bool snapReadPending[kSnapshots] = {false, false, false};
    int snapNext = 0;
    unsigned int snapGeneration[kSnapshots] = {0, 0, 0};
    float4 *snapshotTarget = nullptr;
    int snapshotIndex = -1;
    int snapFrame = -1;
    struct SnapLaunch { hipStream_t stream; hipEvent_t done; size_t firstPixel, pixels; };
    std::vector<SnapLaunch> snapLaunches;

    struct FeedState {
        bool open = false;
        int firstFrame = 0, published = 0;
        int streamIdx = 0, hostWord = 0;
        unsigned int seq = 0;
        int workgroups = 0, queueChunk = 8;
        long long tilesFrame = 0;
        bool withMasks = false;
        bool display = false;
        unsigned int slots16 = 0;
        int pendingSlot = -1;
        unsigned long long base[8] = {0, 0, 0, 0, 0, 0, 0, 0};
        unsigned long long pixelsPerFrame = 0;
    } feed;
    static constexpr int kFeedHostWords = 8;
    unsigned int *hostFeedDone = nullptr, *devFeedHostDone = nullptr;
    unsigned int *hostFeed = nullptr, *devFeedHost = nullptr;
    hipEvent_t feedWordBusy[kFeedHostWords] = {};
    int feedWordNext = 0;
    unsigned int *dFeedDev = nullptr;
    unsigned long long *dFeedDone = nullptr;
    unsigned long long feedDoneBase[2][8] = {{0, 0, 0, 0, 0, 0, 0, 0}, {0, 0, 0, 0, 0, 0, 0, 0}};
    hipEvent_t feedResetEvent = nullptr;
    bool feedCountersStale = false;
    int fusedOrphanSlot = -1;
    int feedIdleStrikes = 0, feedHoldoff = 0;
    unsigned long long statPublishes = 0, statFeedOpens = 0, statFeedIdle = 0;

    std::vector<pt_renderer *> parts;
    int groupBand = 8;
    bool gatherDirect = true;
    hipEvent_t gatherReady = nullptr;
    void *dGatherFull = nullptr;
    size_t gatherFullBytes = 0;
    void *dGatherStage = nullptr;
    size_t gatherStageBytes = 0;
    void *dAsyncStage = nullptr;
    size_t asyncStageBytes = 0;

    std::string error;

    bool isGroup() const { return !parts.empty(); }
    bool externalStream() const { return stream != ownStream; }
    float4 *accum() const { return boundAccum ? boundAccum : dAccum; }
    size_t tilePixels() const { return (size_t)rows * (size_t)width; }
};

namespace ptimpl {

inline bool timeline_blocks_pipelining(const pt_renderer *h) { return PT_TIMELINE_BLOCKS(h); }
int fail(pt_handle h, int code, const std::string &msg);
int hip_fail(pt_handle h, hipError_t e, const char *what);

#define PT_CHECK_HANDLE(h)                                                                                             \
    do {                                                                                                               \
        if (!(h) || (h)->magic != ptimpl::kAlive) return ptimpl::fail(nullptr, PT_E_BAD_HANDLE, "bad handle");        \
    } while (0)

#define PT_HIP(h, call)                                                                                                \
    do {                                                                                                               \
        hipError_t e_ = (call);                                                                                        \
        if (e_ != hipSuccess) return ptimpl::hip_fail((h), e_, #call);                                                 \
    } while (0)

int bind_device(pt_handle h);
void feed_close(pt_handle h);
int flush_frames(pt_handle h);
int flush_frames_bounded(pt_handle h, long waitUs, int maxLaunches);
int batch_limit(pt_handle h);
bool launch_ready(pt_handle h);
int join_stripes(pt_handle h, bool repairNow = true);
int settle_handover(pt_handle h);
hipEvent_t next_launch_event(pt_handle h);
int fix_alpha(pt_handle h, bool repairNow = true);
int ensure_stripe(pt_handle h, int j);
hipStream_t stripe_stream(pt_handle h, int j);
int tone_map_into(pt_handle h, void *dst);
inline hipError_t launch_tone_map(int arithmetic, const float4 *src, void *dstRgba8, size_t pixels, hipStream_t stream)
{
    return arithmetic == PT_ARITH_REFERENCE ? pt::launch_postprocess_reference(src, dstRgba8, pixels, stream) : pt::launch_postprocess(src, dstRgba8, pixels, stream);
}
int ensure_slot_device(pt_handle h, int slot, size_t pixels);
int ensure_slot_host(pt_handle h, int slot, size_t pixels);
int ensure_slot_events(pt_handle h, int slot);
void free_slots(pt_handle h);
int wait_slot(pt_handle h, PresentSlot &s, bool *abandoned);

int group_destroy(pt_handle g);
int group_set_size(pt_handle g, int width, int height);
int group_read_result(pt_handle g, float *dst, size_t row_pitch_bytes);
int group_write_result(pt_handle g, const float *src, size_t row_pitch_bytes, int frame_index);
int group_present_rgba8(pt_handle g, uint8_t *dst, size_t row_pitch_bytes);
int group_present_async(pt_handle g, int slot);
int group_result_device_ptr(pt_handle g, void **out_ptr, size_t *out_bytes);
int group_timer_end(pt_handle g, float *out_ms);
int free_first_hit(pt_handle h);
int free_denoise(pt_handle h);
int group_first_hit_read(pt_handle g, void *dst, size_t row_pitch_bytes);
int group_pick(pt_handle g, int x, int y, int frame_index, int *out_id, float *out_t, float *out_origin, float *out_dir);

}
```

Baseline: 19590.

## Precompute cubemap seam wrap indices into a lookup table for env sampling

Adds a per-environment table, built by a small kernel whenever the cubemap is set, that maps each face edge texel just outside the face to its wrapped neighbour-face index. Bilinear env sampling near face seams now reads these indices instead of computing face_to_dir and reprojecting per tap, and falls back to the general path only for corner taps, under a wave ballot. It also changes the float4 texel load to three scalar loads, accumulates taps with fused multiply-adds, and adds profiling counters. The cost is an extra global table read per seam tap plus a table rebuild on env changes, and it only affects the rarely taken seam branch.

```diff
diff --git a/opentk-pathtracer_amd/csrc/mi355pt.cpp b/opentk-pathtracer_amd/csrc/mi355pt.cpp
--- a/opentk-pathtracer_amd/csrc/mi355pt.cpp
+++ b/opentk-pathtracer_amd/csrc/mi355pt.cpp
@@ -273,6 +273,25 @@
         if (set.guides) PT_HIP(h, hipFree(set.guides));
         set.guides = nullptr;
     }
+    return PT_OK;
+}
+
+int bind_env_seam(pt_handle h, int size)
+{
+    if (h->dEnvSeam && h->envSeamSize == size) return PT_OK;
+    const size_t n = pt::env_seam_entries(size);
+    if (n > h->envSeamCapacity) {
+        PT_HIP(h, hipStreamSynchronize(h->stream));
+        if (h->dEnvSeam) PT_HIP(h, hipFree(h->dEnvSeam));
+        h->dEnvSeam = nullptr;
+        h->envSeamCapacity = 0;
+        h->envSeamSize = 0;
+        PT_HIP(h, hipMalloc((void **)&h->dEnvSeam, n * sizeof(unsigned int)));
+        h->envSeamCapacity = n;
+    }
+    h->envSeamSize = 0;
+    PT_HIP(h, pt::launch_env_seam_table(h->dEnvSeam, size, h->stream));
+    h->envSeamSize = size;
     return PT_OK;
 }
 }
@@ -516,6 +535,7 @@
     if (h->hostAuditLog) (void)hipHostFree(h->hostAuditLog);
     if (h->dAudit) (void)hipFree(h->dAudit);
     if (h->dEnv) (void)hipFree(h->dEnv);
+    if (h->dEnvSeam) (void)hipFree(h->dEnvSeam);
     if (h->dAccum) (void)hipFree(h->dAccum);
     if (h->dRgba8) (void)hipFree(h->dRgba8);
     if (h->dFirstHit) (void)hipFree(h->dFirstHit);
@@ -724,7 +744,7 @@
         PT_HIP(h, hipMemcpyAsync((char *)h->dEnv + f * faceBytes, faces[f], faceBytes, hipMemcpyHostToDevice, h->stream));
     h->envSize = face_size;
     h->envFormat = format;
-    return PT_OK;
+    return ptimpl::bind_env_seam(h, face_size);
 }
 
 }
@@ -761,6 +781,7 @@
     a.envFormat = h->envFormat;
     a.objects = h->dObjects;
     a.env = h->dEnv;
+    a.envSeam = h->dEnvSeam;
     a.srgbLut = h->dLut;
     a.tilesX = (h->width + 7) / 8;
     a.bandRows = h->bandRows;
@@ -1774,7 +1795,7 @@
     PT_HIP(h, h->atmoArithmetic == PT_ARITH_REFERENCE ? pt::launch_atmosphere_reference(a, h->stream) : pt::launch_atmosphere(a, h->stream));
     h->envSize = size;
     h->envFormat = PT_ENV_RGBA32F;
-    return PT_OK;
+    return ptimpl::bind_env_seam(h, size);
 }
 
 PT_API int pt_atmosphere_set_arithmetic(pt_handle h, int mode)
diff --git a/opentk-pathtracer_amd/csrc/pt_denoise.hip b/opentk-pathtracer_amd/csrc/pt_denoise.hip
--- a/opentk-pathtracer_amd/csrc/pt_denoise.hip
+++ b/opentk-pathtracer_amd/csrc/pt_denoise.hip
@@ -20,7 +20,7 @@
     const int ly = ty * 8 + (lane >> 3);
     if (px >= a.width || ly >= a.rows) return;
 #ifdef PT_PROFILE
-    unsigned long long prof_dummy[10] = {0, 0, 0, 0, 0, 0, 0, 0, 0, 0};
+    unsigned long long prof_dummy[12] = {0, 0, 0, 0, 0, 0, 0, 0, 0, 0, 0, 0};
 #endif
     uint32_t seed = pixel_seed(px, global_row(a, ly), a.frame);
     v3 ro, rd;
diff --git a/opentk-pathtracer_amd/csrc/pt_device.hpp b/opentk-pathtracer_amd/csrc/pt_device.hpp
--- a/opentk-pathtracer_amd/csrc/pt_device.hpp
+++ b/opentk-pathtracer_amd/csrc/pt_device.hpp
@@ -45,6 +45,7 @@
     const void *data;
     LdsFloats lut;
     int size, format;
+    const unsigned int *seam;
 };
 
 typedef const __attribute__((address_space(4))) FrameArgs *ColdArgs;
@@ -56,15 +57,19 @@
     return p;
 }
 
-PT_DEV v3 env_texel(const EnvRef &e, int face, int x, int y)
-{
-    size_t idx = ((size_t)face * e.size + (size_t)y) * e.size + (size_t)x;
+PT_DEV v3 env_texel_at(const EnvRef &e, size_t idx)
+{
     if (e.format == 0) {
-        float4 t = ((const float4 *)e.data)[idx];
-        return V(t.x, t.y, t.z);
+        const float *t = (const float *)e.data + 4 * idx;
+        return V(t[0], t[1], t[2]);
     }
     uchar4 t = ((const uchar4 *)e.data)[idx];
     return V(e.lut[t.x], e.lut[t.y], e.lut[t.z]);
+}
+
+PT_DEV v3 env_texel(const EnvRef &e, int face, int x, int y)
+{
+    return env_texel_at(e, ((size_t)face * e.size + (size_t)y) * e.size + (size_t)x);
 }
 
 PT_DEV void face_to_dir(int face, float sc, float tc, float &x, float &y, float &z)
@@ -91,10 +96,8 @@
     }
 }
 
-PT_DEV v3 env_texel_wrapped(const EnvRef &e, int face, int ix, int iy)
-{
-    int S = e.size;
-    if (ix >= 0 && ix < S && iy >= 0 && iy < S) return env_texel(e, face, ix, iy);
+PT_DEV unsigned int env_wrapped_index(int S, int face, int ix, int iy)
+{
     float fs = (float)S;
     float rfs = f_div_ieee(1.0f, fs);
     float sc = ((float)ix + 0.5f) * rfs * 2.0f - 1.0f;
@@ -109,10 +112,46 @@
     int nx = (int)__builtin_floorf(u), ny = (int)__builtin_floorf(v);
     nx = nx < 0 ? 0 : (nx > S - 1 ? S - 1 : nx);
     ny = ny < 0 ? 0 : (ny > S - 1 ? S - 1 : ny);
-    return env_texel(e, nface, nx, ny);
-}
-
-PT_DEV v3 sample_env(const EnvRef &e, v3 d)
+    return ((unsigned int)nface * (unsigned int)S + (unsigned int)ny) * (unsigned int)S + (unsigned int)nx;
+}
+
+PT_DEV void env_seam_tap(int side, int k, int S, int &ix, int &iy)
+{
+    ix = side == 0 ? -1 : (side == 1 ? S : k);
+    iy = side == 2 ? -1 : (side == 3 ? S : k);
+}
+
+PT_DEV v3 env_texel_wrapped(const EnvRef &e, int face, int ix, int iy)
+{
+    int S = e.size;
+    if (ix >= 0 && ix < S && iy >= 0 && iy < S) return env_texel(e, face, ix, iy);
+    return env_texel_at(e, env_wrapped_index(S, face, ix, iy));
+}
+
+PT_DEV unsigned int env_tap_index(const unsigned int *seam, int face, int S, int x, int y, bool miss, bool &general)
+{
+    const bool inx = (unsigned)x < (unsigned)S, iny = (unsigned)y < (unsigned)S;
+    const int off = inx ? y : x;
+    const bool edge = inx != iny && (off == -1 || off == S);
+    general = !miss && !(inx && iny) && !edge;
+    unsigned int idx = 0u;
+    if (inx && iny) idx = ((unsigned)face * (unsigned)S + (unsigned)y) * (unsigned)S + (unsigned)x;
+    if (edge) {
+        const unsigned int side = (inx ? 2u : 0u) + (off < 0 ? 0u : 1u);
+        idx = seam[((unsigned)face * 4u + side) * (unsigned)S + (unsigned)(inx ? x : y)];
+    }
+    return idx;
+}
+
+#ifdef PT_PROFILE
+#define PROF_SEAM_PARAM , unsigned long long *profSeam
+#define PROF_SEAM_PASS , prof + (MASKED ? 11 : 10)
+#else
+#define PROF_SEAM_PARAM
+#define PROF_SEAM_PASS
+#endif
+
+PT_DEV v3 sample_env(const EnvRef &e, v3 d PROF_SEAM_PARAM)
 {
     int S = e.size, face;
     float sc, tc, ma;
@@ -142,19 +181,46 @@
             t01 = V(e.lut[c.x], e.lut[c.y], e.lut[c.z]); t11 = V(e.lut[d.x], e.lut[d.y], e.lut[d.z]);
         }
     } else {
-        bool miss00 = offx0 && offy0, miss10 = offx1 && offy0, miss01 = offx0 && offy1, miss11 = offx1 && offy1;
-        v3 zero = V(0.0f, 0.0f, 0.0f);
-        t00 = miss00 ? zero : env_texel_wrapped(e, face, x0, y0);
-        t10 = miss10 ? zero : env_texel_wrapped(e, face, x1, y0);
-        t01 = miss01 ? zero : env_texel_wrapped(e, face, x0, y1);
-        t11 = miss11 ? zero : env_texel_wrapped(e, face, x1, y1);
-        if (miss00 || miss10 || miss01 || miss11) {
-            float a = (miss00 ? w00 : miss10 ? w10 : miss01 ? w01 : w11) * 0.333333343f;
-            w00 = miss00 ? 0.0f : w00 + a;
-            w10 = miss10 ? 0.0f : w10 + a;
-            w01 = miss01 ? 0.0f : w01 + a;
-            w11 = miss11 ? 0.0f : w11 + a;
-        }
+#ifdef PT_PROFILE
+        profSeam[0] = 1ull;
+#endif
+        const unsigned int *seam = e.seam ? e.seam : cold_args()->envSeam;
+        {
+            bool miss00 = offx0 && offy0, miss10 = offx1 && offy0, miss01 = offx0 && offy1, miss11 = offx1 && offy1;
+            if (miss00 || miss10 || miss01 || miss11) {
+                float a = (miss00 ? w00 : miss10 ? w10 : miss01 ? w01 : w11) * 0.333333343f;
+                w00 = miss00 ? 0.0f : w00 + a;
+                w10 = miss10 ? 0.0f : w10 + a;
+                w01 = miss01 ? 0.0f : w01 + a;
+                w11 = miss11 ? 0.0f : w11 + a;
+            }
+        }
+        bool g00, g10, g01, g11;
+        unsigned int i00 = env_tap_index(seam, face, S, x0, y0, offx0 && offy0, g00), i10 = env_tap_index(seam, face, S, x1, y0, offx1 && offy0, g10);
+        unsigned int i01 = env_tap_index(seam, face, S, x0, y1, offx0 && offy1, g01), i11 = env_tap_index(seam, face, S, x1, y1, offx1 && offy1, g11);
+        const unsigned int gmask = (g00 ? 1u : 0u) | (g10 ? 2u : 0u) | (g01 ? 4u : 0u) | (g11 ? 8u : 0u);
+        if (__builtin_expect(__ballot(gmask != 0u) != 0ull, 0)) {
+#pragma clang loop unroll(disable)
+            for (int t = 0; t < 4; t++) {
+                if ((gmask >> t) & 1u) {
+                    const unsigned int i = env_wrapped_index(S, face, x0 + (t & 1), y0 + (t >> 1));
+                    if (t == 0) i00 = i;
+                    else if (t == 1) i10 = i;
+                    else if (t == 2) i01 = i;
+                    else i11 = i;
+                }
+            }
+        }
+        const v3 zero = V(0.0f, 0.0f, 0.0f);
+        v3 tx = (offx0 && offy0) ? zero : env_texel_at(e, i00);
+        v3 o = V(tx.x * w00, tx.y * w00, tx.z * w00);
+        tx = (offx1 && offy0) ? zero : env_texel_at(e, i10);
+        o = V(f_fma(tx.x, w10, o.x), f_fma(tx.y, w10, o.y), f_fma(tx.z, w10, o.z));
+        tx = (offx0 && offy1) ? zero : env_texel_at(e, i01);
+        o = V(f_fma(tx.x, w01, o.x), f_fma(tx.y, w01, o.y), f_fma(tx.z, w01, o.z));
+        tx = (offx1 && offy1) ? zero : env_texel_at(e, i11);
+        o = V(f_fma(tx.x, w11, o.x), f_fma(tx.y, w11, o.y), f_fma(tx.z, w11, o.z));
+        return o;
     }
     v3 o;
     o.x = f_fma(t11.x, w11, f_fma(t01.x, w01, f_fma(t10.x, w10, t00.x * w00)));
@@ -702,10 +768,10 @@
     v3 e;
     if (env.data == nullptr) {
         ColdArgs ca = cold_args();
-        EnvRef cold{ca->env, env.lut, ca->envSize, ca->envFormat};
-        e = sample_env(cold, rd);
+        EnvRef cold{ca->env, env.lut, ca->envSize, ca->envFormat, nullptr};
+        e = sample_env(cold, rd PROF_SEAM_PASS);
     } else {
-        e = sample_env(env, rd);
+        e = sample_env(env, rd PROF_SEAM_PASS);
     }
     rad = V(f_fma(e.x, throughput.x, rad.x), f_fma(e.y, throughput.y, rad.y), f_fma(e.z, throughput.z, rad.z));
     PROF_MARK(6)
@@ -721,7 +787,7 @@
 PT_DEV v3 radiance(const FrameArgs &a, const SceneLds &sc, const EnvRef &env, v3 ro, v3 rd, uint32_t &seed)
 {
 #ifdef PT_PROFILE
-    unsigned long long prof_dummy[10] = {0, 0, 0, 0, 0, 0, 0, 0, 0, 0};
+    unsigned long long prof_dummy[12] = {0, 0, 0, 0, 0, 0, 0, 0, 0, 0, 0, 0};
 #endif
     v3 throughput = V(1.0f, 1.0f, 1.0f), rad = V(0.0f, 0.0f, 0.0f);
     for (int i = 0; i < a.rayDepth; i++)
diff --git a/opentk-pathtracer_amd/csrc/pt_first_hit.hip b/opentk-pathtracer_amd/csrc/pt_first_hit.hip
--- a/opentk-pathtracer_amd/csrc/pt_first_hit.hip
+++ b/opentk-pathtracer_amd/csrc/pt_first_hit.hip
@@ -20,7 +20,7 @@
     const int ly = ty * 8 + (lane >> 3);
     if (px >= a.width || ly >= a.rows) return;
 #ifdef PT_PROFILE
-    unsigned long long prof_dummy[10] = {0, 0, 0, 0, 0, 0, 0, 0, 0, 0};
+    unsigned long long prof_dummy[12] = {0, 0, 0, 0, 0, 0, 0, 0, 0, 0, 0, 0};
 #endif
     uint32_t seed = pixel_seed(px, global_row(a, ly), a.frame);
     v3 ro, rd;
diff --git a/opentk-pathtracer_amd/csrc/pt_helper_kernels.hip b/opentk-pathtracer_amd/csrc/pt_helper_kernels.hip
--- a/opentk-pathtracer_amd/csrc/pt_helper_kernels.hip
+++ b/opentk-pathtracer_amd/csrc/pt_helper_kernels.hip
@@ -84,6 +84,23 @@
     return hipGetLastError();
 }
 
+__global__ __launch_bounds__(256) void pt_env_seam_kernel(unsigned int *table, int size)
+{
+    const size_t i = (size_t)blockIdx.x * 256 + threadIdx.x;
+    if (i >= env_seam_entries(size)) return;
+    const int row = (int)(i / (size_t)size), k = (int)(i - (size_t)row * (size_t)size);
+    int ix, iy;
+    env_seam_tap(row & 3, k, size, ix, iy);
+    table[i] = env_wrapped_index(size, row >> 2, ix, iy);
+}
+
+hipError_t launch_env_seam_table(unsigned int *table, int envSize, hipStream_t stream)
+{
+    const size_t n = env_seam_entries(envSize);
+    hipLaunchKernelGGL(pt_env_seam_kernel, dim3((unsigned)((n + 255) / 256)), dim3(256), 0, stream, table, envSize);
+    return hipGetLastError();
+}
+
 __global__ __launch_bounds__(256) void pt_postprocess_kernel(const float4 *accum, uchar4 *out, size_t n)
 {
     __builtin_amdgcn_s_setprio(3);
diff --git a/opentk-pathtracer_amd/csrc/pt_integrate_multisample.hip b/opentk-pathtracer_amd/csrc/pt_integrate_multisample.hip
--- a/opentk-pathtracer_amd/csrc/pt_integrate_multisample.hip
+++ b/opentk-pathtracer_amd/csrc/pt_integrate_multisample.hip
@@ -21,7 +21,7 @@
     }
     CHAOS(1);
     SceneLds sc = stage_scene(a);
-    EnvRef env{nullptr, (LdsFloats)sc.lut, 0, 0};
+    EnvRef env{nullptr, (LdsFloats)sc.lut, 0, 0, nullptr};
     const int tid = threadIdx.x, wave = tid >> 6, lane = tid & 63;
     char *ringBase = (char *)g_lds + scene_lds_bytes(a.numSpheres, a.numCuboids, a.envFormat, a.materialsInLds != 0, a.gridLdsBytes);
     PathEntryM *ring = (PathEntryM *)ringBase + wave * 64;
@@ -83,7 +83,7 @@
     bool needRay = false, pending = false;
     float walkFrom = -1.0f;
 #ifdef PT_PROFILE
-    unsigned long long prof_dummy[10] = {0, 0, 0, 0, 0, 0, 0, 0, 0, 0};
+    unsigned long long prof_dummy[12] = {0, 0, 0, 0, 0, 0, 0, 0, 0, 0, 0, 0};
 #endif
     uint32_t seed = 0;
     v3 ro = V(0, 0, 0), rd = V(0, 0, 1), throughput = V(1, 1, 1), rad = V(0, 0, 0);
diff --git a/opentk-pathtracer_amd/csrc/pt_integrate_persistent.hip b/opentk-pathtracer_amd/csrc/pt_integrate_persistent.hip
--- a/opentk-pathtracer_amd/csrc/pt_integrate_persistent.hip
+++ b/opentk-pathtracer_amd/csrc/pt_integrate_persistent.hip
@@ -8,7 +8,7 @@
 __global__ __launch_bounds__(256) void pt_integrate_kernel(const FrameArgs a)
 {
     SceneLds sc = stage_scene(a);
-    EnvRef env{a.env, (LdsFloats)sc.lut, a.envSize, a.envFormat};
+    EnvRef env{a.env, (LdsFloats)sc.lut, a.envSize, a.envFormat, a.envSeam};
     const int tid = threadIdx.x;
     const int b = xcd_band_id(blockIdx.x, gridDim.x);
     const int wave = tid >> 6, lane = tid & 63;
@@ -29,11 +29,11 @@
 {
     if (*(const volatile unsigned int *)a.abandonWord > a.launchSeq) return;
     SceneLds sc = stage_scene(a);
-    EnvRef env{a.env, (LdsFloats)sc.lut, a.envSize, a.envFormat};
+    EnvRef env{a.env, (LdsFloats)sc.lut, a.envSize, a.envFormat, a.envSeam};
     const int tid = threadIdx.x, wave = tid >> 6, lane = tid & 63;
     const int tiles = a.tilesX * a.tilesY, n = a.batchFrames;
 #ifdef PT_PROFILE
-    unsigned long long prof_dummy[10] = {0, 0, 0, 0, 0, 0, 0, 0, 0, 0};
+    unsigned long long prof_dummy[12] = {0, 0, 0, 0, 0, 0, 0, 0, 0, 0, 0, 0};
 #endif
     for (int tile = (int)blockIdx.x * 4 + wave; tile < tiles; tile += (int)gridDim.x * 4) {
         const int tx = tile % a.tilesX, ty = tile / a.tilesX;
@@ -113,7 +113,7 @@
 __global__ __launch_bounds__(256) void pt_integrate_pool_kernel(const FrameArgs a, const int poolTiles)
 {
     SceneLds sc = stage_scene(a);
-    EnvRef env{a.env, (LdsFloats)sc.lut, a.envSize, a.envFormat};
+    EnvRef env{a.env, (LdsFloats)sc.lut, a.envSize, a.envFormat, a.envSeam};
     const int tid = threadIdx.x;
     const int b = xcd_band_id(blockIdx.x, gridDim.x);
     const int wave = tid >> 6;
@@ -125,7 +125,7 @@
     if (next >= poolEnd) return;
 
 #ifdef PT_PROFILE
-    unsigned long long prof_dummy[10] = {0, 0, 0, 0, 0, 0, 0, 0, 0, 0};
+    unsigned long long prof_dummy[12] = {0, 0, 0, 0, 0, 0, 0, 0, 0, 0, 0, 0};
 #endif
     int pix = -1;
     int px = 0, py = 0, sample = 0, bounce = 0;
@@ -266,7 +266,7 @@
     }
     CHAOS(1);
     SceneLds sc = stage_scene(a);
-    EnvRef env{nullptr, (LdsFloats)sc.lut, 0, 0};
+    EnvRef env{nullptr, (LdsFloats)sc.lut, 0, 0, nullptr};
     const int tid = threadIdx.x, wave = tid >> 6, lane = tid & 63;
     [[maybe_unused]] unsigned int *const myDone = waveDone + (FEED ? wave * 8 : 0);
     [[maybe_unused]] auto count_resolved = [&](int rfj) -> void {
@@ -379,7 +379,7 @@
     bool exhausted = false;
     bool lastAlive = false;
 #ifdef PT_PROFILE
-    unsigned long long prof[10] = {0, 0, 0, 0, 0, 0, 0, 0, 0, 0}, prof_dummy[10] = {0, 0, 0, 0, 0, 0, 0, 0, 0, 0}, prof_util[3] = {0, 0, 0};
+    unsigned long long prof[12] = {0, 0, 0, 0, 0, 0, 0, 0, 0, 0, 0, 0}, prof_dummy[12] = {0, 0, 0, 0, 0, 0, 0, 0, 0, 0, 0, 0}, prof_util[3] = {0, 0, 0}, prof_seam[3] = {0, 0, 0};
     unsigned long long prof_t = __builtin_readcyclecounter();
 #endif
     unsigned long long tStart = 0, tExhausted = 0, nIter = 0;
@@ -570,6 +570,11 @@
                                 tkeep = !try_resolve(tpix, tfj, tirr);
                             }
                         }
+#ifdef PT_PROFILE
+                        prof_seam[1] += 1ull;
+                        prof_seam[2] += __ballot(prof_dummy[11] != 0ull) != 0ull ? 1ull : 0ull;
+                        prof_dummy[11] = 0ull;
+#endif
                         if (parking) {
                             const bool twait = valid && !tcont && tkeep;
                             if (park_resolves(twait, tpix, tfj, v_add(V(0.0f, 0.0f, 0.0f), trad))) tkeep = false;
@@ -861,6 +866,10 @@
             const bool trace = active && !pending;
             bool cont = false;
             if (trace && bounce < a.rayDepth) cont = bounce_step_t<false, MATLDS, GRID, (MATLDS && !GRID)>(sc, a.numSpheres, a.numCuboids, env, ro, rd, throughput, rad, seed, nullptr, walkFrom PROF_PASS);
+#ifdef PT_PROFILE
+            prof_seam[0] += __ballot(prof[10] != 0ull) != 0ull ? 1ull : 0ull;
+            prof[10] = 0ull;
+#endif
             if (trace && !(GRID && walkFrom >= 0.0f)) {
                 bounce++;
                 pending = !cont || bounce >= a.rayDepth;
@@ -914,6 +923,10 @@
             const bool trace = active && !pending;
             bool cont = false;
             if (trace && bounce < a.rayDepth) cont = bounce_step_t<false, MATLDS, GRID>(sc, a.numSpheres, a.numCuboids, env, ro, rd, throughput, rad, seed, nullptr, walkFrom PROF_PASS);
+#ifdef PT_PROFILE
+            prof_seam[0] += __ballot(prof[10] != 0ull) != 0ull ? 1ull : 0ull;
+            prof[10] = 0ull;
+#endif
             if (trace) {
                 const bool sliced = GRID && walkFrom >= 0.0f;
                 if (!sliced) bounce++;
@@ -961,6 +974,7 @@
             atomicAdd(a.timeline + 200000 + k, prof[k]);
             if (k < 3) atomicAdd(a.timeline + 200008 + k, prof_util[k]);
             if (k < 2) atomicAdd(a.timeline + 200011 + k, prof[8 + k]);
+            if (k < 3) atomicAdd(a.timeline + 200013 + k, prof_seam[k]);
         }
 #endif
     if (TIMELINE && lane == 0) {
diff --git a/opentk-pathtracer_amd/csrc/pt_kernels.hpp b/opentk-pathtracer_amd/csrc/pt_kernels.hpp
--- a/opentk-pathtracer_amd/csrc/pt_kernels.hpp
+++ b/opentk-pathtracer_amd/csrc/pt_kernels.hpp
@@ -19,6 +19,7 @@
     int envSize, envFormat;
     const float *objects;
     const void *env;
+    const unsigned int *envSeam;
     const float *srgbLut;
     float4 *accum;
     int tilesX, tilesY;
@@ -199,6 +200,8 @@
 hipError_t launch_assemble_bands(const AssembleArgs &a, hipStream_t stream);
 hipError_t launch_postprocess(const float4 *accum, void *outRgba8, size_t n, hipStream_t stream);
 hipError_t launch_postprocess_reference(const float4 *accum, void *outRgba8, size_t n, hipStream_t stream);
+__host__ __device__ inline size_t env_seam_entries(int envSize) { return (size_t)24 * (size_t)envSize; }
+hipError_t launch_env_seam_table(unsigned int *table, int envSize, hipStream_t stream);
 hipError_t launch_env_to_float(const void *env, int envSize, int envFormat, const float *srgbLut, float4 *out,
                                hipStream_t stream);
 
diff --git a/opentk-pathtracer_amd/csrc/pt_renderer.hpp b/opentk-pathtracer_amd/csrc/pt_renderer.hpp
--- a/opentk-pathtracer_amd/csrc/pt_renderer.hpp
+++ b/opentk-pathtracer_amd/csrc/pt_renderer.hpp
@@ -120,6 +120,9 @@
     void *dEnv = nullptr;
     size_t envBytes = 0;
     int envSize = 0, envFormat = PT_ENV_RGBA32F;
+    unsigned int *dEnvSeam = nullptr;
+    size_t envSeamCapacity = 0;
+    int envSeamSize = 0;
 
     float4 *dAccum = nullptr;
     size_t accumCapacity = 0;
@@ -278,6 +281,7 @@
 int group_timer_end(pt_handle g, float *out_ms);
 int free_first_hit(pt_handle h);
 int free_denoise(pt_handle h);
+int bind_env_seam(pt_handle h, int size);
 int group_first_hit_read(pt_handle g, void *dst, size_t row_pitch_bytes);
 int group_pick(pt_handle g, int x, int y, int frame_index, int *out_id, float *out_t, float *out_origin, float *out_dir);
 
```

Result: no change. 19560 (-0.2%).
